# FrankYard/CDV-SLAM

Hardware: AMD Instinct MI355X
Metric: frames/sec per GPU (CDVO update, 96 patches, win=10); ATE vs ref (higher is better)
Workload: dtype f32

## Files before the change

cdv_slam_amd/csrc/cdv_graph.h:

```cpp
#pragma once
#include <stddef.h>
#include <stdint.h>

namespace cdv {

enum {
  GM_U = 0,
  GM_KMIN = 2,
  GM_KMAX = 3,
  GM_JMIN = 4,
  GM_JMAX = 5,
  GM_ERROR = 6,
  GM_E = 7,
  GM_KRANGE = 8,
  GM_HAS_II = 9,
  GM_STAGE = 16,
  GM_MODE = 20,
  GM_GEN = 21,
  GM_TCAP = 23,
  GM_GENNEXT = 24,
  GM_PRECN = 26,
  GM_OVFN = 28,
  GM_TERR = 30,
  GM_WORDS = 64
};

constexpr int GRAPH_MAX_BLOCKS = 1024;
constexpr int ELL_SLOTS = 32;
constexpr int ELL_CHUNKS = 4096;
constexpr int TAB_MAX_DEG = 128;
constexpr int64_t TAB_CAP_MAX = 1 << 16;
constexpr int ORD_BINS = 32;
constexpr int CORR_REC_WORDS = 24;

struct CorrStream {
  const float* coords;
  uint32_t kmod, jmod, kmagic, jmagic, Ng, slots;
  float inv_scale0;
};

struct GraphLayout {
  int64_t E_max, k_range;
  size_t meta, stage, khist, kcount, kcursor, krank, koff_u, kx, ku, pcsr_tmp, pcsr, prec, pell, nprev, nnext, ocnt, order, crec,
      tcur, town, tdeg, tplo, tkid, tlive, ttab, tovf, tprec, total;
  int64_t tab_chunks;
  int64_t ell_chunks;
};

static inline size_t align256(size_t x) { return (x + 255) & ~(size_t)255; }

static inline GraphLayout graph_layout(int64_t E_max, int64_t k_range) {
  GraphLayout L;
  L.E_max = E_max; L.k_range = k_range;
  const int64_t U_max = k_range < E_max ? k_range : E_max;
  size_t o = 0;
  L.meta = o;     o = align256(o + sizeof(int32_t) * GM_WORDS);
  L.stage = o;    o = align256(o + sizeof(int32_t) * 4 * GRAPH_MAX_BLOCKS);
  L.khist = o;    o = align256(o + sizeof(int32_t) * (size_t)(k_range + 1));
  L.kcount = o;   o = align256(o + sizeof(int32_t) * (size_t)(k_range + 1));
  L.kcursor = o;  o = align256(o + sizeof(int32_t) * (size_t)(k_range + 1));
  L.krank = o;    o = align256(o + sizeof(int32_t) * (size_t)k_range);
  L.koff_u = o;   o = align256(o + sizeof(int32_t) * (size_t)(U_max + 1));
  L.kx = o;       o = align256(o + sizeof(int64_t) * (size_t)U_max);
  L.ku = o;       o = align256(o + sizeof(int32_t) * (size_t)E_max);
  L.pcsr_tmp = o; o = align256(o + sizeof(int32_t) * 4 * (size_t)E_max);
  L.pcsr = o;     o = align256(o + sizeof(int32_t) * (size_t)E_max);
  L.prec = o;     o = align256(o + sizeof(int32_t) * 4 * (size_t)E_max);
  L.ell_chunks = (U_max + 15) / 16 < ELL_CHUNKS ? (U_max + 15) / 16 : ELL_CHUNKS;
  L.pell = o;     o = align256(o + sizeof(int32_t) * 4 * 16 * (size_t)ELL_SLOTS * (size_t)L.ell_chunks);
  L.nprev = o;    o = align256(o + sizeof(int32_t) * (size_t)E_max);
  L.nnext = o;    o = align256(o + sizeof(int32_t) * (size_t)E_max);
  L.ocnt = o;     o = align256(o + sizeof(int32_t) * ORD_BINS * GRAPH_MAX_BLOCKS);
  L.order = o;    o = align256(o + sizeof(int32_t) * (size_t)E_max);
  L.crec = o;     o = align256(o + sizeof(uint32_t) * CORR_REC_WORDS * (size_t)E_max);
  const int64_t tcap = k_range < TAB_CAP_MAX ? k_range : TAB_CAP_MAX;
  L.tab_chunks = (tcap + 15) / 16;
  L.tcur = o;     o = align256(o + sizeof(int32_t) * (size_t)(tcap + 16));
  L.town = o;     o = align256(o + sizeof(uint64_t) * (size_t)(tcap + 16));
  L.tdeg = o;     o = align256(o + sizeof(int32_t) * (size_t)(tcap + 16));
  L.tplo = o;     o = align256(o + sizeof(int32_t) * (size_t)(tcap + 16));
  L.tkid = o;     o = align256(o + sizeof(int32_t) * (size_t)(tcap + 16));
  L.tlive = o;    o = align256(o + sizeof(int32_t) * (size_t)(tcap / 8 + 2));
  L.ttab = o;     o = align256(o + sizeof(int32_t) * 4 * 16 * (size_t)ELL_SLOTS * (size_t)L.tab_chunks);
  L.tovf = o;     o = align256(o + sizeof(int32_t) * 4 * (size_t)E_max);
  L.tprec = o;    o = align256(o + sizeof(int32_t) * 4 * ((size_t)E_max + 1));
  L.total = o;
  return L;
}

struct GraphView {
  int32_t* meta;
  int32_t *stage, *khist, *kcount, *kcursor, *krank, *koff_u, *ku, *pcsr_tmp, *pcsr, *prec, *pell, *nprev, *nnext, *ocnt, *order;
  uint32_t* crec;
  int32_t *tcur, *tdeg, *tplo, *tkid, *tlive, *ttab, *tovf, *tprec;
  unsigned long long* town;
  int64_t* kx;
};

static inline GraphView graph_view(void* ws, const GraphLayout& L) {
  char* b = (char*)ws;
  GraphView v;
  v.meta = (int32_t*)(b + L.meta);
  v.stage = (int32_t*)(b + L.stage);
  v.khist = (int32_t*)(b + L.khist);
  v.kcount = (int32_t*)(b + L.kcount);
  v.kcursor = (int32_t*)(b + L.kcursor);
  v.krank = (int32_t*)(b + L.krank);
  v.koff_u = (int32_t*)(b + L.koff_u);
  v.kx = (int64_t*)(b + L.kx);
  v.ku = (int32_t*)(b + L.ku);
  v.pcsr_tmp = (int32_t*)(b + L.pcsr_tmp);
  v.pcsr = (int32_t*)(b + L.pcsr);
  v.prec = (int32_t*)(b + L.prec);
  v.pell = (int32_t*)(b + L.pell);
  v.nprev = (int32_t*)(b + L.nprev);
  v.nnext = (int32_t*)(b + L.nnext);
  v.ocnt = (int32_t*)(b + L.ocnt);
  v.order = (int32_t*)(b + L.order);
  v.crec = (uint32_t*)(b + L.crec);
  v.tcur = (int32_t*)(b + L.tcur);
  v.tdeg = (int32_t*)(b + L.tdeg);
  v.tplo = (int32_t*)(b + L.tplo);
  v.town = (unsigned long long*)(b + L.town);
  v.tkid = (int32_t*)(b + L.tkid);
  v.tlive = (int32_t*)(b + L.tlive);
  v.ttab = (int32_t*)(b + L.ttab);
  v.tovf = (int32_t*)(b + L.tovf);
  v.tprec = (int32_t*)(b + L.tprec);
  return v;
}

}

bool cdv_graph_lookup(const void* ws, cdv::GraphLayout* out);

void cdv_graph_forget(const void* ws);

void cdv_graph_no_corr_order(const void* ws);

bool cdv_graph_has_ii(const void* ws);

bool cdv_graph_is_table(const void* ws);
int64_t cdv_graph_table_capacity(const void* ws);

namespace cdv {
__device__ __forceinline__ int graph_error(const int32_t* __restrict__ meta) {
  const int e = meta[GM_ERROR], t0 = meta[GM_TERR], t1 = meta[GM_TERR + 1], g = meta[GM_GEN];
  return meta[GM_MODE] ? ((g & 1) ? t1 : t0) : e;
}
__device__ __forceinline__ int graph_error_of(const int32_t* __restrict__ meta, bool table) {
  const int e = meta[GM_ERROR], t0 = meta[GM_TERR], t1 = meta[GM_TERR + 1], g = meta[GM_GEN];
  return table ? ((g & 1) ? t1 : t0) : e;
}
}

namespace cdv { struct TFillArgs; }
int cdv_graph_table_prepare(const int64_t* ii, const int64_t* jj, const int64_t* kk, int64_t E, void* ws, size_t ws_bytes,
                            int64_t E_max, int64_t k_range, int64_t tab_cap, int64_t* ix, int64_t* jx, void* stream,
                            cdv::TFillArgs* fill, int* fill_blocks, const int32_t* dyn = nullptr);
int cdv_graph_table_finish(const cdv::TFillArgs& fill, int fill_blocks, void* ws, int64_t E_max, int64_t k_range, int64_t* ix,
                           int64_t* jx, const float* poses, const float* patches, const float* intr, float* coords_out,
                           bool with_stream, void* stream);

namespace cdv { struct HistArgs; }
int cdv_graph_prepare(const int64_t* jj, const int64_t* kk, int64_t E, void* ws, size_t ws_bytes, int64_t E_max,
                      int64_t k_range, int64_t* ix, int64_t* jx, void* stream, cdv::HistArgs* hist, int* hist_blocks);
int cdv_graph_finish(const int64_t* ii, const int64_t* jj, const int64_t* kk, int64_t E, void* ws, int64_t E_max,
                     int64_t k_range, int hist_blocks, int64_t* ix, int64_t* jx, void* stream);
```

cdv_slam_amd/csrc/corr.hip:

```cpp
#include <math.h>
#include <stdlib.h>

#include "cdv_common.h"
#include "cdv_graph.h"
#include "cdv_parts.h"

CDV_STAMP_TU(corr)

#ifdef CDV_STAMPS
#define CDV_EXP(bit) ((exp & (bit)) != 0)
#else
#define CDV_EXP(bit) false
#endif

namespace {

constexpr int PADX = CDV_FMAP_PADX;
constexpr int PADY = CDV_FMAP_PADY;

constexpr int RAW_ROWS = 12;
constexpr int NQ_MAX = 8;
constexpr int RAW_MSH = RAW_ROWS * 16 + 12;
constexpr int RAW_HALFS = 9 * RAW_MSH;
constexpr int CW = 4;
constexpr int OUT_POLICY = 16;
constexpr int OUT_HALFS = 896;
constexpr int WAVE_LDS_BYTES = RAW_HALFS * 2 + OUT_HALFS * 2;
constexpr int DUMP_OFF_B = 3712;
constexpr int WAVE_LDS2_BYTES = DUMP_OFF_B + 512;
static_assert(RAW_HALFS * 2 <= DUMP_OFF_B && OUT_HALFS * 2 <= RAW_HALFS * 2, "LDS layout");

typedef _Float16 cdv_half4 __attribute__((ext_vector_type(4)));
typedef _Float16 cdv_half2 __attribute__((ext_vector_type(2)));

__device__ __forceinline__ void wave_lds_sync() {
  asm volatile("s_waitcnt lgkmcnt(0)" ::: "memory");
  __builtin_amdgcn_wave_barrier();
}

template <bool IS_MIN>
__device__ __forceinline__ int row16_reduce_i32(int v) {
#define CDV_ROR(n)                                                                                             \
  if (IS_MIN) asm volatile("s_nop 1\n\tv_min_i32_dpp %0, %1, %1 row_ror:" #n " row_mask:0xf bank_mask:0xf" : "=v"(v) : "0"(v)); \
  else asm volatile("s_nop 1\n\tv_max_i32_dpp %0, %1, %1 row_ror:" #n " row_mask:0xf bank_mask:0xf" : "=v"(v) : "0"(v));
  CDV_ROR(8) CDV_ROR(4) CDV_ROR(2) CDV_ROR(1)
#undef CDV_ROR
  return v;
}

__device__ __forceinline__ void row16_minmax4(int x, int y, int& xmin, int& xmax, int& ymin, int& ymax) {
  int a = x, b = x, c = y, d = y;
#define CDV_STEP(n)                                                                                  \
  asm volatile("v_min_i32_dpp %0, %0, %0 row_ror:" #n " row_mask:0xf bank_mask:0xf\n\t"               \
               "v_max_i32_dpp %1, %1, %1 row_ror:" #n " row_mask:0xf bank_mask:0xf\n\t"               \
               "v_min_i32_dpp %2, %2, %2 row_ror:" #n " row_mask:0xf bank_mask:0xf\n\t"               \
               "v_max_i32_dpp %3, %3, %3 row_ror:" #n " row_mask:0xf bank_mask:0xf"                    \
               : "+v"(a), "+v"(b), "+v"(c), "+v"(d));
  asm volatile("s_nop 1" ::: "memory");
  CDV_STEP(8) CDV_STEP(4) CDV_STEP(2) CDV_STEP(1)
#undef CDV_STEP
  xmin = a; xmax = b; ymin = c; ymax = d;
}

struct LevelParams {
  const _Float16* fmap;
  int H, W;
  float inv_scale;
  int shift;
};

struct Box {
  int x0, y0;
  int Wb, Hb;
  bool fast;
  int stride;
  bool outside;
  int x0c, y0c;
};

__device__ __forceinline__ int floor_clamped(float v) {
  return (int)fminf(fmaxf(floorf(v), -1.0e6f), 1.0e6f);
}

__device__ __forceinline__ Box make_box(int ixmin, int ixmax, int iymin, int iymax, const LevelParams& LP) {
  Box b;
  b.x0 = ixmin - 3;
  b.y0 = iymin - 3;
  b.Wb = ixmax + 4 - b.x0 + 1;
  b.Hb = iymax + 4 - b.y0 + 1;
  b.fast = (b.Wb <= 16) && (b.Hb <= RAW_ROWS);
  b.stride = b.fast ? b.Wb : 16;
  b.x0c = min(max(b.x0, -PADX), LP.W);
  b.y0c = min(max(b.y0, -PADY), LP.H);
  b.outside = (b.x0c != b.x0) || (b.y0c != b.y0);
  return b;
}

template <int KS>
__device__ __forceinline__ void mfma_row_store(const cdv_half8 (&win)[KS], const cdv_half8 (&pat)[KS],
                                               _Float16* __restrict__ raw_lane, int t) {
  cdv_float4 acc = {0.f, 0.f, 0.f, 0.f};
#pragma unroll
  for (int s = 0; s < KS; s++) acc = __builtin_amdgcn_mfma_f32_16x16x32_f16(win[s], pat[s], acc, 0, 0, 0);
  cdv_half4 h = {(_Float16)acc[0], (_Float16)acc[1], (_Float16)acc[2], (_Float16)acc[3]};
  *reinterpret_cast<cdv_half4*>(raw_lane + t * 16) = h;
}

struct BlendGeo {
  int hb;
  int stride_b;
  cdv_half2 wx;
  float dy;
};

__device__ __forceinline__ BlendGeo blend_geo(float xm, float ym, int m, int xo, const LevelParams& LP,
                                              const Box& b, bool per_pixel) {
  BlendGeo g;
  const float x = xm * LP.inv_scale, y = ym * LP.inv_scale;
  const float fxf = floorf(x), fyf = floorf(y);
  const float dx = (float)(_Float16)(x - fxf);
  g.wx = cdv_half2{(_Float16)(1.0f - dx), (_Float16)dx};
  g.dy = (float)(_Float16)(y - fyf);
  const int bx = per_pixel ? 0 : floor_clamped(x) - 3 - b.x0;
  const int by = per_pixel ? 0 : floor_clamped(y) - 3 - b.y0;
  g.hb = 2 * (m * RAW_MSH + __mul24(by, b.stride) + bx + xo);
  g.stride_b = 2 * b.stride;
  return g;
}

__device__ __forceinline__ float dot2_f16(uint32_t pair, uint32_t w) {
  float r;
  asm("v_dot2_f32_f16 %0, %1, %2, 0" : "=v"(r) : "v"(pair), "v"(w));
  return r;
}

template <typename TR>
__device__ __forceinline__ void blend_level(const _Float16* __restrict__ raw, const BlendGeo& g, TR (&res)[7]) {
  const char* rb = reinterpret_cast<const char*>(raw);
  float h[8];
  const int hb1 = g.hb + g.stride_b;
  const char* p0 = rb + (g.hb & ~3);
  const char* p1 = rb + (hb1 & ~3);
  const unsigned s0 = (unsigned)g.hb << 3, s1 = (unsigned)hb1 << 3;
  const int step2 = 2 * g.stride_b;
  const uint32_t wxb = __builtin_bit_cast(uint32_t, g.wx);
#pragma unroll
  for (int r = 0; r < 8; r++) {
    const uint32_t* pd = reinterpret_cast<const uint32_t*>((r & 1) ? p1 : p0);
    const uint32_t lo = pd[0], hi = pd[1];
    const uint32_t pr = __builtin_amdgcn_alignbit(hi, lo, (r & 1) ? s1 : s0);
    h[r] = dot2_f16(pr, wxb);
    if (r & 1) p1 += step2; else p0 += step2;
  }
#pragma unroll
  for (int yo = 0; yo < 7; yo++) res[yo] = (TR)__builtin_fmaf(g.dy, h[yo + 1] - h[yo], h[yo]);
}

template <int KS, int LM = 1>
__device__ __forceinline__ void slow_level(const LevelParams& LP, int64_t jslot, float xv, float yv,
                                           const cdv_half8 (&pat)[KS], _Float16* __restrict__ raw, int lane, int C) {
  const int n = lane & 15, g = lane >> 4;
  const int Wp = LP.W + 2 * PADX, Hp = LP.H + 2 * PADY;
  const _Float16* fbase = LP.fmap + (size_t)jslot * Hp * Wp * C;
#pragma unroll 1
  for (int m = 0; m < 9; m++) {
    const float xm = __int_as_float(__builtin_amdgcn_readlane(__float_as_int(xv), LM * m));
    const float ym = __int_as_float(__builtin_amdgcn_readlane(__float_as_int(yv), LM * m));
    const int x0 = floor_clamped(xm * LP.inv_scale) - 3, y0 = floor_clamped(ym * LP.inv_scale) - 3;
    const int x0c = min(max(x0, -PADX), LP.W), y0c = min(max(y0, -PADY), LP.H);
    const bool outside = (x0c != x0) || (y0c != y0);
#pragma unroll 1
    for (int t2 = 0; t2 < 4; t2++) {
      const int py = y0c + PADY + 2 * t2 + (n >> 3), px = x0c + PADX + (n & 7);
      cdv_float4 acc = {0.f, 0.f, 0.f, 0.f};
#pragma unroll
      for (int s = 0; s < KS; s++) {
        const int chg = min(32 * s + 8 * g, C - 8);
        const cdv_half8 v = *reinterpret_cast<const cdv_half8*>(fbase + ((size_t)py * Wp + px) * C + chg);
        acc = __builtin_amdgcn_mfma_f32_16x16x32_f16(v, pat[s], acc, 0, 0, 0);
      }
      if (n == m) {
        const int row = 2 * t2 + (g >> 1), col = 4 * (g & 1);
        cdv_half4 h = {(_Float16)acc[0], (_Float16)acc[1], (_Float16)acc[2], (_Float16)acc[3]};
        if (outside) h = cdv_half4{0, 0, 0, 0};
        *reinterpret_cast<cdv_half4*>(raw + m * RAW_MSH + row * 16 + col) = h;
      }
    }
  }
}

__device__ __forceinline__ void zero_raw(_Float16* __restrict__ raw, int lane) {
  typedef uint32_t cdv_u32x4z __attribute__((ext_vector_type(4)));
  const cdv_u32x4z z = {0u, 0u, 0u, 0u};
  for (int i = lane; i < RAW_HALFS / 8; i += 64) reinterpret_cast<cdv_u32x4z*>(raw)[i] = z;
}

template <int KS>
__global__ __launch_bounds__(256) void corr_wide_kernel(const _Float16* __restrict__ gmap, LevelParams L0,
                                                         LevelParams L1, const float* __restrict__ coords,
                                                         const int64_t* __restrict__ kk,
                                                         const int64_t* __restrict__ jj,
                                                         const int32_t* __restrict__ order,
                                                         _Float16* __restrict__ out, int E, int64_t Ng, int64_t slots,
                                                         int C, int nlev, int64_t kmod, int64_t jmod, uint32_t kmagic,
                                                         uint32_t jmagic, int gmap_pm,
                                                         int exp) {
  extern __shared__ __attribute__((aligned(16))) unsigned char smem_raw[];
  const int lane = threadIdx.x & 63;
  const int wave = __builtin_amdgcn_readfirstlane(threadIdx.x >> 6);
  _Float16* raw = reinterpret_cast<_Float16*>(smem_raw + (size_t)wave * WAVE_LDS_BYTES);
  _Float16* outT = raw + RAW_HALFS;
  const int p = blockIdx.x * 4 + wave;
  if (p >= E) return;
  const int e = order ? __builtin_amdgcn_readfirstlane(order[p]) : p;
  CDV_STAMP(corr, p, 0);

  int64_t kpatch = kk[e], jslot = jj[e];
  if (kmod > 0 && kpatch >= 0 && kpatch < ((int64_t)1 << 31)) {
    const uint32_t x = (uint32_t)kpatch, d = (uint32_t)kmod;
    const uint32_t q = __builtin_amdgcn_readfirstlane((int)__umulhi(x, kmagic));
    const int32_t r = (int32_t)(x - q * d);
    kpatch = (d == 1u) ? 0 : (r < 0 ? r + (int32_t)d : r);
  }
  if (jmod > 0 && jslot >= 0 && jslot < ((int64_t)1 << 31)) {
    const uint32_t x = (uint32_t)jslot, d = (uint32_t)jmod;
    const uint32_t q = __builtin_amdgcn_readfirstlane((int)__umulhi(x, jmagic));
    const int32_t r = (int32_t)(x - q * d);
    jslot = (d == 1u) ? 0 : (r < 0 ? r + (int32_t)d : r);
  }
  const bool idx_ok = kpatch >= 0 && kpatch < Ng && jslot >= 0 && jslot < slots;
  if (!idx_ok) { kpatch = 0; jslot = 0; }
  if (CDV_EXP(16)) jslot = 0;
  const float* cptr = coords + (size_t)e * 18;
  const int mm = lane < 9 ? lane : 0;
  const int bm = min(lane / 7, 8), bxo = lane - 7 * (lane / 7);
  const int cval = __float_as_int(cptr[min(lane, 17)]);
  const float xv = __int_as_float(__builtin_amdgcn_ds_bpermute(4 * mm, cval));
  const float yv = __int_as_float(__builtin_amdgcn_ds_bpermute(4 * (9 + mm), cval));
  const float xb = __int_as_float(__builtin_amdgcn_ds_bpermute(4 * bm, cval));
  const float yb = __int_as_float(__builtin_amdgcn_ds_bpermute(4 * (9 + bm), cval));
  const int ixl = floor_clamped(xv * L0.inv_scale), iyl = floor_clamped(yv * L0.inv_scale);
  const int ixmin = __builtin_amdgcn_readfirstlane(row16_reduce_i32<true>(ixl));
  const int ixmax = __builtin_amdgcn_readfirstlane(row16_reduce_i32<false>(ixl));
  const int iymin = __builtin_amdgcn_readfirstlane(row16_reduce_i32<true>(iyl));
  const int iymax = __builtin_amdgcn_readfirstlane(row16_reduce_i32<false>(iyl));
  const Box b0 = make_box(ixmin, ixmax, iymin, iymax, L0);
  const int sh1 = nlev == 2 ? L1.shift : 0;
  const Box b1 = make_box(ixmin >> sh1, ixmax >> sh1, iymin >> sh1, iymax >> sh1, nlev == 2 ? L1 : L0);
  CDV_STAMP(corr, p, 1);

  const int n = lane & 15, g = lane >> 4;
  cdv_half8 pat[KS];
  if (gmap_pm) {
    typedef int cdv_i32x4p __attribute__((ext_vector_type(4)));
    const unsigned tile_b = 9u * (unsigned)C * 2u;
    const auto rs = __builtin_amdgcn_make_buffer_rsrc(
        const_cast<char*>(reinterpret_cast<const char*>(gmap) + (size_t)kpatch * tile_b), (short)0, (int)tile_b, 0x00020000);
#pragma unroll
    for (int s = 0; s < KS; s++) {
      const int chg = 32 * s + 8 * g;
      const unsigned voff = (chg < C) ? (unsigned)(n * C + chg) * 2u : 0x40000000u;
      pat[s] = __builtin_bit_cast(cdv_half8, (cdv_i32x4p)__builtin_amdgcn_raw_buffer_load_b128(rs, (int)voff, 0, 0));
    }
  } else {
    const _Float16* gp = gmap + (size_t)kpatch * C * 9 + (n < 9 ? n : 0);
#pragma unroll
    for (int s = 0; s < KS; s++) {
#pragma unroll
      for (int j = 0; j < 8; j++) {
        const int ch = 32 * s + 8 * g + j;
        const _Float16 v = gp[min(ch, C - 1) * 9];
        pat[s][j] = (n < 9 && ch < C) ? v : (_Float16)0.f;
      }
    }
  }

  float res0[7], res1[7];
#pragma unroll
  for (int i = 0; i < 7; i++) { res0[i] = 0.f; res1[i] = 0.f; }
  _Float16* raw_lane = (n < 9) ? raw + n * RAW_MSH + 4 * g : outT + ((n - 9) * 4 + g) * 4;

  for (int lev = 0; lev < nlev; lev++) {
    const LevelParams& LP = lev == 0 ? L0 : L1;
    Box b = lev == 0 ? b0 : b1;
    b.stride = 16;
    const int Wp = LP.W + 2 * PADX, Hp = LP.H + 2 * PADY;
    if (lev == 1) wave_lds_sync();
    if (b.fast && !b.outside) {
      const _Float16* fb = LP.fmap + (((size_t)jslot * Hp + (b.y0c + PADY)) * Wp + (b.x0c + PADX)) * C;
      for (int t = 0; t < b.Hb; t++) {
        cdv_half8 wa[KS];
#pragma unroll
        for (int s = 0; s < KS; s++)
          wa[s] = *reinterpret_cast<const cdv_half8*>(fb + ((size_t)t * Wp + n) * C + min(32 * s + 8 * g, C - 8));
        cdv_float4 acc = {0.f, 0.f, 0.f, 0.f};
#pragma unroll
        for (int s = 0; s < KS; s++) acc = __builtin_amdgcn_mfma_f32_16x16x32_f16(wa[s], pat[s], acc, 0, 0, 0);
        if (n < 9) {
          cdv_half4 h = {(_Float16)acc[0], (_Float16)acc[1], (_Float16)acc[2], (_Float16)acc[3]};
          *reinterpret_cast<cdv_half4*>(raw_lane + t * 16) = h;
        }
      }
    } else if (!b.fast) {
      slow_level<KS>(LP, jslot, xv, yv, pat, raw, lane, C);
    }
    wave_lds_sync();
    if (!(b.fast && b.outside)) {
      const BlendGeo gg = blend_geo(xb, yb, bm, bxo, LP, b, !b.fast);
      if (lev == 0) blend_level(raw, gg, res0); else blend_level(raw, gg, res1);
    }
  }

  if (lane < 63 && !CDV_EXP(512)) {
    if (nlev == 2) {
      uint32_t* o32 = reinterpret_cast<uint32_t*>(outT) + bxo * 63 + bm;
#pragma unroll
      for (int yo = 0; yo < 7; yo++) {
        const _Float16 h0 = idx_ok ? (_Float16)res0[yo] : (_Float16)0.f;
        const _Float16 h1 = idx_ok ? (_Float16)res1[yo] : (_Float16)0.f;
        const uint32_t lo = __builtin_bit_cast(unsigned short, h0), hi = __builtin_bit_cast(unsigned short, h1);
        o32[yo * 9] = lo | (hi << 16);
      }
    } else {
#pragma unroll
      for (int yo = 0; yo < 7; yo++) outT[(bxo * 7 + yo) * 9 + bm] = idx_ok ? (_Float16)res0[yo] : (_Float16)0.f;
    }
  }
  wave_lds_sync();
  CDV_STAMP(corr, p, 7);
  if (!CDV_EXP(2)) {
  if (nlev == 2) {
    const uint32_t* src = reinterpret_cast<const uint32_t*>(outT);
    uint32_t* dst = reinterpret_cast<uint32_t*>(out) + (size_t)e * 441;
    typedef uint32_t cdv_u32x4 __attribute__((ext_vector_type(4)));
    typedef uint32_t cdv_u32x4u __attribute__((ext_vector_type(4), aligned(4)));
    const cdv_u32x4 v0 = *reinterpret_cast<const cdv_u32x4*>(src + 4 * lane);
    *reinterpret_cast<cdv_u32x4u*>(dst + 4 * lane) = v0;
    if (lane < 46) {
      const cdv_u32x4 v1 = *reinterpret_cast<const cdv_u32x4*>(src + 256 + 4 * lane);
      *reinterpret_cast<cdv_u32x4u*>(dst + 256 + 4 * lane) = v1;
    }
    if (lane == 63) dst[440] = src[440];
  } else {
    _Float16* dst = out + (size_t)e * 441;
#pragma unroll
    for (int i = 0; i < 7; i++) {
      const int t = i * 64 + lane;
      if (t < 441) dst[t] = outT[t];
    }
  }
  }
  CDV_STAMP(corr, p, 8);
}

struct CorrLevel {
  const char* base_m;
  int H, W;
  float inv_scale;
  int shift;
  uint32_t pitch;
  uint32_t slot_bytes;
};
struct CorrArgs2 {
  const float* coords;
  const int64_t* kk;
  const int64_t* jj;
  const int32_t* order;
  int E;
  uint32_t kmod, jmod, kmagic, jmagic;
  uint32_t Ng, slots;
  const char* gmap;
  _Float16* out;
  CorrLevel L0, L1;
  int C;
  int gmap_pm;
  int exp;
  int out_stride, out_off, out_pitch;
  const float* coords_ref;
  float ref_mul;
  const uint32_t* rec;
  const int32_t* dynE;
};

constexpr uint32_t FBIAS = 0x4B000000u;

__device__ __forceinline__ LevelParams level_params(const CorrLevel& L) {
  return LevelParams{reinterpret_cast<const _Float16*>(L.base_m + (size_t)FBIAS), L.H, L.W, L.inv_scale, L.shift};
}

struct EdgeCoords {
  int cval;
  float xb, yb;
  int ixmin, ixmax, iymin, iymax;
};

template <int CC, int NLEV, bool REC>
__device__ __forceinline__ void corr_edge(const CorrArgs2& a, int p, int e, const EdgeCoords& ec, uint32_t kq, uint32_t jq,
                                          bool idx_ok, int lane, _Float16* __restrict__ raw, _Float16* __restrict__ outT) {
  CDV_STAMP(corr, p, 0);
  const int C = CC ? CC : a.C;
#ifdef CDV_STAMPS
  const int exp = a.exp;
#endif
  const int mm = lane < 9 ? lane : 0;
  const int bm = min(lane / 7, 8), bxo = lane - 7 * (lane / 7);
  const int n = lane & 15, g = lane >> 4;
  if (!idx_ok) { kq = 0u; jq = 0u; }
  if (CDV_EXP(16)) jq = 0u;
  const int64_t jslot = (int64_t)jq;

  typedef int cdv_i32x4 __attribute__((ext_vector_type(4)));
  cdv_half8 pat[1];
  if (a.gmap_pm) {
    const unsigned tile_b = 9u * (unsigned)C * 2u;
    const auto rs = __builtin_amdgcn_make_buffer_rsrc(const_cast<char*>(a.gmap) + (size_t)(kq * tile_b), (short)0,
                                                      (int)tile_b, 0x00020000);
    const unsigned voff = (8 * g < C) ? (unsigned)(n * C + 8 * g) * 2u : 0x40000000u;
    pat[0] = __builtin_bit_cast(cdv_half8, (cdv_i32x4)__builtin_amdgcn_raw_buffer_load_b128(rs, (int)voff, 0, 0));
  } else {
    const _Float16* gp = reinterpret_cast<const _Float16*>(a.gmap) + (size_t)kq * C * 9 + (n < 9 ? n : 0);
#pragma unroll
    for (int j = 0; j < 8; j++) {
      const int ch = 8 * g + j;
      const _Float16 v = gp[min(ch, C - 1) * 9];
      pat[0][j] = (n < 9 && ch < C) ? v : (_Float16)0.f;
    }
  }

  const LevelParams L0 = level_params(a.L0), L1 = level_params(NLEV == 2 ? a.L1 : a.L0);
  float xv, yv, xb, yb;
  int ixmin, ixmax, iymin, iymax;
  if (REC) {
    xb = ec.xb; yb = ec.yb;
    xv = xb; yv = yb;
    ixmin = ec.ixmin; ixmax = ec.ixmax; iymin = ec.iymin; iymax = ec.iymax;
  } else {
    const int cval = ec.cval;
    xv = __int_as_float(__builtin_amdgcn_ds_bpermute(4 * mm, cval));
    yv = __int_as_float(__builtin_amdgcn_ds_bpermute(4 * (9 + mm), cval));
    xb = __int_as_float(__builtin_amdgcn_ds_bpermute(4 * bm, cval));
    yb = __int_as_float(__builtin_amdgcn_ds_bpermute(4 * (9 + bm), cval));
    const int ixl = floor_clamped(xv * L0.inv_scale), iyl = floor_clamped(yv * L0.inv_scale);
    int vxmin, vxmax, vymin, vymax;
    row16_minmax4(ixl, iyl, vxmin, vxmax, vymin, vymax);
    ixmin = __builtin_amdgcn_readfirstlane(vxmin); ixmax = __builtin_amdgcn_readfirstlane(vxmax);
    iymin = __builtin_amdgcn_readfirstlane(vymin); iymax = __builtin_amdgcn_readfirstlane(vymax);
  }
  const Box b0 = make_box(ixmin, ixmax, iymin, iymax, L0);
  const int sh1 = NLEV == 2 ? L1.shift : 0;
  const Box b1 = make_box(ixmin >> sh1, ixmax >> sh1, iymin >> sh1, iymax >> sh1, L1);
  CDV_STAMP(corr, p, 1);

  _Float16 res0[7], res1[7];
  _Float16* raw_lane = (n < 9) ? raw + n * RAW_MSH + 4 * g
                               : reinterpret_cast<_Float16*>(reinterpret_cast<char*>(raw) + DUMP_OFF_B +
                                                             4 * ((n * (RAW_MSH / 2) + 2 * g) & 31));

  const unsigned CB = (unsigned)C * 2u;
  const char* r0 = a.L0.base_m + (size_t)(jq * a.L0.slot_bytes + (unsigned)(b0.y0c + PADY) * a.L0.pitch +
                                          (unsigned)(b0.x0c + PADX) * CB);
  const CorrLevel& A1 = NLEV == 2 ? a.L1 : a.L0;
  const char* r1 = A1.base_m + (size_t)(jq * A1.slot_bytes + (unsigned)(b1.y0c + PADY) * A1.pitch +
                                        (unsigned)(b1.x0c + PADX) * CB);
  const unsigned pitch0 = a.L0.pitch, pitch1 = A1.pitch;
  cdv_half8 w[NQ_MAX][1];
  const bool do0 = b0.fast && !b0.outside && idx_ok;
  const bool do1 = NLEV == 2 && b1.fast && !b1.outside && idx_ok;
  const int nq0 = (b0.Wb * b0.Hb + 15) >> 4, nq1 = (b1.Wb * b1.Hb + 15) >> 4;
  typedef float cdv_f32x2 __attribute__((ext_vector_type(2)));
  const float nhalf = (float)n + 0.5f;
  const float lanebase = (8 * g < C) ? (float)((unsigned)n * CB + (unsigned)(8 * g) * 2u) + 8388608.0f : 33554432.0f;
  constexpr int NQF0 = 8, NQF1 = 6;
#define CDV2_LOAD_SETUP(BX, RB, PITCH)                                                             \
    const unsigned Wb_ = (unsigned)(BX).Wb, pitch_ = (PITCH);                                      \
    const auto rsrc_ = __builtin_amdgcn_make_buffer_rsrc(const_cast<char*>(RB), (short)0,          \
                                                         (int)((unsigned)(BX).Hb * pitch_ + FBIAS), 0x00020000); \
    const float invW_ = __builtin_amdgcn_rcpf((float)Wb_);                                         \
    const float wrapf_ = (float)(pitch_ - Wb_ * CB);                                               \
    const cdv_f32x2 dtb_ = {16.0f * invW_, (float)(16u * CB)};
#define CDV2_LD1(q)                                                                                \
    {                                                                                              \
      const float vf_ = __builtin_fmaf(__builtin_floorf(tb_[0]), wrapf_, tb_[1]);                  \
      const cdv_i32x4 v_ = __builtin_amdgcn_raw_buffer_load_b128(rsrc_, __float_as_int(vf_), 0, 0); \
      w[q][0] = __builtin_bit_cast(cdv_half8, v_);                                                 \
      tb_ += dtb_;                                                                                 \
    }
#define CDV2_LOAD_FIXED(BX, RB, PITCH, NQF, NQ)                                                    \
  {                                                                                                \
    CDV2_LOAD_SETUP(BX, RB, PITCH)                                                                 \
    cdv_f32x2 tb_ = {nhalf * invW_, lanebase};                                                     \
    CDV2_LD1(0) CDV2_LD1(1) CDV2_LD1(2) CDV2_LD1(3) CDV2_LD1(4)                                    \
    if (NQF > 6) { CDV2_LD1(5) CDV2_LD1(6) }                                                       \
    if ((NQ) >= (NQF)) { CDV2_LD1(NQF - 1) }                                                       \
  }
#define CDV2_MF1(WQ, q)                                                                            \
    {                                                                                              \
      cdv_float4 acc = {0.f, 0.f, 0.f, 0.f};                                                       \
      acc = __builtin_amdgcn_mfma_f32_16x16x32_f16(WQ, pat[0], acc, 0, 0, 0);                      \
      cdv_half4 h = {(_Float16)acc[0], (_Float16)acc[1], (_Float16)acc[2], (_Float16)acc[3]};      \
      *reinterpret_cast<cdv_half4*>(raw_lane + (q) * 16) = h;                                      \
    }
#define CDV2_MF2(qa, qb) CDV2_MF1(w[qa][0], qa) CDV2_MF1(w[qb][0], qb) __builtin_amdgcn_sched_barrier(0);
#define CDV2_MFMA_FIXED(NQF, NQ)                                                                   \
  {                                                                                                \
    CDV2_MF2(0, 1) CDV2_MF2(2, 3)                                                                  \
    if (NQF > 6) { CDV2_MF2(4, 5) CDV2_MF1(w[6][0], 6) } else { CDV2_MF1(w[4][0], 4) }             \
    if ((NQ) >= (NQF)) { CDV2_MF1(w[NQF - 1][0], NQF - 1) }                                        \
  }
#define CDV2_TAIL(BX, RB, PITCH, NQF, NQ)                                                          \
  if ((NQ) > (NQF)) {                                                                              \
    CDV2_LOAD_SETUP(BX, RB, PITCH)                                                                 \
    cdv_f32x2 tb_ = {(nhalf + (float)(16 * (NQF))) * invW_, lanebase + (float)(16u * (unsigned)(NQF) * CB)}; \
    _Pragma("unroll 1") for (int q_ = (NQF); q_ < (NQ); q_++) {                                    \
      const float vf_ = __builtin_fmaf(__builtin_floorf(tb_[0]), wrapf_, tb_[1]);                  \
      const cdv_i32x4 v_ = __builtin_amdgcn_raw_buffer_load_b128(rsrc_, __float_as_int(vf_), 0, 0); \
      tb_ += dtb_;                                                                                 \
      CDV2_MF1(__builtin_bit_cast(cdv_half8, v_), q_)                                              \
    }                                                                                              \
  }
  if (do0 && !CDV_EXP(1)) CDV2_LOAD_FIXED(b0, r0, pitch0, NQF0, nq0)
  const BlendGeo g0 = blend_geo(xb, yb, bm, bxo, L0, b0, !b0.fast);
  const BlendGeo g1 = blend_geo(xb, yb, bm, bxo, L1, b1, !b1.fast);
  CDV_STAMP(corr, p, 2);
  if (do0 && !CDV_EXP(256)) {
    CDV2_MFMA_FIXED(NQF0, nq0)
    CDV2_TAIL(b0, r0, pitch0, NQF0, nq0)
  } else if (!b0.fast && idx_ok) {
    slow_level<1, REC ? 7 : 1>(L0, jslot, xv, yv, pat, raw, lane, C);
  } else {
    zero_raw(raw, lane);
  }
  __builtin_amdgcn_sched_barrier(0);
  if (do1 && !CDV_EXP(1)) CDV2_LOAD_FIXED(b1, r1, pitch1, NQF1, nq1)
  wave_lds_sync();
  CDV_STAMP(corr, p, 3);
  if (!CDV_EXP(128)) blend_level(raw, g0, res0);
  CDV_STAMP(corr, p, 4);
  if (NLEV == 2) {
    wave_lds_sync();
    if (do1 && !CDV_EXP(256)) {
      CDV2_MFMA_FIXED(NQF1, nq1)
      CDV2_TAIL(b1, r1, pitch1, NQF1, nq1)
    } else if (!b1.fast && idx_ok) {
      slow_level<1, REC ? 7 : 1>(L1, jslot, xv, yv, pat, raw, lane, C);
    } else {
      zero_raw(raw, lane);
    }
    wave_lds_sync();
    CDV_STAMP(corr, p, 5);
    if (!CDV_EXP(128)) blend_level(raw, g1, res1);
    CDV_STAMP(corr, p, 6);
  }
#undef CDV2_LOAD_FIXED
#undef CDV2_LOAD_SETUP
#undef CDV2_LD1
#undef CDV2_MF1
#undef CDV2_MF2
#undef CDV2_MFMA_FIXED
#undef CDV2_TAIL

  wave_lds_sync();
  if (lane < 63 && !CDV_EXP(512)) {
    if (NLEV == 2) {
      uint32_t* o32 = reinterpret_cast<uint32_t*>(outT) + __mul24(bxo, 63) + bm;
#pragma unroll
      for (int yo = 0; yo < 7; yo++) {
        const cdv_half2 h = {res0[yo], res1[yo]};
        o32[yo * 9] = __builtin_bit_cast(uint32_t, h);
      }
    } else {
#pragma unroll
      for (int yo = 0; yo < 7; yo++) outT[(bxo * 7 + yo) * 9 + bm] = res0[yo];
    }
  }
  wave_lds_sync();
  CDV_STAMP(corr, p, 7);
  if (!CDV_EXP(2)) {
    if (NLEV == 2) {
      const uint32_t* src = reinterpret_cast<const uint32_t*>(outT);
      uint32_t* dst = reinterpret_cast<uint32_t*>(a.out) + (size_t)e * 441;
      typedef uint32_t cdv_u32x4 __attribute__((ext_vector_type(4)));
      const cdv_u32x4 v0 = *reinterpret_cast<const cdv_u32x4*>(src + 4 * lane);
      typedef int cdv_i32x4s __attribute__((ext_vector_type(4)));
      const auto rso = __builtin_amdgcn_make_buffer_rsrc(reinterpret_cast<char*>(dst), (short)0, 1768, 0x00020000);
      __builtin_amdgcn_raw_buffer_store_b128((cdv_i32x4s)v0, rso, 16 * lane, 0, OUT_POLICY);
      if (lane < 46) {
        const cdv_u32x4 v1 = *reinterpret_cast<const cdv_u32x4*>(src + 256 + 4 * lane);
        __builtin_amdgcn_raw_buffer_store_b128((cdv_i32x4s)v1, rso, 1024 + 16 * lane, 0, OUT_POLICY);
      }
      if (lane == 63) __builtin_amdgcn_raw_buffer_store_b32((int)src[440], rso, 1760, 0, OUT_POLICY);
    } else {
      _Float16* dst = a.out + (size_t)e * a.out_pitch + a.out_off;
#pragma unroll
      for (int i = 0; i < 7; i++) {
        const int t = i * 64 + lane;
        if (t < 441) dst[t * a.out_stride] = outT[t];
      }
    }
  }
  CDV_STAMP(corr, p, 8);
}

__device__ __forceinline__ bool ring_index(int64_t v64, uint32_t mod, uint32_t magic, uint32_t limit, uint32_t& q) {
  q = (uint32_t)v64;
  const bool small = (uint32_t)(v64 >> 32) == 0u && q < 0x80000000u;
  if (mod > 1u) {
    const int32_t r = (int32_t)(q - __umulhi(q, magic) * mod);
    q = (uint32_t)(r < 0 ? r + (int32_t)mod : r);
  } else if (mod == 1u) {
    q = 0u;
  }
  return small && q < limit;
}

template <int CC, int NLEV, bool REC = false>
__global__ __launch_bounds__(64 * CW) void corr_fused2_kernel(const uint32_t* __restrict__ rec_h, const int32_t* __restrict__ dynE_h,
                                                          int E_h, int eighth_h, const CorrArgs2 a) {
  extern __shared__ __attribute__((aligned(16))) unsigned char smem_raw[];
  const int lane = threadIdx.x & 63;
  const int wave = __builtin_amdgcn_readfirstlane(threadIdx.x >> 6);
  _Float16* raw = reinterpret_cast<_Float16*>(smem_raw + (size_t)wave * WAVE_LDS2_BYTES);
  _Float16* outT = raw;
  int E = E_h, eighth = eighth_h;
  if (REC && dynE_h) {
    E = min(__builtin_amdgcn_readfirstlane(*dynE_h), E_h);
    eighth = (E + 8 * CW - 1) / (8 * CW);
    if (((int)blockIdx.x >> 3) >= eighth) return;
  }
  const int p0 = (((int)blockIdx.x & 7) * eighth + ((int)blockIdx.x >> 3)) * CW + wave;
  if (p0 >= E) return;
  if (REC) {
    const uint32_t* r = rec_h + (size_t)p0 * cdv::CORR_REC_WORDS;
    const int bm = min(lane / 7, 8);
    EdgeCoords ec;
    ec.cval = 0;
    ec.xb = __int_as_float((int)r[bm]);
    ec.yb = __int_as_float((int)r[9 + bm]);
    const int e = (int)r[18];
    const uint32_t kq = r[19], jq = r[20];
    const int bx = (int)r[21], by = (int)r[22];
    ec.ixmin = (int)(short)(bx & 0xffff); ec.ixmax = bx >> 16;
    ec.iymin = (int)(short)(by & 0xffff); ec.iymax = by >> 16;
    corr_edge<CC, NLEV, true>(a, p0, e, ec, kq, jq, jq != 0xFFFFFFFFu, lane, raw, outT);
    return;
  }
  const int e = a.order ? __builtin_amdgcn_readfirstlane(a.order[p0]) : p0;
  const int cval = __float_as_int(a.coords[(size_t)e * 18 + min(lane, 17)]);
  if (NLEV == 1 && a.coords_ref) {
    const float r = a.coords_ref[(size_t)e * 18 + min(lane, 17)] * a.ref_mul;
    if (__all(lane >= 18 || __float_as_int(r) == cval)) return;
  }
  uint32_t kq, jq;
  const bool k_ok = ring_index(a.kk[e], a.kmod, a.kmagic, a.Ng, kq);
  const bool j_ok = ring_index(a.jj[e], a.jmod, a.jmagic, a.slots, jq);
  EdgeCoords ec;
  ec.cval = cval;
  corr_edge<CC, NLEV, false>(a, p0, e, ec, kq, jq, k_ok && j_ok, lane, raw, outT);
}

template <typename T>
__global__ __launch_bounds__(256) void corr_generic_kernel(const T* __restrict__ fmap1, const T* __restrict__ fmap2,
                                                           const float* __restrict__ coords,
                                                           const int64_t* __restrict__ us,
                                                           const int64_t* __restrict__ vs, T* __restrict__ out,
                                                           int64_t M, int64_t N1, int64_t N2, int C, int P, int H2,
                                                           int W2, int R) {
  const int D1 = 2 * R + 1;
  const int64_t total = M * D1 * D1 * P * P;
  for (int64_t idx = (int64_t)blockIdx.x * blockDim.x + threadIdx.x; idx < total;
       idx += (int64_t)gridDim.x * blockDim.x) {
    int64_t t = idx;
    const int j0 = (int)(t % P); t /= P;
    const int i0 = (int)(t % P); t /= P;
    const int yo = (int)(t % D1); t /= D1;
    const int xo = (int)(t % D1); t /= D1;
    const int64_t m = t;
    const int64_t ix = us[m], jx = vs[m];
    const float x = coords[((m * 2 + 0) * P + i0) * P + j0];
    const float y = coords[((m * 2 + 1) * P + i0) * P + j0];
    const float fxf = floorf(x), fyf = floorf(y);
    const float dx = (float)(T)(x - fxf), dy = (float)(T)(y - fyf);
    const int fx = (int)fminf(fmaxf(fxf, -1.0e6f), 1.0e6f), fy = (int)fminf(fmaxf(fyf, -1.0e6f), 1.0e6f);
    float c[2][2];
    const bool idx_ok = ix >= 0 && ix < N1 && jx >= 0 && jx < N2;
#pragma unroll
    for (int a = 0; a < 2; a++)
#pragma unroll
      for (int b = 0; b < 2; b++) {
        const int i1 = fy + yo + a - R, j1 = fx + xo + b - R;
        float s = 0.f;
        if (idx_ok && i1 >= 0 && i1 < H2 && j1 >= 0 && j1 < W2) {
          const T* p1 = fmap1 + ((ix * C) * P + i0) * P + j0;
          const T* p2 = fmap2 + ((jx * C) * (int64_t)H2 + i1) * W2 + j1;
          for (int ch = 0; ch < C; ch++) s += (float)p1[(int64_t)ch * P * P] * (float)p2[(int64_t)ch * H2 * W2];
        }
        c[a][b] = s;
      }
    const float v = (1.f - dx) * (1.f - dy) * c[0][0] + dx * (1.f - dy) * c[0][1] + (1.f - dx) * dy * c[1][0] +
                    dx * dy * c[1][1];
    out[idx] = (T)v;
  }
}

__global__ __launch_bounds__(256) void nchw_to_nhwc_kernel(const _Float16* __restrict__ src,
                                                           _Float16* __restrict__ dst, int64_t first, int64_t count,
                                                           int C, int H, int W) {
  const int G = C / 8;
  const int64_t total = count * H * W * G;
  for (int64_t idx = (int64_t)blockIdx.x * blockDim.x + threadIdx.x; idx < total;
       idx += (int64_t)gridDim.x * blockDim.x) {
    int64_t t = idx;
    const int xw = (int)(t % W); t /= W;
    const int gq = (int)(t % G); t /= G;
    const int yh = (int)(t % H); t /= H;
    const int64_t nslot = first + t;
    cdv_half8 v;
#pragma unroll
    for (int j = 0; j < 8; j++) v[j] = src[((nslot * C + 8 * gq + j) * H + yh) * W + xw];
    *reinterpret_cast<cdv_half8*>(dst + ((nslot * (H + 2 * PADY) + yh + PADY) * (W + 2 * PADX) + xw + PADX) * C +
                                  8 * gq) = v;
  }
}

constexpr int FP_PARTS = 16;

__device__ __forceinline__ void fingerprint_body(const uint32_t* __restrict__ src, int64_t words_per_slot,
                                                 uint64_t* __restrict__ fp, int bid) {
  const int slot = bid / FP_PARTS, part = bid % FP_PARTS;
  typedef uint32_t u32x4 __attribute__((ext_vector_type(4)));
  const u32x4* p = reinterpret_cast<const u32x4*>(src + (size_t)slot * words_per_slot);
  const int64_t n4 = words_per_slot / 4;
  uint64_t acc = 0;
  for (int64_t i = (int64_t)part * 256 + threadIdx.x; i < n4; i += (int64_t)FP_PARTS * 256) {
    const u32x4 v = p[i];
    const uint64_t key = 0x9E3779B97F4A7C15ull + 2ull * (uint64_t)i;
    acc += ((uint64_t)v[0] | ((uint64_t)v[1] << 32)) * key;
    acc += ((uint64_t)v[2] | ((uint64_t)v[3] << 32)) * (key ^ 0xD6E8FEB86659FD92ull);
  }
#pragma unroll
  for (int o = 32; o > 0; o >>= 1) acc += __shfl_xor(acc, o);
  __shared__ uint64_t sw[4];
  if ((threadIdx.x & 63) == 0) sw[threadIdx.x >> 6] = acc;
  __syncthreads();
  if (threadIdx.x == 0) fp[(size_t)slot * FP_PARTS + part] = (sw[0] + sw[1]) + (sw[2] + sw[3]) + 1ull;
}

__global__ __launch_bounds__(256) void fmap_fingerprint_kernel(const uint32_t* __restrict__ src, int64_t words_per_slot,
                                                               uint64_t* __restrict__ fp) {
  fingerprint_body(src, words_per_slot, fp, (int)blockIdx.x);
}

__device__ __forceinline__ void dirty_body(const _Float16* __restrict__ src, _Float16* __restrict__ dst, int C, int H, int W,
                                           const uint64_t* __restrict__ fp_new, const uint64_t* __restrict__ fp_old,
                                           int wg_per_slot, int32_t* __restrict__ n_dirty, int bid) {
  const int64_t nslot = bid / wg_per_slot;
  const int wg = bid % wg_per_slot;
  bool same = true;
#pragma unroll
  for (int i = 0; i < FP_PARTS; i++) same = same && fp_new[nslot * FP_PARTS + i] == fp_old[nslot * FP_PARTS + i];
  if (same) return;
  if (wg == 0 && threadIdx.x == 0 && n_dirty) atomicAdd(n_dirty, 1);
  const int G = C / 8;
  const int64_t total = (int64_t)H * W * G;
  for (int64_t idx = (int64_t)wg * 256 + threadIdx.x; idx < total; idx += (int64_t)wg_per_slot * 256) {
    int64_t t = idx;
    const int xw = (int)(t % W); t /= W;
    const int gq = (int)(t % G); t /= G;
    const int yh = (int)t;
    cdv_half8 v;
#pragma unroll
    for (int j = 0; j < 8; j++) v[j] = src[((nslot * C + 8 * gq + j) * H + yh) * W + xw];
    *reinterpret_cast<cdv_half8*>(dst + ((nslot * (H + 2 * PADY) + yh + PADY) * (W + 2 * PADX) + xw + PADX) * C +
                                  8 * gq) = v;
  }
}

__global__ __launch_bounds__(256) void nchw_to_nhwc_dirty_kernel(const _Float16* __restrict__ src,
                                                                 _Float16* __restrict__ dst, int C, int H, int W,
                                                                 const uint64_t* __restrict__ fp_new,
                                                                 const uint64_t* __restrict__ fp_old, int wg_per_slot,
                                                                 int32_t* __restrict__ n_dirty) {
  dirty_body(src, dst, C, H, W, fp_new, fp_old, wg_per_slot, n_dirty, (int)blockIdx.x);
}

struct ShadowJob {
  const _Float16* src; _Float16* dst;
  uint64_t *fp_new; const uint64_t* fp_old;
  int32_t* n_dirty;
  int64_t words_per_slot;
  int C, H, W, wg_per_slot, fp_blocks, cv_blocks;
};
struct ShadowJobs {
  ShadowJob j[2];
  int n;
  const _Float16* g_src; _Float16* g_dst;
  int64_t g_count;
  int g_C, g_blocks;
};

__global__ __launch_bounds__(256) void shadows_fingerprint_kernel(const ShadowJobs J) {
  int b = (int)blockIdx.x;
  for (int q = 0; q < J.n; q++) {
    if (b < J.j[q].fp_blocks) {
      fingerprint_body(reinterpret_cast<const uint32_t*>(J.j[q].src), J.j[q].words_per_slot, J.j[q].fp_new, b);
      return;
    }
    b -= J.j[q].fp_blocks;
  }
}

__global__ __launch_bounds__(256) void shadows_convert_kernel(const ShadowJobs J) {
  int b = (int)blockIdx.x;
  for (int q = 0; q < J.n; q++) {
    const ShadowJob& s = J.j[q];
    if (b < s.cv_blocks) {
      dirty_body(s.src, s.dst, s.C, s.H, s.W, s.fp_new, s.fp_old, s.wg_per_slot, s.n_dirty, b);
      return;
    }
    b -= s.cv_blocks;
  }
  if (J.g_src) cdv::gmap_pm_convert(J.g_src, J.g_dst, 0, J.g_count, J.g_C, (int64_t)b * 256 + threadIdx.x, (int64_t)J.g_blocks * 256);
}

__global__ __launch_bounds__(256) void gmap_pm_kernel(const _Float16* __restrict__ src, _Float16* __restrict__ dst,
                                                      int64_t first, int64_t count, int C) {
  cdv::gmap_pm_convert(src, dst, first, count, C, (int64_t)blockIdx.x * blockDim.x + threadIdx.x,
                       (int64_t)gridDim.x * blockDim.x);
}

__global__ __launch_bounds__(256) void fmap_ingest_kernel(cdv::IngestArgs a) {
  cdv::ingest_body(a, (int)blockIdx.x, (int)blockDim.x, (int)threadIdx.x);
}

template <typename T>
__global__ __launch_bounds__(256) void patchify_kernel(const T* __restrict__ net, const float* __restrict__ coords,
                                                       T* __restrict__ patches, int B, int64_t M, int C, int H, int W,
                                                       int R) {
  const int D = 2 * R + 2;
  const int64_t total = (int64_t)B * M * C * D * D;
  for (int64_t idx = (int64_t)blockIdx.x * blockDim.x + threadIdx.x; idx < total;
       idx += (int64_t)gridDim.x * blockDim.x) {
    int64_t t = idx;
    const int b2 = (int)(t % D); t /= D;
    const int a2 = (int)(t % D); t /= D;
    const int ch = (int)(t % C); t /= C;
    const int64_t m = t % M; t /= M;
    const int bb = (int)t;
    const float x = coords[(bb * M + m) * 2 + 0], y = coords[(bb * M + m) * 2 + 1];
    const int i = (int)fminf(fmaxf(floorf(y), -1.0e6f), 1.0e6f) + (a2 - R);
    const int j = (int)fminf(fmaxf(floorf(x), -1.0e6f), 1.0e6f) + (b2 - R);
    T v = (T)0.f;
    if (i >= 0 && i < H && j >= 0 && j < W) v = net[(((int64_t)bb * C + ch) * H + i) * W + j];
    patches[idx] = v;
  }
}

template <typename T>
__global__ __launch_bounds__(256) void patchify_blend_kernel(const T* __restrict__ net, const float* __restrict__ coords,
                                                             void* __restrict__ outv, int B, int64_t M, int C, int H,
                                                             int W, int R, int mode) {
  const int d = (mode == 2) ? 1 : 2 * R + 1;
  const int64_t total = (int64_t)B * M * C * d * d;
  for (int64_t idx = (int64_t)blockIdx.x * blockDim.x + threadIdx.x; idx < total;
       idx += (int64_t)gridDim.x * blockDim.x) {
    int64_t t = idx;
    const int b2 = (int)(t % d); t /= d;
    const int a2 = (int)(t % d); t /= d;
    const int ch = (int)(t % C); t /= C;
    const int64_t m = t % M; t /= M;
    const int bb = (int)t;
    const float x = coords[(bb * M + m) * 2 + 0], y = coords[(bb * M + m) * 2 + 1];
    const float fxf = floorf(x), fyf = floorf(y);
    const int i0 = (int)fminf(fmaxf(fyf, -1.0e6f), 1.0e6f) + (a2 - R);
    const int j0 = (int)fminf(fmaxf(fxf, -1.0e6f), 1.0e6f) + (b2 - R);
    const T* np = net + ((int64_t)bb * C + ch) * H * W;
    auto tap = [&](int i, int j) -> T { return (i >= 0 && i < H && j >= 0 && j < W) ? np[(int64_t)i * W + j] : (T)0.f; };
    if (mode == 2) {
      reinterpret_cast<T*>(outv)[idx] = tap(i0, j0);
    } else {
      const float dx = x - fxf, dy = y - fyf;
      const float x00 = (1.0f - dy) * (1.0f - dx) * (float)tap(i0, j0);
      const float x01 = (1.0f - dy) * dx * (float)tap(i0, j0 + 1);
      const float x10 = dy * (1.0f - dx) * (float)tap(i0 + 1, j0);
      const float x11 = dy * dx * (float)tap(i0 + 1, j0 + 1);
      reinterpret_cast<float*>(outv)[idx] = ((x00 + x01) + x10) + x11;
    }
  }
}

struct PatchifyJobs {
  cdv_patchify_job j[CDV_MAX_PATCHIFY_JOBS];
  int first[CDV_MAX_PATCHIFY_JOBS + 1];
  int n_jobs;
};

template <typename T>
__device__ __forceinline__ void patchify_job_body(const cdv_patchify_job& J, const float* __restrict__ coords, int64_t M,
                                                  int64_t idx0, int64_t stride) {
  const int R = J.radius, mode = J.mode, C = J.C, H = J.H, W = J.W;
  const int d = (mode == 2) ? 1 : 2 * R + 1;
  const int64_t total = M * C * d * d;
  const T* net = reinterpret_cast<const T*>(J.net);
  for (int64_t idx = idx0; idx < total; idx += stride) {
    int64_t t = idx;
    const int b2 = (int)(t % d); t /= d;
    const int a2 = (int)(t % d); t /= d;
    const int ch = (int)(t % C); t /= C;
    const int64_t m = t;
    const float x = (coords[m * 2 + 0] + J.ox) * J.sx, y = (coords[m * 2 + 1] + J.oy) * J.sy;
    const float fxf = floorf(x), fyf = floorf(y);
    const int i0 = (int)fminf(fmaxf(fyf, -1.0e6f), 1.0e6f) + (a2 - R);
    const int j0 = (int)fminf(fmaxf(fxf, -1.0e6f), 1.0e6f) + (b2 - R);
    const T* np = net + (int64_t)ch * H * W;
    auto tap = [&](int i, int j) -> T { return (i >= 0 && i < H && j >= 0 && j < W) ? np[(int64_t)i * W + j] : (T)0.f; };
    if (mode == 2) {
      reinterpret_cast<T*>(J.out)[idx] = tap(i0, j0);
    } else {
      const float dx = x - fxf, dy = y - fyf;
      const float x00 = (1.0f - dy) * (1.0f - dx) * (float)tap(i0, j0);
      const float x01 = (1.0f - dy) * dx * (float)tap(i0, j0 + 1);
      const float x10 = dy * (1.0f - dx) * (float)tap(i0 + 1, j0);
      const float x11 = dy * dx * (float)tap(i0 + 1, j0 + 1);
      reinterpret_cast<float*>(J.out)[idx] = ((x00 + x01) + x10) + x11;
    }
  }
}

__global__ __launch_bounds__(256) void patchify_multi_kernel(const PatchifyJobs P, const float* __restrict__ coords,
                                                             int64_t M) {
  int ji = 0;
  while (ji + 1 < P.n_jobs && (int)blockIdx.x >= P.first[ji + 1]) ji++;
  const cdv_patchify_job& J = P.j[ji];
  const int nb = P.first[ji + 1] - P.first[ji];
  const int64_t idx0 = (int64_t)((int)blockIdx.x - P.first[ji]) * 256 + threadIdx.x, stride = (int64_t)nb * 256;
  if (J.dtype == CDV_F16) patchify_job_body<_Float16>(J, coords, M, idx0, stride);
  else patchify_job_body<float>(J, coords, M, idx0, stride);
}

}

extern "C" int cdv_patchify_multi(const cdv_patchify_job* jobs, int n_jobs, const float* coords, int64_t M, void* stream) {
  CDV_REQUIRE(n_jobs >= 0 && n_jobs <= CDV_MAX_PATCHIFY_JOBS, CDV_ERR_ARG, "cdv_patchify_multi: too many jobs");
  if (n_jobs == 0 || M == 0) return CDV_OK;
  CDV_REQUIRE(jobs != nullptr && coords != nullptr && M > 0, CDV_ERR_ARG, "cdv_patchify_multi: NULL argument");
  PatchifyJobs P;
  P.n_jobs = n_jobs;
  P.first[0] = 0;
  for (int i = 0; i < n_jobs; i++) {
    const cdv_patchify_job& J = jobs[i];
    CDV_REQUIRE(J.dtype == CDV_F16 || J.dtype == CDV_F32, CDV_ERR_UNSUPPORTED, "cdv_patchify_multi: dtype must be f16 or f32");
    CDV_REQUIRE(J.mode == 1 || J.mode == 2, CDV_ERR_ARG, "cdv_patchify_multi: mode 1 (bilinear) or 2 (upperleft)");
    CDV_REQUIRE(J.net && J.out && J.C > 0 && J.H > 0 && J.W > 0 && J.radius >= 0, CDV_ERR_ARG, "cdv_patchify_multi: bad job");
    const int d = (J.mode == 2) ? 1 : 2 * J.radius + 1;
    const int64_t total = M * J.C * d * d;
    P.j[i] = J;
    P.first[i + 1] = P.first[i] + (int)(cdv_div_up(total, 256) < 4096 ? cdv_div_up(total, 256) : 4096);
  }
  hipLaunchKernelGGL(patchify_multi_kernel, dim3(P.first[n_jobs]), dim3(256), 0, (hipStream_t)stream, P, coords, M);
  CDV_LAUNCH_CHECK();
  return CDV_OK;
}

extern "C" int cdv_patchify_blend(const void* net, const float* coords, void* out, int B, int64_t M, int C, int H, int W,
                                  int radius, int mode, int dtype, void* stream) {
  CDV_REQUIRE(dtype == CDV_F16 || dtype == CDV_F32, CDV_ERR_UNSUPPORTED, "cdv_patchify_blend: dtype must be f16 or f32");
  CDV_REQUIRE(mode == 1 || mode == 2, CDV_ERR_ARG, "cdv_patchify_blend: mode 1 (bilinear) or 2 (upperleft)");
  const int d = (mode == 2) ? 1 : 2 * radius + 1;
  const int64_t total = (int64_t)B * M * C * d * d;
  if (total == 0) return CDV_OK;
  const int blocks = cdv_div_up(total, 256) < 16384 ? cdv_div_up(total, 256) : 16384;
  hipStream_t s = (hipStream_t)stream;
  if (dtype == CDV_F16)
    hipLaunchKernelGGL(patchify_blend_kernel<_Float16>, dim3(blocks), dim3(256), 0, s, (const _Float16*)net, coords, out,
                       B, M, C, H, W, radius, mode);
  else
    hipLaunchKernelGGL(patchify_blend_kernel<float>, dim3(blocks), dim3(256), 0, s, (const float*)net, coords, out, B, M,
                       C, H, W, radius, mode);
  CDV_LAUNCH_CHECK();
  return CDV_OK;
}

extern "C" int cdv_corr_fwd(const void* fmap1, const void* fmap2, const float* coords, const int64_t* us,
                            const int64_t* vs, void* out, int64_t M, int64_t N1, int64_t N2, int C, int P, int H2,
                            int W2, int radius, int dtype, void* stream) {
  CDV_REQUIRE(dtype == CDV_F16 || dtype == CDV_F32, CDV_ERR_UNSUPPORTED, "cdv_corr_fwd: dtype must be f16 or f32");
  CDV_REQUIRE(C > 0 && P > 0 && radius >= 0 && H2 > 0 && W2 > 0, CDV_ERR_ARG, "cdv_corr_fwd: bad shape");
  if (M == 0) return CDV_OK;
  const int D1 = 2 * radius + 1;
  const int64_t total = M * D1 * D1 * P * P;
  const int blocks = cdv_div_up(total, 256) < 65536 ? cdv_div_up(total, 256) : 65536;
  hipStream_t s = (hipStream_t)stream;
  if (dtype == CDV_F16)
    hipLaunchKernelGGL(corr_generic_kernel<_Float16>, dim3(blocks), dim3(256), 0, s, (const _Float16*)fmap1,
                       (const _Float16*)fmap2, coords, us, vs, (_Float16*)out, M, N1, N2, C, P, H2, W2, radius);
  else
    hipLaunchKernelGGL(corr_generic_kernel<float>, dim3(blocks), dim3(256), 0, s, (const float*)fmap1,
                       (const float*)fmap2, coords, us, vs, (float*)out, M, N1, N2, C, P, H2, W2, radius);
  CDV_LAUNCH_CHECK();
  return CDV_OK;
}

extern "C" size_t cdv_fmap_padded_elems(int64_t slots, int C, int H, int W) {
  return (size_t)slots * (size_t)(H + 2 * PADY) * (size_t)(W + 2 * PADX) * (size_t)C;
}

extern "C" int cdv_fmap_to_nhwc(const void* src_nchw, void* dst_nhwc, int64_t N, int C, int H, int W, int64_t first,
                                int64_t count, void* stream) {
  CDV_REQUIRE(C % 8 == 0 && C > 0, CDV_ERR_ARG, "cdv_fmap_to_nhwc: C must be a multiple of 8");
  CDV_REQUIRE(first >= 0 && count >= 0 && first + count <= N, CDV_ERR_ARG, "cdv_fmap_to_nhwc: slot range");
  CDV_REQUIRE_ALIGNED(dst_nhwc, 16, "cdv_fmap_to_nhwc: dst_nhwc must be 16-byte aligned");
  if (count == 0) return CDV_OK;
  const int64_t total = count * H * W * (C / 8);
  const int blocks = cdv_div_up(total, 256) < 16384 ? cdv_div_up(total, 256) : 16384;
  hipLaunchKernelGGL(nchw_to_nhwc_kernel, dim3(blocks), dim3(256), 0, (hipStream_t)stream, (const _Float16*)src_nchw,
                     (_Float16*)dst_nhwc, first, count, C, H, W);
  CDV_LAUNCH_CHECK();
  return CDV_OK;
}

extern "C" size_t cdv_fmap_sync_workspace_bytes(int64_t N) {
  return (size_t)(2 * (N > 0 ? N : 1) * FP_PARTS) * sizeof(uint64_t) + 64;
}

extern "C" int cdv_fmap_sync_nhwc(const void* src_nchw, void* dst_nhwc, int64_t N, int C, int H, int W, void* ws,
                                  int parity, void* stream) {
  CDV_REQUIRE(C % 8 == 0 && C > 0, CDV_ERR_ARG, "cdv_fmap_sync_nhwc: C must be a multiple of 8");
  CDV_REQUIRE(src_nchw && dst_nhwc && ws && N >= 0 && H > 0 && W > 0, CDV_ERR_ARG, "cdv_fmap_sync_nhwc: bad argument");
  CDV_REQUIRE_ALIGNED(dst_nhwc, 16, "cdv_fmap_sync_nhwc: dst_nhwc must be 16-byte aligned");
  CDV_REQUIRE_ALIGNED(src_nchw, 4, "cdv_fmap_sync_nhwc: src_nchw must be 4-byte aligned");
  CDV_REQUIRE_ALIGNED(ws, 16, "cdv_fmap_sync_nhwc: ws must be 16-byte aligned");
  if (N == 0) return CDV_OK;
  uint64_t* fp = (uint64_t*)ws;
  uint64_t* fp_new = fp + (size_t)(parity & 1) * N * FP_PARTS;
  const uint64_t* fp_old = fp + (size_t)((parity & 1) ^ 1) * N * FP_PARTS;
  int32_t* n_dirty = (int32_t*)(fp + 2 * (size_t)N * FP_PARTS);
  const int64_t words = (int64_t)C * H * W / 2;
  hipStream_t s = (hipStream_t)stream;
  hipLaunchKernelGGL(fmap_fingerprint_kernel, dim3((unsigned)(N * FP_PARTS)), dim3(256), 0, s, (const uint32_t*)src_nchw,
                     words, fp_new);
  const int wg_per_slot = (int)(cdv_div_up((int64_t)H * W * (C / 8), 256) < 64 ? cdv_div_up((int64_t)H * W * (C / 8), 256) : 64);
  hipLaunchKernelGGL(nchw_to_nhwc_dirty_kernel, dim3((unsigned)(N * wg_per_slot)), dim3(256), 0, s, (const _Float16*)src_nchw,
                     (_Float16*)dst_nhwc, C, H, W, fp_new, fp_old, wg_per_slot, n_dirty);
  CDV_LAUNCH_CHECK();
  return CDV_OK;
}

extern "C" int cdv_shadows_sync(const cdv_shadow_ring* rings, int n_rings, const void* gmap_planar, void* gmap_pm, int64_t Ng,
                                int C_tiles, void* stream) {
  CDV_REQUIRE(n_rings >= 0 && n_rings <= 2 && (n_rings == 0 || rings != nullptr), CDV_ERR_ARG, "cdv_shadows_sync: 0 to 2 rings");
  const bool do_g = gmap_planar != nullptr && gmap_pm != nullptr && Ng > 0;
  CDV_REQUIRE(!do_g || (C_tiles % 8 == 0 && C_tiles > 0), CDV_ERR_ARG, "cdv_shadows_sync: C of the tiles must be a multiple of 8");
  CDV_REQUIRE_ALIGNED(gmap_pm, 16, "cdv_shadows_sync: gmap_pm must be 16-byte aligned");
  for (int q = 0; q < n_rings; q++) {
    CDV_REQUIRE_ALIGNED(rings[q].dst_nhwc, 16, "cdv_shadows_sync: dst_nhwc must be 16-byte aligned");
    CDV_REQUIRE_ALIGNED(rings[q].src_nchw, 4, "cdv_shadows_sync: src_nchw must be 4-byte aligned");
    CDV_REQUIRE_ALIGNED(rings[q].ws, 16, "cdv_shadows_sync: ws must be 16-byte aligned");
  }
  ShadowJobs J;
  J.n = 0;
  int fp_total = 0, cv_total = 0;
  for (int q = 0; q < n_rings; q++) {
    const cdv_shadow_ring& r = rings[q];
    CDV_REQUIRE(r.C % 8 == 0 && r.C > 0 && r.src_nchw && r.dst_nhwc && r.ws && r.N >= 0 && r.H > 0 && r.W > 0, CDV_ERR_ARG,
                "cdv_shadows_sync: bad ring");
    if (r.N == 0) continue;
    ShadowJob& s = J.j[J.n++];
    uint64_t* fp = (uint64_t*)r.ws;
    s.src = (const _Float16*)r.src_nchw; s.dst = (_Float16*)r.dst_nhwc;
    s.fp_new = fp + (size_t)(r.parity & 1) * r.N * FP_PARTS;
    s.fp_old = fp + (size_t)((r.parity & 1) ^ 1) * r.N * FP_PARTS;
    s.n_dirty = (int32_t*)(fp + 2 * (size_t)r.N * FP_PARTS);
    s.words_per_slot = (int64_t)r.C * r.H * r.W / 2;
    s.C = r.C; s.H = r.H; s.W = r.W;
    const int64_t per = cdv_div_up((int64_t)r.H * r.W * (r.C / 8), 256);
    s.wg_per_slot = (int)(per < 64 ? per : 64);
    s.fp_blocks = (int)(r.N * FP_PARTS);
    s.cv_blocks = (int)(r.N * s.wg_per_slot);
    fp_total += s.fp_blocks; cv_total += s.cv_blocks;
  }
  J.g_src = do_g ? (const _Float16*)gmap_planar : nullptr;
  J.g_dst = (_Float16*)gmap_pm;
  J.g_count = Ng; J.g_C = C_tiles;
  const int64_t gtotal = do_g ? Ng * 9 * (C_tiles / 8) : 0;
  J.g_blocks = (int)(cdv_div_up(gtotal, 256) < 16384 ? cdv_div_up(gtotal, 256) : 16384);
  if (!do_g) J.g_blocks = 0;
  hipStream_t s = (hipStream_t)stream;
  if (fp_total > 0) hipLaunchKernelGGL(shadows_fingerprint_kernel, dim3((unsigned)fp_total), dim3(256), 0, s, J);
  if (cv_total + J.g_blocks > 0)
    hipLaunchKernelGGL(shadows_convert_kernel, dim3((unsigned)(cv_total + J.g_blocks)), dim3(256), 0, s, J);
  CDV_LAUNCH_CHECK();
  return CDV_OK;
}

extern "C" int cdv_frame_ingest(const void* fmap_chw, void* fmap1_nhwc, void* fmap2_nhwc, void* fmap1_nchw,
                                void* fmap2_nchw, int slot, int C, int H, int W, const void* gmap_planar, void* gmap_pm,
                                int64_t Ng, int64_t gmap_first, int64_t gmap_count, void* stream) {
  CDV_REQUIRE(C % 8 == 0 && C > 0, CDV_ERR_ARG, "cdv_fmap_ingest: C must be a multiple of 8");
  CDV_REQUIRE(H % 4 == 0 && W % 4 == 0, CDV_ERR_ARG, "cdv_fmap_ingest: H and W must be multiples of 4");
  CDV_REQUIRE(slot >= 0, CDV_ERR_ARG, "cdv_fmap_ingest: slot");
  CDV_REQUIRE_ALIGNED(fmap1_nhwc, 16, "cdv_fmap_ingest: fmap1_nhwc must be 16-byte aligned");
  CDV_REQUIRE_ALIGNED(fmap2_nhwc, 16, "cdv_fmap_ingest: fmap2_nhwc must be 16-byte aligned");
  CDV_REQUIRE_ALIGNED(gmap_pm, 16, "cdv_frame_ingest: gmap_pm must be 16-byte aligned");
  const bool do_g = gmap_planar != nullptr && gmap_pm != nullptr && gmap_count > 0;
  CDV_REQUIRE(!do_g || (gmap_first >= 0 && gmap_first + gmap_count <= Ng), CDV_ERR_ARG, "cdv_frame_ingest: tile range");
  const int64_t total = (int64_t)(H / 4) * (W / 4) * (C / 8) * 16;
  const int blocks = cdv_div_up(total, 256);
  const int gblocks = do_g ? (int)cdv_div_up(gmap_count * 9 * (C / 8), 256) : 0;
  const cdv::IngestArgs a{(const _Float16*)fmap_chw, (_Float16*)fmap1_nhwc, (_Float16*)fmap2_nhwc, (_Float16*)fmap1_nchw,
                          (_Float16*)fmap2_nchw, slot, C, H, W, (const _Float16*)gmap_planar, (_Float16*)gmap_pm,
                          gmap_first, gmap_count, blocks, gblocks};
  hipLaunchKernelGGL(fmap_ingest_kernel, dim3(blocks + gblocks), dim3(256), 0, (hipStream_t)stream, a);
  CDV_LAUNCH_CHECK();
  return CDV_OK;
}

extern "C" int cdv_fmap_ingest(const void* fmap_chw, void* fmap1_nhwc, void* fmap2_nhwc, void* fmap1_nchw,
                               void* fmap2_nchw, int slot, int C, int H, int W, void* stream) {
  return cdv_frame_ingest(fmap_chw, fmap1_nhwc, fmap2_nhwc, fmap1_nchw, fmap2_nchw, slot, C, H, W, nullptr, nullptr, 0,
                          0, 0, stream);
}

extern "C" int cdv_gmap_to_pixel_major(const void* gmap_planar, void* gmap_pm, int64_t Ng, int C, int64_t first,
                                       int64_t count, void* stream) {
  CDV_REQUIRE(C % 8 == 0 && C > 0, CDV_ERR_ARG, "cdv_gmap_to_pixel_major: C must be a multiple of 8");
  CDV_REQUIRE(first >= 0 && count >= 0 && first + count <= Ng, CDV_ERR_ARG, "cdv_gmap_to_pixel_major: tile range");
  CDV_REQUIRE_ALIGNED(gmap_pm, 16, "cdv_gmap_to_pixel_major: gmap_pm must be 16-byte aligned");
  if (count == 0) return CDV_OK;
  const int64_t total = count * 9 * (C / 8);
  const int blocks = cdv_div_up(total, 256) < 16384 ? cdv_div_up(total, 256) : 16384;
  hipLaunchKernelGGL(gmap_pm_kernel, dim3(blocks), dim3(256), 0, (hipStream_t)stream, (const _Float16*)gmap_planar,
                     (_Float16*)gmap_pm, first, count, C);
  CDV_LAUNCH_CHECK();
  return CDV_OK;
}

static int corr_fused_impl(const void* gmap, const void* fmap0_nhwc, const void* fmap1_nhwc, const float* coords,
                           const int64_t* kk, const int64_t* jj, const int32_t* order, void* out, int64_t E,
                           int64_t Ng, int64_t slots, int C, int H0, int W0, int H1, int W1, float scale0,
                           float scale1, int nlev, int64_t kmod, int64_t jmod, int gmap_pixel_major, void* stream,
                           int out_stride, int out_off, int out_pitch, const float* coords_ref, float ref_mul,
                           const uint32_t* rec = nullptr, const int32_t* dynE = nullptr) {
  CDV_REQUIRE(nlev == 1 || nlev == 2, CDV_ERR_ARG, "cdv_corr_fused: nlev must be 1 or 2");
  CDV_REQUIRE(C % 8 == 0 && C > 0 && C <= 128, CDV_ERR_UNSUPPORTED, "cdv_corr_fused: C must be a multiple of 8, <= 128");
  CDV_REQUIRE(E >= 0 && E < ((int64_t)1 << 31), CDV_ERR_ARG, "cdv_corr_fused: E out of range");
  int ex0 = 0, ex1 = 0;
  CDV_REQUIRE(scale0 > 0.f && frexpf(scale0, &ex0) == 0.5f && (nlev == 1 || (scale1 > 0.f && frexpf(scale1, &ex1) == 0.5f)),
              CDV_ERR_UNSUPPORTED, "cdv_corr_fused: pyramid scales must be powers of two (1 and 4 in SLAM.corr)");
  CDV_REQUIRE(fmap0_nhwc != nullptr && (nlev == 1 || fmap1_nhwc != nullptr), CDV_ERR_ARG, "cdv_corr_fused: NULL map");
  CDV_REQUIRE_ALIGNED(fmap0_nhwc, 16, "cdv_corr_fused: fmap0_nhwc must be 16-byte aligned");
  CDV_REQUIRE_ALIGNED(nlev == 2 ? fmap1_nhwc : nullptr, 16, "cdv_corr_fused: fmap1_nhwc must be 16-byte aligned");
  CDV_REQUIRE_ALIGNED(gmap_pixel_major ? gmap : nullptr, 16, "cdv_corr_fused: pixel-major gmap must be 16-byte aligned");
  CDV_REQUIRE_ALIGNED(out, 4, "cdv_corr_fused: out must be 4-byte aligned");
  CDV_REQUIRE(cdv_fmap_padded_elems(slots, C, H0, W0) * 2 < ((size_t)1 << 32) &&
                  (nlev == 1 || cdv_fmap_padded_elems(slots, C, H1, W1) * 2 < ((size_t)1 << 32)),
              CDV_ERR_UNSUPPORTED, "cdv_corr_fused: a feature ring of 4 GB or more");
  CDV_REQUIRE(kmod >= 0 && jmod >= 0 && kmod < ((int64_t)1 << 31) && jmod < ((int64_t)1 << 31), CDV_ERR_ARG,
              "cdv_corr_fused: kmod / jmod out of range");
  const uint32_t kmagic = kmod > 1 ? (uint32_t)((((uint64_t)1 << 32) + (uint64_t)kmod - 1) / (uint64_t)kmod) : 0u;
  const uint32_t jmagic = jmod > 1 ? (uint32_t)((((uint64_t)1 << 32) + (uint64_t)jmod - 1) / (uint64_t)jmod) : 0u;
  if (E == 0) return CDV_OK;
  CDV_REQUIRE(nlev == 1 || ex1 >= ex0, CDV_ERR_UNSUPPORTED, "cdv_corr_fused: level 1 must not be finer than level 0");
  const size_t smem = 4 * (size_t)(C <= 32 ? WAVE_LDS2_BYTES : WAVE_LDS_BYTES);
  static const int exp = getenv("CDV_CORR_EXP") ? atoi(getenv("CDV_CORR_EXP")) : 0;
  hipStream_t s = (hipStream_t)stream;
  if (C <= 32) {
    CDV_REQUIRE(Ng < ((int64_t)1 << 31) && slots < ((int64_t)1 << 31) && (size_t)Ng * 9 * (size_t)C * 2 < ((size_t)1 << 32),
                CDV_ERR_UNSUPPORTED, "cdv_corr_fused: 4 GB or more of patch tiles");
    auto level = [&](const void* ring, int H, int W, float scale, int shift) {
      const uint32_t pitch = (uint32_t)(W + 2 * PADX) * (uint32_t)C * 2u;
      return CorrLevel{(const char*)ring - (size_t)FBIAS, H, W, 1.0f / scale, shift, pitch, pitch * (uint32_t)(H + 2 * PADY)};
    };
    const CorrLevel A0 = level(fmap0_nhwc, H0, W0, scale0, 0);
    const CorrArgs2 a{coords, kk, jj, order, (int)E, (uint32_t)kmod, (uint32_t)jmod, kmagic, jmagic, (uint32_t)Ng,
                      (uint32_t)slots, (const char*)gmap, (_Float16*)out, A0,
                      nlev == 2 ? level(fmap1_nhwc, H1, W1, scale1, ex1 - ex0) : A0, C, gmap_pixel_major, exp,
                      out_stride, out_off, out_pitch, coords_ref, ref_mul, rec, dynE};
    const int blocks = 8 * (int)cdv_div_up(E, 8 * CW);
    const size_t smem2 = (size_t)CW * WAVE_LDS2_BYTES;
    if (rec) {
      CDV_REQUIRE(nlev == 2 && coords_ref == nullptr, CDV_ERR_UNSUPPORTED, "cdv_corr_fused_stream: two fused levels only");
      if (C == 24) hipLaunchKernelGGL((corr_fused2_kernel<24, 2, true>), dim3(blocks), dim3(64 * CW), smem2, s, rec, dynE, (int)E, blocks >> 3, a);
      else hipLaunchKernelGGL((corr_fused2_kernel<0, 2, true>), dim3(blocks), dim3(64 * CW), smem2, s, rec, dynE, (int)E, blocks >> 3, a);
    } else if (nlev == 2 && C == 24)
      hipLaunchKernelGGL((corr_fused2_kernel<24, 2>), dim3(blocks), dim3(64 * CW), smem2, s, rec, dynE, (int)E, blocks >> 3, a);
    else if (nlev == 2)
      hipLaunchKernelGGL((corr_fused2_kernel<0, 2>), dim3(blocks), dim3(64 * CW), smem2, s, rec, dynE, (int)E, blocks >> 3, a);
    else if (C == 24)
      hipLaunchKernelGGL((corr_fused2_kernel<24, 1>), dim3(blocks), dim3(64 * CW), smem2, s, rec, dynE, (int)E, blocks >> 3, a);
    else
      hipLaunchKernelGGL((corr_fused2_kernel<0, 1>), dim3(blocks), dim3(64 * CW), smem2, s, rec, dynE, (int)E, blocks >> 3, a);
  } else {
    CDV_REQUIRE(out_stride == 1 && out_off == 0 && coords_ref == nullptr, CDV_ERR_UNSUPPORTED,
                "cdv_corr_fused: checked calls need C <= 32");
    LevelParams L0{(const _Float16*)fmap0_nhwc, H0, W0, 1.0f / scale0, 0};
    LevelParams L1{(const _Float16*)fmap1_nhwc, H1, W1, nlev == 2 ? 1.0f / scale1 : 1.0f, nlev == 2 ? ex1 - ex0 : 0};
    hipLaunchKernelGGL(corr_wide_kernel<4>, dim3(cdv_div_up(E, 4)), dim3(256), smem, s, (const _Float16*)gmap, L0, L1, coords,
                       kk, jj, order, (_Float16*)out, (int)E, Ng, slots, C, nlev, kmod, jmod, kmagic, jmagic,
                       gmap_pixel_major, exp);
  }
  CDV_LAUNCH_CHECK();
  return CDV_OK;
}

extern "C" int cdv_corr_fused(const void* gmap, const void* fmap0_nhwc, const void* fmap1_nhwc, const float* coords,
                              const int64_t* kk, const int64_t* jj, const int32_t* order, void* out, int64_t E,
                              int64_t Ng, int64_t slots, int C, int H0, int W0, int H1, int W1, float scale0,
                              float scale1, int nlev, int64_t kmod, int64_t jmod, int gmap_pixel_major, void* stream) {
  return corr_fused_impl(gmap, fmap0_nhwc, fmap1_nhwc, coords, kk, jj, order, out, E, Ng, slots, C, H0, W0, H1, W1, scale0,
                         scale1, nlev, kmod, jmod, gmap_pixel_major, stream, 1, 0, 441, nullptr, 1.0f);
}

extern "C" int cdv_corr_fused_stream(const void* gmap, const void* fmap0_nhwc, const void* fmap1_nhwc, const void* records,
                                     void* out, int64_t E, int64_t Ng, int64_t slots, int C, int H0, int W0, int H1, int W1,
                                     float scale0, float scale1, int gmap_pixel_major, void* stream) {
  CDV_REQUIRE(records != nullptr, CDV_ERR_ARG, "cdv_corr_fused_stream: NULL record stream");
  CDV_REQUIRE(C <= 32, CDV_ERR_UNSUPPORTED, "cdv_corr_fused_stream: C must be <= 32");
  return corr_fused_impl(gmap, fmap0_nhwc, fmap1_nhwc, nullptr, nullptr, nullptr, nullptr, out, E, Ng, slots, C, H0, W0, H1,
                         W1, scale0, scale1, 2, 0, 0, gmap_pixel_major, stream, 1, 0, 441, nullptr, 1.0f,
                         (const uint32_t*)records);
}

extern "C" int cdv_corr_fused_stream_dyn(const void* gmap, const void* fmap0_nhwc, const void* fmap1_nhwc, const void* records,
                                         void* out, int64_t E_bound, const int32_t* dyn, int64_t Ng, int64_t slots, int C, int H0,
                                         int W0, int H1, int W1, float scale0, float scale1, int gmap_pixel_major, void* stream) {
  CDV_REQUIRE(records != nullptr && dyn != nullptr, CDV_ERR_ARG, "cdv_corr_fused_stream_dyn: NULL record stream / dynamic block");
  CDV_REQUIRE(C <= 32, CDV_ERR_UNSUPPORTED, "cdv_corr_fused_stream_dyn: C must be <= 32");
  return corr_fused_impl(gmap, fmap0_nhwc, fmap1_nhwc, nullptr, nullptr, nullptr, nullptr, out, E_bound, Ng, slots, C, H0, W0,
                         H1, W1, scale0, scale1, 2, 0, 0, gmap_pixel_major, stream, 1, 0, 441, nullptr, 1.0f,
                         (const uint32_t*)records, dyn + CDV_DYN_E);
}

extern "C" int cdv_corr_level_checked_interleaved(const void* gmap, const void* fmap_nhwc, const float* coords,
                                                  const float* coords_ref, float ref_mul, const int64_t* kk, const int64_t* jj,
                                                  void* out, int level, int64_t E, int64_t Ng, int64_t slots, int C, int H, int W,
                                                  float scale, int64_t kmod, int64_t jmod, int gmap_pixel_major, void* stream) {
  CDV_REQUIRE(level == 0 || level == 1, CDV_ERR_ARG, "cdv_corr_level_checked_interleaved: level must be 0 or 1");
  CDV_REQUIRE(coords_ref != nullptr && out != nullptr, CDV_ERR_ARG, "cdv_corr_level_checked_interleaved: NULL argument");
  CDV_REQUIRE(C <= 32, CDV_ERR_UNSUPPORTED, "cdv_corr_level_checked_interleaved: C must be <= 32");
  return corr_fused_impl(gmap, fmap_nhwc, nullptr, coords, kk, jj, nullptr, out, E, Ng, slots, C, H, W, 0, 0, scale, 1.0f, 1,
                         kmod, jmod, gmap_pixel_major, stream, 2, level, 882, coords_ref, ref_mul);
}

extern "C" int cdv_patchify_fwd(const void* net, const float* coords, void* patches, int B, int64_t M, int C, int H,
                                int W, int radius, int dtype, void* stream) {
  CDV_REQUIRE(dtype == CDV_F16 || dtype == CDV_F32, CDV_ERR_UNSUPPORTED, "cdv_patchify_fwd: dtype must be f16 or f32");
  const int D = 2 * radius + 2;
  const int64_t total = (int64_t)B * M * C * D * D;
  if (total == 0) return CDV_OK;
  const int blocks = cdv_div_up(total, 256) < 16384 ? cdv_div_up(total, 256) : 16384;
  hipStream_t s = (hipStream_t)stream;
  if (dtype == CDV_F16)
    hipLaunchKernelGGL(patchify_kernel<_Float16>, dim3(blocks), dim3(256), 0, s, (const _Float16*)net, coords,
                       (_Float16*)patches, B, M, C, H, W, radius);
  else
    hipLaunchKernelGGL(patchify_kernel<float>, dim3(blocks), dim3(256), 0, s, (const float*)net, coords,
                       (float*)patches, B, M, C, H, W, radius);
  CDV_LAUNCH_CHECK();
  return CDV_OK;
}
```

cdv_slam_amd/csrc/graph.hip:

```cpp
#include <mutex>
#include <unordered_map>
#include <unordered_set>
#include <vector>

#include "cdv_common.h"
#include "cdv_graph.h"
#include "cdv_parts.h"

using namespace cdv;

CDV_STAMP_TU(graph)

namespace {

struct RegEntry {
  GraphLayout L;
  bool initialised;
  bool has_ii;
  CorrStream cs;
  bool table;
  int32_t tab_cap;
};
std::mutex g_reg_mutex;
std::unordered_map<const void*, RegEntry> g_registry;
std::unordered_set<const void*> g_no_order;


__global__ __launch_bounds__(256) void graph_init_kernel(int32_t* meta, int32_t* khist, int32_t* kcursor, int32_t* tcur,
                                                         unsigned long long* town, int64_t k_cap) {
  const int64_t n = k_cap + 1 > GM_WORDS ? k_cap + 1 : GM_WORDS;
  const int64_t tcap = (k_cap < TAB_CAP_MAX ? k_cap : TAB_CAP_MAX) + 16;
  for (int64_t t = (int64_t)blockIdx.x * blockDim.x + threadIdx.x; t < n; t += (int64_t)gridDim.x * blockDim.x) {
    if (t <= k_cap) {
      khist[t] = 0;
      kcursor[t] = 0;
      if (t < tcap) { tcur[t] = 0; town[t] = 0ull; }
    }
    if (t < GM_WORDS) {
      meta[t] = 0;
    }
  }
}

__global__ __launch_bounds__(256) void graph_hist_kernel(cdv::HistArgs a) {
  cdv::graph_hist_body(a, (int)blockIdx.x, (int)gridDim.x, (int)blockDim.x, (int)threadIdx.x);
}

__global__ __launch_bounds__(1024) void graph_scan_kernel(int32_t* meta, const int32_t* __restrict__ stage,
                                                          int nstage, int32_t* khist, int32_t* kcount,
                                                          int32_t* krank, int32_t E, int64_t k_cap) {
  cdv::graph_scan_wide_body(meta, stage, nstage, khist, kcount, krank, E, k_cap, (int)blockDim.x, (int)threadIdx.x);
}

constexpr int SCAN_WG = 64, SCAN_T = 256;
__device__ __forceinline__ void scan_wide_range(const int32_t* __restrict__ stage, int nstage, int32_t E, int64_t k_cap, int t,
                                                int (&mm)[4], bool& bad, int& n) {
  constexpr int IMAX = 0x7fffffff, IMIN = (int)0x80000000;
  __shared__ int s_mm[SCAN_T / 64][4];
  int kmin = IMAX, kmax = IMIN, jmin = IMAX, jmax = IMIN;
  for (int i = t; i < nstage; i += SCAN_T) {
    kmin = min(kmin, stage[4 * i]); kmax = max(kmax, stage[4 * i + 1]);
    jmin = min(jmin, stage[4 * i + 2]); jmax = max(jmax, stage[4 * i + 3]);
  }
#pragma unroll
  for (int o = 32; o > 0; o >>= 1) {
    kmin = min(kmin, __shfl_xor(kmin, o)); kmax = max(kmax, __shfl_xor(kmax, o));
    jmin = min(jmin, __shfl_xor(jmin, o)); jmax = max(jmax, __shfl_xor(jmax, o));
  }
  if ((t & 63) == 0) { s_mm[t >> 6][0] = kmin; s_mm[t >> 6][1] = kmax; s_mm[t >> 6][2] = jmin; s_mm[t >> 6][3] = jmax; }
  __syncthreads();
  for (int w = 0; w < SCAN_T / 64; w++) {
    kmin = min(kmin, s_mm[w][0]); kmax = max(kmax, s_mm[w][1]);
    jmin = min(jmin, s_mm[w][2]); jmax = max(jmax, s_mm[w][3]);
  }
  mm[0] = kmin; mm[1] = kmax; mm[2] = jmin; mm[3] = jmax;
  const int64_t krange = (E > 0) ? (int64_t)kmax - kmin + 1 : 0;
  bad = E > 0 && (kmin < 0 || krange > k_cap);
  n = (int)krange;
}
__device__ __forceinline__ int scan_wide_slice(int n) { return ((n + SCAN_WG - 1) / SCAN_WG + SCAN_T - 1) / SCAN_T * SCAN_T; }

__global__ __launch_bounds__(SCAN_T) void graph_scan_part_kernel(const int32_t* __restrict__ stage, int nstage, const int32_t* __restrict__ khist,
                                                                  int32_t* __restrict__ part, int32_t E, int64_t k_cap) {
  const int t = threadIdx.x;
  int mm[4], n; bool bad;
  scan_wide_range(stage, nstage, E, k_cap, t, mm, bad, n);
  __shared__ int s_sum[SCAN_T / 64], s_cnt[SCAN_T / 64];
  int32_t sum = 0, cnt = 0;
  if (!bad && E > 0) {
    const int R = (int)k_cap, b0 = mm[0] % R, S = scan_wide_slice(n);
    const int lo = min((int)blockIdx.x * S, n), hi = min(lo + S, n);
    for (int i = lo + t; i < hi; i += SCAN_T) {
      int bin = b0 + i; bin = (bin >= R) ? bin - R : bin;
      const int32_t v = khist[bin];
      sum += v; cnt += (v > 0);
    }
  }
#pragma unroll
  for (int o = 32; o > 0; o >>= 1) { sum += __shfl_xor(sum, o); cnt += __shfl_xor(cnt, o); }
  if ((t & 63) == 0) { s_sum[t >> 6] = sum; s_cnt[t >> 6] = cnt; }
  __syncthreads();
  if (t == 0) {
    int32_t a = 0, c = 0;
    for (int w = 0; w < SCAN_T / 64; w++) { a += s_sum[w]; c += s_cnt[w]; }
    part[2 * blockIdx.x] = a; part[2 * blockIdx.x + 1] = c;
  }
}

__global__ __launch_bounds__(SCAN_T) void graph_scan_apply_kernel(int32_t* meta, const int32_t* __restrict__ stage, int nstage, int32_t* khist,
                                                                   int32_t* kcount, int32_t* krank, const int32_t* __restrict__ part,
                                                                   int32_t E, int64_t k_cap) {
  const int t = threadIdx.x, lane = t & 63, wv = t >> 6;
  int mm[4], n; bool bad;
  scan_wide_range(stage, nstage, E, k_cap, t, mm, bad, n);
  const int R = (int)k_cap;
  if (blockIdx.x == 0 && t == 0) {
    meta[GM_KMIN] = mm[0]; meta[GM_KMAX] = mm[1]; meta[GM_JMIN] = mm[2]; meta[GM_JMAX] = mm[3];
    meta[GM_E] = E;
    meta[GM_ERROR] = bad ? 1 : 0;
    meta[GM_KRANGE] = bad ? 0 : n;
    if (bad || E == 0) meta[GM_U] = 0;
  }
  if (bad || E == 0) {
    for (int i = blockIdx.x * SCAN_T + t; i < R; i += gridDim.x * SCAN_T) khist[i] = 0;
    return;
  }
  __shared__ int s_a[SCAN_T / 64][4];
  int32_t run = 0, rk = 0, tot = 0, totc = 0;
  for (int w = t; w < SCAN_WG; w += SCAN_T) {
    const int32_t a = part[2 * w], c = part[2 * w + 1];
    tot += a; totc += c;
    if (w < (int)blockIdx.x) { run += a; rk += c; }
  }
#pragma unroll
  for (int o = 32; o > 0; o >>= 1) {
    run += __shfl_xor(run, o); rk += __shfl_xor(rk, o); tot += __shfl_xor(tot, o); totc += __shfl_xor(totc, o);
  }
  if (lane == 0) { s_a[wv][0] = run; s_a[wv][1] = rk; s_a[wv][2] = tot; s_a[wv][3] = totc; }
  __syncthreads();
  run = rk = tot = totc = 0;
  for (int w = 0; w < SCAN_T / 64; w++) { run += s_a[w][0]; rk += s_a[w][1]; tot += s_a[w][2]; totc += s_a[w][3]; }
  if (blockIdx.x == 0 && t == 0) { kcount[n] = tot; meta[GM_U] = totc; }
  const int b0 = mm[0] % R, S = scan_wide_slice(n);
  const int lo = min((int)blockIdx.x * S, n), hi = min(lo + S, n);
  __shared__ int s_ws[SCAN_T / 64], s_wc[SCAN_T / 64];
  for (int i0 = lo; i0 < hi; i0 += SCAN_T) {
    const int i = i0 + t;
    const bool in = i < hi;
    int bin = b0 + min(i, hi - 1); bin = (bin >= R) ? bin - R : bin;
    const int32_t v = in ? khist[bin] : 0;
    int32_t is = v, ic = (v > 0);
#pragma unroll
    for (int o = 1; o < 64; o <<= 1) {
      const int32_t a1 = __shfl_up(is, o), c1 = __shfl_up(ic, o);
      if (lane >= o) { is += a1; ic += c1; }
    }
    __syncthreads();
    if (lane == 63) { s_ws[wv] = is; s_wc[wv] = ic; }
    __syncthreads();
    int32_t wb = 0, wc = 0, rt = 0, rc = 0;
    for (int w = 0; w < SCAN_T / 64; w++) {
      if (w < wv) { wb += s_ws[w]; wc += s_wc[w]; }
      rt += s_ws[w]; rc += s_wc[w];
    }
    if (in) {
      khist[bin] = 0;
      kcount[i] = run + wb + is - v;
      krank[i] = rk + wc + ic - (v > 0);
    }
    run += rt; rk += rc;
  }
}

__device__ __forceinline__ bool corr_ring_index(int64_t v64, uint32_t mod, uint32_t magic, uint32_t limit, uint32_t& q) {
  q = (uint32_t)v64;
  const bool small = (uint32_t)(v64 >> 32) == 0u && q < 0x80000000u;
  if (mod > 1u) {
    const int32_t r = (int32_t)(q - __umulhi(q, magic) * mod);
    q = (uint32_t)(r < 0 ? r + (int32_t)mod : r);
  } else if (mod == 1u) {
    q = 0u;
  }
  return small && q < limit;
}

__global__ __launch_bounds__(256) void graph_fill_kernel(const int64_t* __restrict__ kk, int32_t E,
                                                         const int32_t* __restrict__ meta,
                                                         const int32_t* __restrict__ kcount, int32_t* kcursor,
                                                         const int32_t* __restrict__ krank,
                                                         int32_t* __restrict__ koff_u, int64_t* __restrict__ kx,
                                                         int32_t* __restrict__ ku, int32_t* __restrict__ pcsr_tmp,
                                                         const int64_t* __restrict__ jj,
                                                         const int32_t* __restrict__ ocnt, int nblk_hist,
                                                         int32_t* __restrict__ order, const CorrStream cs,
                                                         uint32_t* __restrict__ crec) {
  const bool do_order = order && nblk_hist == (int)gridDim.x;
  __shared__ int s_pos[ORD_BINS];
  const int t_first = blockIdx.x * blockDim.x + threadIdx.x;
  const int64_t kk_first = t_first < E ? kk[t_first] : 0;
  const int64_t jj_first = t_first < E ? jj[t_first] : 0;
  const int err = meta[GM_ERROR];
  const int krange = meta[GM_KRANGE], kmin = meta[GM_KMIN];
  int d_first = 0, p_first = 0, kc_first = 0, kr_first = 0;
  const int flane = threadIdx.x & 63;
  if (!err) {
    d_first = t_first < E ? (int)kk_first - kmin : 0;
    p_first = (E > cdv::GRAPH_WIDE_EDGES) ? cdv::group_atomic_add(kcursor, d_first, t_first < E, flane)
                                          : cdv::run_atomic_add(kcursor, d_first, t_first < E, flane);
    if (t_first < E) {
      kc_first = kcount[d_first];
      kr_first = krank[d_first];
    }
  }
  if (do_order) {
    __shared__ int s_tot[32][ORD_BINS + 1], s_pre[32][ORD_BINS + 1];
    const int tid = threadIdx.x, bq = tid & 7, part = tid >> 3;
    int tot[4] = {0, 0, 0, 0}, pre[4] = {0, 0, 0, 0};
    const int4* tab = reinterpret_cast<const int4*>(ocnt);
    for (int b0 = part; b0 < nblk_hist; b0 += 32 * 4) {
      int4 c[4];
#pragma unroll
      for (int u = 0; u < 4; u++) {
        const int b = b0 + 32 * u;
        c[u] = (b < nblk_hist) ? tab[b * (ORD_BINS / 4) + bq] : int4{0, 0, 0, 0};
      }
#pragma unroll
      for (int u = 0; u < 4; u++) {
        const bool before = b0 + 32 * u < (int)blockIdx.x;
        tot[0] += c[u].x; tot[1] += c[u].y; tot[2] += c[u].z; tot[3] += c[u].w;
        pre[0] += before ? c[u].x : 0; pre[1] += before ? c[u].y : 0; pre[2] += before ? c[u].z : 0; pre[3] += before ? c[u].w : 0;
      }
    }
#pragma unroll
    for (int q = 0; q < 4; q++) { s_tot[part][4 * bq + q] = tot[q]; s_pre[part][4 * bq + q] = pre[q]; }
    __syncthreads();
    if (tid < ORD_BINS) {
      int t = 0, p = 0;
#pragma unroll
      for (int q = 0; q < 32; q++) { t += s_tot[q][tid]; p += s_pre[q][tid]; }
      int incl = t;
#pragma unroll
      for (int o = 1; o < ORD_BINS; o <<= 1) {
        const int up = __shfl_up(incl, o);
        if (tid >= o) incl += up;
      }
      s_pos[tid] = incl - t + p;
    }
    __syncthreads();
    for (int e = t_first; e < E; e += gridDim.x * blockDim.x) {
      const int64_t j64 = e == t_first ? jj_first : jj[e];
      const int b = (int)j64 & (ORD_BINS - 1);
      const int pos = atomicAdd(&s_pos[b], 1);
      order[pos] = e;
      if (cs.coords) {
        const int64_t k64 = e == t_first ? kk_first : kk[e];
        uint32_t kq, jq;
        const bool ok = corr_ring_index(k64, cs.kmod, cs.kmagic, cs.Ng, kq) & corr_ring_index(j64, cs.jmod, cs.jmagic, cs.slots, jq);
        const float2* c2 = reinterpret_cast<const float2*>(cs.coords + (size_t)e * 18);
        uint32_t* r = crec + (size_t)pos * CORR_REC_WORDS;
        float2 c[9];
#pragma unroll
        for (int i = 0; i < 9; i++) c[i] = c2[i];
        typedef uint32_t u32x4 __attribute__((ext_vector_type(4)));
        const auto bits = [](float f) { return (uint32_t)__float_as_int(f); };
        u32x4* r4 = reinterpret_cast<u32x4*>(r);
        r4[0] = u32x4{bits(c[0].x), bits(c[0].y), bits(c[1].x), bits(c[1].y)};
        r4[1] = u32x4{bits(c[2].x), bits(c[2].y), bits(c[3].x), bits(c[3].y)};
        r4[2] = u32x4{bits(c[4].x), bits(c[4].y), bits(c[5].x), bits(c[5].y)};
        r4[3] = u32x4{bits(c[6].x), bits(c[6].y), bits(c[7].x), bits(c[7].y)};
        r4[4] = u32x4{bits(c[8].x), bits(c[8].y), (uint32_t)e, ok ? kq : 0xFFFFFFFFu};
        const auto fl = [&](float v) { return (int)fminf(fmaxf(floorf(v * cs.inv_scale0), -30000.f), 30000.f); };
        int xlo = 30000, xhi = -30000, ylo = 30000, yhi = -30000;
#pragma unroll
        for (int i = 0; i < 18; i++) {
          const int v = fl((i & 1) ? c[i >> 1].y : c[i >> 1].x);
          if (i < 9) { xlo = min(xlo, v); xhi = max(xhi, v); } else { ylo = min(ylo, v); yhi = max(yhi, v); }
        }
        const uint32_t bxw = ((uint32_t)xhi << 16) | ((uint32_t)xlo & 0xffffu);
        const uint32_t byw = ((uint32_t)yhi << 16) | ((uint32_t)ylo & 0xffffu);
        r4[5] = u32x4{ok ? jq : 0xFFFFFFFFu, bxw, byw, 0u};
      }
    }
  }
  if (err) return;
  const int n = max(E, krange + 1);
  for (int t = blockIdx.x * blockDim.x + threadIdx.x; t - flane < n; t += gridDim.x * blockDim.x) {
    const bool first = t == t_first;
    int p_run = 0;
    if (!first) p_run = (E > cdv::GRAPH_WIDE_EDGES) ? cdv::group_atomic_add(kcursor, t < E ? (int)kk[t] - kmin : 0, t < E, flane)
                                                    : cdv::run_atomic_add(kcursor, t < E ? (int)kk[t] - kmin : 0, t < E, flane);
    if (t <= krange) {
      if (t == krange) {
        koff_u[meta[GM_U]] = kcount[krange];
      } else if (kcount[t + 1] > kcount[t]) {
        const int r = krank[t];
        kx[r] = (int64_t)(kmin + t);
        koff_u[r] = kcount[t];
      }
    }
    if (t < E) {
      const int d = first ? d_first : (int)kk[t] - kmin;
      const int jt = first ? (int)jj_first : (int)jj[t];
      const int p = first ? p_first : p_run;
      *reinterpret_cast<int4*>(pcsr_tmp + 4 * (size_t)((first ? kc_first : kcount[d]) + p)) = make_int4(t, jt, d, 0);
      ku[t] = first ? kr_first : krank[d];
    }
  }
}

__global__ __launch_bounds__(256) void graph_segsort_kernel(const int64_t* __restrict__ ii,
                                                            const int64_t* __restrict__ jj,
                                                            const int64_t* __restrict__ kk, int32_t E,
                                                            int32_t* __restrict__ meta,
                                                            const int32_t* __restrict__ kcount,
                                                            const int32_t* __restrict__ pcsr_tmp,
                                                            int32_t* __restrict__ pcsr, int32_t* __restrict__ prec,
                                                            int32_t* __restrict__ pell, int ell_chunks,
                                                            const int32_t* __restrict__ krank,
                                                            int32_t* __restrict__ nprev,
                                                            int32_t* __restrict__ nnext, int32_t* __restrict__ kcursor,
                                                            int64_t* __restrict__ ix, int64_t* __restrict__ jx) {
  if (meta[GM_ERROR]) {
    if (ix)
      for (int e = blockIdx.x * blockDim.x + threadIdx.x; e < E; e += gridDim.x * blockDim.x) { ix[e] = -1; jx[e] = -1; }
    return;
  }
  if (blockIdx.x == 0 && threadIdx.x == 0) { meta[GM_HAS_II] = ii ? 1 : 0; meta[GM_MODE] = 0; }
  const int krange = meta[GM_KRANGE];
  for (int t = blockIdx.x * blockDim.x + threadIdx.x; t <= krange; t += gridDim.x * blockDim.x)
    kcursor[t] = 0;
  for (int p = blockIdx.x * blockDim.x + threadIdx.x; p < E; p += gridDim.x * blockDim.x) {
    const int4 me = *reinterpret_cast<const int4*>(pcsr_tmp + 4 * (size_t)p);
    const int e = me.x, d = me.z;
    const int lo = kcount[d], hi = kcount[d + 1];
    const uint64_t ke = ((uint64_t)(uint32_t)me.y << 32) | (uint32_t)e;
    int r = 0;
    uint64_t pk = 0, nk = ~(uint64_t)0;
    constexpr int SU = 16;
    for (int s0 = lo; s0 < hi; s0 += SU) {
      uint64_t ko[SU];
#pragma unroll
      for (int u = 0; u < SU; u++) {
        const int2 o = *reinterpret_cast<const int2*>(pcsr_tmp + 4 * (size_t)min(s0 + u, hi - 1));
        ko[u] = ((uint64_t)(uint32_t)o.y << 32) | (uint32_t)o.x;
      }
#pragma unroll
      for (int u = 0; u < SU; u++) {
        const bool in = s0 + u < hi;
        const bool below = in && ko[u] < ke, above = in && ko[u] > ke;
        r += below;
        pk = (below && (ko[u] >= pk)) ? ko[u] : pk;
        nk = (above && (ko[u] <= nk)) ? ko[u] : nk;
      }
    }
    const bool hasp = r > 0, hasn = lo + r + 1 < hi;
    const int pe = hasp ? (int)(uint32_t)pk : -1, ne = hasn ? (int)(uint32_t)nk : -1;
    pcsr[lo + r] = e;
    const int4 record = make_int4(e, ii ? (int)ii[e] : -1, (int)(ke >> 32), 0);
    *reinterpret_cast<int4*>(prec + 4 * (size_t)(lo + r)) = record;
    const int u = krank[d];
    if (r < ELL_SLOTS && (u >> 4) < ell_chunks)
      *reinterpret_cast<int4*>(pell + 4 * ((size_t)((u >> 4) * ELL_SLOTS + r) * 16 + (u & 15))) = record;
    nprev[e] = pe;
    nnext[e] = ne;
    if (ix) {
      ix[e] = (int64_t)pe;
      jx[e] = (int64_t)ne;
    }
  }
}

__global__ __launch_bounds__(256) void graph_neighbors_kernel(int32_t E, const int32_t* __restrict__ meta,
                                                              const int32_t* __restrict__ nprev,
                                                              const int32_t* __restrict__ nnext,
                                                              int64_t* __restrict__ ix, int64_t* __restrict__ jx) {
  const bool bad = graph_error(meta) != 0;
  for (int e = blockIdx.x * blockDim.x + threadIdx.x; e < E; e += gridDim.x * blockDim.x) {
    if (bad) { ix[e] = -1; jx[e] = -1; continue; }
    ix[e] = (int64_t)nprev[e];
    jx[e] = (int64_t)nnext[e];
  }
}

__global__ __launch_bounds__(256) void graph_copy_unique_kernel(const int32_t* __restrict__ meta,
                                                                const int64_t* __restrict__ kx_src,
                                                                const int32_t* __restrict__ ku_src,
                                                                int64_t* __restrict__ kx, int64_t kx_cap,
                                                                int64_t* __restrict__ ku, int32_t E) {
  if (meta[GM_ERROR]) return;
  const int U = meta[GM_U];
  const int n = max(U, E);
  for (int t = blockIdx.x * blockDim.x + threadIdx.x; t < n; t += gridDim.x * blockDim.x) {
    if (kx && t < U && t < kx_cap) kx[t] = kx_src[t];
    if (ku && t < E) ku[t] = (int64_t)ku_src[t];
  }
}

struct TSortArgs {
  int32_t* meta;
  int32_t R, E;
  int32_t *tcur, *tdeg, *tplo, *tkid, *tlive, *ttab, *tovf, *tprec;
  unsigned long long* town;
  int32_t *nprev, *nnext;
  int64_t *ix, *jx;
  int n_patch_wg;
  const int32_t* ocnt;
  int nblk_edges;
  int32_t* order;
  const int64_t *ii, *jj, *kk;
  CorrStream cs;
  uint32_t* crec;
  const float *poses, *patches, *intr;
  float* coords_out;
  const int32_t* dyn;
};

constexpr int TS_OVF_MAX = TAB_MAX_DEG;

typedef int cdv_i4 __attribute__((ext_vector_type(4)));

__device__ __forceinline__ size_t tab_index(int slot, int t) {
  return 4 * ((size_t)((slot >> 4) * ELL_SLOTS + t) * 16 + (slot & 15));
}

__device__ __forceinline__ uint64_t rec_key(const cdv_i4& r) { return ((uint64_t)(uint32_t)r.z << 32) | (uint32_t)r.x; }

__device__ __forceinline__ void reproject_edge(const TSortArgs& A, int64_t ix, int64_t jx, int64_t kx, float (&cx)[9],
                                               float (&cy)[9]) {
  const float* __restrict__ poses = A.poses;
  const float* __restrict__ intr = A.intr;
  float G[7], t[3], q[4];
  tf_relative(poses, ix, jx, false, G, t, q);
  const cdv_float4 Ki = *reinterpret_cast<const cdv_float4*>(intr + 4 * ix);
  const cdv_float4 Kj = *reinterpret_cast<const cdv_float4*>(intr + 4 * jx);
  typedef float f4u __attribute__((ext_vector_type(4), aligned(4)));
  const float* pk = A.patches + kx * 27;
  float pv[28];
#pragma unroll
  for (int v = 0; v < 6; v++) {
    const f4u x4 = *reinterpret_cast<const f4u*>(pk + 4 * v);
    pv[4 * v] = x4[0]; pv[4 * v + 1] = x4[1]; pv[4 * v + 2] = x4[2]; pv[4 * v + 3] = x4[3];
  }
  pv[24] = pk[24]; pv[25] = pk[25]; pv[26] = pk[26];
#pragma unroll
  for (int a = 0; a < 9; a++) {
    float X1[4];
    tf_pixel(t, q, pv[a], pv[9 + a], pv[18 + a], Ki[0], Ki[1], Ki[2], Ki[3], Kj[0], Kj[1], Kj[2], Kj[3], cx[a], cy[a], X1);
  }
}

__global__ __launch_bounds__(256) void graph_tsort_kernel(const TSortArgs A_in) {
  TSortArgs A = A_in;
  if (A.dyn) A.E = min(A.dyn[CDV_DYN_E], A_in.E);
  const int tid = threadIdx.x, lane = tid & 63, wave = tid >> 6;
  CDV_IF_STAMPS(const int sslot = (int)blockIdx.x;)
  if (tid < 64) { CDV_STAMP_RT(graph, sslot, 0); CDV_STAMP(graph, sslot, 1); }
  const int gen = A.meta[GM_GEN], par = gen & 1;
  const bool terr = A.meta[GM_TERR + par] != 0;
  if ((int)blockIdx.x >= A.n_patch_wg) {
    const int bid = (int)blockIdx.x - A.n_patch_wg;
    const int nblk = A.nblk_edges;
    __shared__ int s_pos[ORD_BINS];
    __shared__ int s_tot[32][ORD_BINS + 1], s_pre[32][ORD_BINS + 1];
    __shared__ __attribute__((aligned(16))) float s_xy[256 * 18];
    const int bq = tid & 7, part = tid >> 3;
    const cdv_i4* tab = reinterpret_cast<const cdv_i4*>(A.ocnt);
    cdv_i4 c0[8];
#pragma unroll
    for (int u = 0; u < 8; u++) {
      const int b = part + 32 * u;
      c0[u] = (b < nblk) ? tab[b * (ORD_BINS / 4) + bq] : cdv_i4{0, 0, 0, 0};
    }
    const auto load_edge = [&](int e, bool in, float (&cx)[9], float (&cy)[9], int64_t& k64, int64_t& j64) {
      k64 = 0; j64 = 0;
      if (in) {
        k64 = A.kk[e]; j64 = A.jj[e];
        if (A.poses) {
          reproject_edge(A, A.ii[e], j64, k64, cx, cy);
#pragma unroll
          for (int a = 0; a < 9; a++) { s_xy[tid * 18 + a] = cx[a]; s_xy[tid * 18 + 9 + a] = cy[a]; }
        } else if (A.cs.coords && A.crec) {
          const float2* c2 = reinterpret_cast<const float2*>(A.cs.coords + (size_t)e * 18);
#pragma unroll
          for (int a = 0; a < 9; a++) {
            const float2 v = c2[a];
            if (2 * a < 9) cx[2 * a] = v.x; else cy[2 * a - 9] = v.x;
            if (2 * a + 1 < 9) cx[2 * a + 1] = v.y; else cy[2 * a + 1 - 9] = v.y;
          }
        }
        if (terr && A.ix) { A.ix[e] = -1; A.jx[e] = -1; }
      }
    };
    float cx[9], cy[9];
    int64_t k64 = 0, j64 = 0;
    const int e_first = bid * 256;
    load_edge(e_first + tid, e_first + tid < A.E, cx, cy, k64, j64);
    {
      int tot[4] = {0, 0, 0, 0}, pre[4] = {0, 0, 0, 0};
#pragma unroll
      for (int u = 0; u < 8; u++) {
        const bool before = part + 32 * u < bid;
#pragma unroll
        for (int q = 0; q < 4; q++) { tot[q] += c0[u][q]; pre[q] += before ? c0[u][q] : 0; }
      }
      for (int b0 = part + 32 * 8; b0 < nblk; b0 += 32 * 8) {
        cdv_i4 c[8];
#pragma unroll
        for (int u = 0; u < 8; u++) {
          const int b = b0 + 32 * u;
          c[u] = (b < nblk) ? tab[b * (ORD_BINS / 4) + bq] : cdv_i4{0, 0, 0, 0};
        }
#pragma unroll
        for (int u = 0; u < 8; u++) {
          const bool before = b0 + 32 * u < bid;
#pragma unroll
          for (int q = 0; q < 4; q++) { tot[q] += c[u][q]; pre[q] += before ? c[u][q] : 0; }
        }
      }
#pragma unroll
      for (int q = 0; q < 4; q++) { s_tot[part][4 * bq + q] = tot[q]; s_pre[part][4 * bq + q] = pre[q]; }
      __syncthreads();
      if (tid < ORD_BINS) {
        int t = 0, p = 0;
#pragma unroll
        for (int q = 0; q < 32; q++) { t += s_tot[q][tid]; p += s_pre[q][tid]; }
        int incl = t;
#pragma unroll
        for (int o = 1; o < ORD_BINS; o <<= 1) {
          const int up = __shfl_up(incl, o);
          if (tid >= o) incl += up;
        }
        s_pos[tid] = incl - t + p;
      }
      __syncthreads();
    }
    if (tid < 64) { CDV_STAMP(graph, sslot, 2); }
    for (int e0 = e_first; e0 < A.E; e0 += nblk * 256) {
      const int e = e0 + tid;
      const bool in = e < A.E;
      if (e0 != e_first) load_edge(e, in, cx, cy, k64, j64);
      if (A.poses) {
        __syncthreads();
        const int n_e = min(256, A.E - e0);
        cdv_float4* dst = reinterpret_cast<cdv_float4*>(A.coords_out + (size_t)e0 * 18);
        const cdv_float4* src = reinterpret_cast<const cdv_float4*>(s_xy);
        const int n4 = (n_e * 18) >> 2;
        for (int v = tid; v < n4; v += 256) dst[v] = src[v];
        if (tid == 0 && ((n_e * 18) & 3)) {
          A.coords_out[(size_t)e0 * 18 + 4 * n4] = s_xy[4 * n4];
          A.coords_out[(size_t)e0 * 18 + 4 * n4 + 1] = s_xy[4 * n4 + 1];
        }
      }
      if (in) {
        const int b = (int)j64 & (ORD_BINS - 1);
        const int pos = atomicAdd(&s_pos[b], 1);
        A.order[pos] = e;
        if (A.crec) {
          uint32_t kq, jq;
          const bool ok = corr_ring_index(k64, A.cs.kmod, A.cs.kmagic, A.cs.Ng, kq) &
                          corr_ring_index(j64, A.cs.jmod, A.cs.jmagic, A.cs.slots, jq);
          const auto bits = [](float f) { return (uint32_t)__float_as_int(f); };
          const auto fl = [&](float v) { return (int)fminf(fmaxf(floorf(v * A.cs.inv_scale0), -30000.f), 30000.f); };
          int xlo = 30000, xhi = -30000, ylo = 30000, yhi = -30000;
#pragma unroll
          for (int a = 0; a < 9; a++) {
            const int vx = fl(cx[a]), vy = fl(cy[a]);
            xlo = min(xlo, vx); xhi = max(xhi, vx); ylo = min(ylo, vy); yhi = max(yhi, vy);
          }
          typedef uint32_t u32x4 __attribute__((ext_vector_type(4)));
          u32x4* r4 = reinterpret_cast<u32x4*>(A.crec + (size_t)pos * CORR_REC_WORDS);
          r4[0] = u32x4{bits(cx[0]), bits(cx[1]), bits(cx[2]), bits(cx[3])};
          r4[1] = u32x4{bits(cx[4]), bits(cx[5]), bits(cx[6]), bits(cx[7])};
          r4[2] = u32x4{bits(cx[8]), bits(cy[0]), bits(cy[1]), bits(cy[2])};
          r4[3] = u32x4{bits(cy[3]), bits(cy[4]), bits(cy[5]), bits(cy[6])};
          r4[4] = u32x4{bits(cy[7]), bits(cy[8]), (uint32_t)e, ok ? kq : 0xFFFFFFFFu};
          r4[5] = u32x4{ok ? jq : 0xFFFFFFFFu, ((uint32_t)xhi << 16) | ((uint32_t)xlo & 0xffffu),
                        ((uint32_t)yhi << 16) | ((uint32_t)ylo & 0xffffu), 0u};
        }
      }
      if (A.poses) __syncthreads();
    }
    if (tid < 64) { CDV_STAMP(graph, sslot, 3); CDV_STAMP_RT(graph, sslot, 15); }
    return;
  }
  const int h = tid >> 5, hl = tid & 31;
  const int slot = 8 * (int)blockIdx.x + h;
  const bool in_tab = slot < A.R;
  const int cs = in_tab ? slot : 0;
  const int deg_raw = A.tcur[cs];
  cdv_i4 rec = *reinterpret_cast<const cdv_i4*>(A.ttab + tab_index(cs, hl));
  __shared__ uint64_t s_key[8][32];
  __shared__ int s_e[8][32];
  __shared__ int s_flag[8];
  __shared__ cdv_i4 s_orec[TS_OVF_MAX];
  __shared__ uint64_t s_okey[TS_OVF_MAX];
  __shared__ int s_osort[TS_OVF_MAX], s_ocnt;
  if (blockIdx.x == 0 && tid == 0) {
    A.meta[GM_OVFN + (par ^ 1)] = 0;
    A.meta[GM_TERR + (par ^ 1)] = 0;
    A.meta[GM_GENNEXT] = (int)((unsigned)gen + 1u);
  }
  const int deg = in_tab ? deg_raw : 0;
  const int d32 = min(deg, ELL_SLOTS);
  const int k0 = __shfl(rec.w, lane & 32);
  const bool clash = hl < d32 && rec.w != k0;
  if (__ballot(clash) != 0ull && lane == 0) A.meta[GM_TERR + par] = 1;
  if (in_tab && hl == 0) {
    A.tdeg[slot] = min(deg, TS_OVF_MAX);
    A.tplo[slot] = 0;
    A.tkid[slot] = deg > 0 ? k0 : -1;
    if (deg > 0) { A.tcur[slot] = 0; A.town[slot] = 0ull; }
    s_flag[h] = deg > 0 ? 1 : 0;
  } else if (hl == 0) {
    s_flag[h] = 0;
  }
  if (tid < 64) { CDV_STAMP(graph, sslot, 2); }
  if (deg > 0 && deg <= ELL_SLOTS) {
    const uint64_t key = hl < deg ? rec_key(rec) : ~0ull;
    s_key[h][hl] = key;
    asm volatile("s_waitcnt lgkmcnt(0)" ::: "memory");
    __builtin_amdgcn_wave_barrier();
    int rank = 0;
    for (int u = 0; u < deg; u++) rank += (s_key[h][u] < key) ? 1 : 0;
    if (hl < deg) s_e[h][rank] = rec.x;
    asm volatile("s_waitcnt lgkmcnt(0)" ::: "memory");
    __builtin_amdgcn_wave_barrier();
    if (hl < deg) {
      *reinterpret_cast<cdv_i4*>(A.ttab + tab_index(slot, rank)) = rec;
      const int pe = rank > 0 ? s_e[h][rank - 1] : -1, ne = rank + 1 < deg ? s_e[h][rank + 1] : -1;
      A.nprev[rec.x] = pe;
      A.nnext[rec.x] = ne;
      if (A.ix && !terr) { A.ix[rec.x] = (int64_t)pe; A.jx[rec.x] = (int64_t)ne; }
    }
  }
  __syncthreads();
  if (tid == 0) {
    int n = 0;
#pragma unroll
    for (int u = 0; u < 8; u++) n += s_flag[u];
    A.tlive[blockIdx.x] = n;
  }
  __shared__ int s_deg8[8];
  if (hl == 0) s_deg8[h] = deg;
  __syncthreads();
  if (tid < 64) { CDV_STAMP(graph, sslot, 3); CDV_STAMP_RT(graph, sslot, 15); }
  if (wave != 0) return;
  bool any_ovf = false;
#pragma unroll
  for (int u = 0; u < 8; u++) any_ovf |= s_deg8[u] > ELL_SLOTS;
  if (!any_ovf) return;
  const int n_ovf = A.meta[GM_OVFN + par];
  for (int hs = 0; hs < 8; hs++) {
    const int sdeg = s_deg8[hs], oslot = 8 * (int)blockIdx.x + hs;
    if (sdeg <= ELL_SLOTS) continue;
    if (sdeg > TS_OVF_MAX) {
      if (lane == 0) A.meta[GM_TERR + par] = 1;
      continue;
    }
    if (lane < ELL_SLOTS) s_orec[lane] = *reinterpret_cast<const cdv_i4*>(A.ttab + tab_index(oslot, lane));
    if (lane == 0) s_ocnt = ELL_SLOTS;
    asm volatile("s_waitcnt lgkmcnt(0)" ::: "memory");
    __builtin_amdgcn_wave_barrier();
    const int okid = s_orec[0].w;
    const float rinv = 1.0f / (float)A.R;
    for (int u = lane; u < n_ovf; u += 64) {
      const cdv_i4 r = *reinterpret_cast<const cdv_i4*>(A.tovf + 4 * (size_t)u);
      int q = (int)((float)r.w * rinv);
      int rs = r.w - q * A.R;
      rs = (rs < 0) ? rs + A.R : rs;
      rs = (rs >= A.R) ? rs - A.R : rs;
      if (rs == oslot) {
        if (r.w != okid) A.meta[GM_TERR + par] = 1;
        const int idx = atomicAdd(&s_ocnt, 1);
        if (idx < TS_OVF_MAX) s_orec[idx] = r;
      }
    }
    asm volatile("s_waitcnt lgkmcnt(0)" ::: "memory");
    __builtin_amdgcn_wave_barrier();
    const int total = min(s_ocnt, TS_OVF_MAX);
    for (int x = lane; x < total; x += 64) s_okey[x] = rec_key(s_orec[x]);
    asm volatile("s_waitcnt lgkmcnt(0)" ::: "memory");
    __builtin_amdgcn_wave_barrier();
    for (int x = lane; x < total; x += 64) {
      const uint64_t key = s_okey[x];
      int rank = 0;
      for (int y = 0; y < total; y++) rank += (s_okey[y] < key) ? 1 : 0;
      s_osort[rank] = x;
    }
    int plo = 0;
    if (lane == 0) plo = atomicAdd(&A.meta[GM_PRECN], total);
    plo = __shfl(plo, 0);
    asm volatile("s_waitcnt lgkmcnt(0)" ::: "memory");
    __builtin_amdgcn_wave_barrier();
    for (int x = lane; x < total; x += 64) {
      const cdv_i4 r = s_orec[s_osort[x]];
      *reinterpret_cast<cdv_i4*>(A.tprec + 4 * (size_t)(plo + x)) = r;
      if (x < ELL_SLOTS) *reinterpret_cast<cdv_i4*>(A.ttab + tab_index(oslot, x)) = r;
      const int pe = x > 0 ? s_orec[s_osort[x - 1]].x : -1, ne = x + 1 < total ? s_orec[s_osort[x + 1]].x : -1;
      A.nprev[r.x] = pe;
      A.nnext[r.x] = ne;
      if (A.ix && !terr) { A.ix[r.x] = (int64_t)pe; A.jx[r.x] = (int64_t)ne; }
    }
    if (lane == 0) A.tplo[oslot] = plo;
    asm volatile("s_waitcnt lgkmcnt(0)" ::: "memory");
    __builtin_amdgcn_wave_barrier();
  }
}

__global__ __launch_bounds__(256) void graph_tfill_kernel(cdv::TFillArgs a) {
  cdv::graph_tfill_body(a, (int)blockIdx.x, (int)gridDim.x, (int)blockDim.x, (int)threadIdx.x);
}

inline int grid_for(int64_t n, int threads, int cap) {
  const int b = cdv_div_up(n > 0 ? n : 1, threads);
  return b < cap ? b : cap;
}

}

bool cdv_graph_lookup(const void* ws, GraphLayout* out) {
  std::lock_guard<std::mutex> lk(g_reg_mutex);
  auto it = g_registry.find(ws);
  if (it == g_registry.end()) return false;
  *out = it->second.L;
  return true;
}

bool cdv_graph_has_ii(const void* ws) {
  std::lock_guard<std::mutex> lk(g_reg_mutex);
  auto it = g_registry.find(ws);
  return it != g_registry.end() && it->second.has_ii;
}

void cdv_graph_forget(const void* ws) {
  std::lock_guard<std::mutex> lk(g_reg_mutex);
  g_registry.erase(ws);
  g_no_order.erase(ws);
}

extern "C" int cdv_graph_workspace_init(void* ws, size_t ws_bytes, int64_t E_max, int64_t k_range, void* stream) {
  CDV_REQUIRE(ws != nullptr, CDV_ERR_ARG, "cdv_graph_workspace_init: workspace is NULL");
  CDV_REQUIRE_ALIGNED(ws, 16, "cdv_graph_workspace_init: workspace must be 16-byte aligned");
  CDV_REQUIRE(k_range >= 1 && k_range < ((int64_t)1 << 31) - 64 && E_max >= 1, CDV_ERR_ARG, "cdv_graph_workspace_init: bad sizes");
  const GraphLayout L = graph_layout(E_max, k_range);
  CDV_REQUIRE(L.total <= ws_bytes, CDV_ERR_WORKSPACE, "cdv_graph_workspace_init: workspace too small for (E_max, k_range)");
  const GraphView v = graph_view(ws, L);
  hipLaunchKernelGGL(graph_init_kernel, dim3(grid_for(k_range + 1 + GM_WORDS, 256, 2048)), dim3(256), 0, (hipStream_t)stream,
                     v.meta, v.khist, v.kcursor, v.tcur, v.town, k_range);
  CDV_LAUNCH_CHECK();
  std::lock_guard<std::mutex> lk(g_reg_mutex);
  g_registry[ws] = RegEntry{L, true, false, CorrStream{nullptr, 0, 0, 0, 0, 0, 0, 1.0f}, false, 0};
  return CDV_OK;
}

extern "C" size_t cdv_graph_workspace_bytes(int64_t E_max, int64_t k_range) {
  if (E_max < 1) E_max = 1;
  if (k_range < 1) k_range = 1;
  return graph_layout(E_max, k_range).total;
}

extern "C" int cdv_graph_build(const int64_t* jj, const int64_t* kk, int64_t E, void* ws, size_t ws_bytes,
                               int64_t E_max, int64_t k_range, void* stream) {
  return cdv_graph_build_edges(nullptr, jj, kk, E, ws, ws_bytes, E_max, k_range, nullptr, nullptr, stream);
}

int cdv_graph_prepare(const int64_t* jj, const int64_t* kk, int64_t E, void* ws, size_t ws_bytes, int64_t E_max,
                      int64_t k_range, int64_t* ix, int64_t* jx, void* stream, cdv::HistArgs* hist, int* hist_blocks) {
  (void)jj; (void)kk;
  CDV_REQUIRE((ix == nullptr) == (jx == nullptr), CDV_ERR_ARG, "cdv_graph_build_edges: give both ix and jx or neither");
  CDV_REQUIRE(ws != nullptr, CDV_ERR_ARG, "cdv_graph_build: workspace is NULL");
  CDV_REQUIRE_ALIGNED(ws, 16, "cdv_graph_build: workspace must be 16-byte aligned");
  CDV_REQUIRE(E >= 0 && E < (int64_t)1 << 31, CDV_ERR_ARG, "cdv_graph_build: E out of range");
  CDV_REQUIRE(k_range >= 1 && E_max >= 1 && E <= E_max, CDV_ERR_ARG,
              "cdv_graph_build: need 1 <= E <= E_max, k_range >= 1");
  const GraphLayout L = graph_layout(E_max, k_range);
  CDV_REQUIRE(L.total <= ws_bytes, CDV_ERR_WORKSPACE, "cdv_graph_build: workspace too small for (E_max, k_range)");
  bool need_init;
  {
    std::lock_guard<std::mutex> lk(g_reg_mutex);
    auto it = g_registry.find(ws);
    need_init = it == g_registry.end() || !it->second.initialised || it->second.L.E_max != E_max ||
                it->second.L.k_range != k_range;
    const CorrStream keep = it != g_registry.end() ? it->second.cs : CorrStream{nullptr, 0, 0, 0, 0, 0, 0, 1.0f};
    g_registry[ws] = RegEntry{L, true, false, keep, false, 0};
  }
  const GraphView v = graph_view(ws, L);
  if (need_init)
    hipLaunchKernelGGL(graph_init_kernel, dim3(grid_for(k_range + 1 + GM_WORDS, 256, 2048)), dim3(256), 0,
                       (hipStream_t)stream, v.meta, v.khist, v.kcursor, v.tcur, v.town, k_range);
  *hist = cdv::HistArgs{jj, kk, (int32_t)E, v.stage, v.khist, (int32_t)k_range, v.meta, v.kcount, v.krank, v.ocnt};
  *hist_blocks = E > 0 ? grid_for(E, 256, GRAPH_MAX_BLOCKS) : 0;
  return CDV_OK;
}

int cdv_graph_finish(const int64_t* ii, const int64_t* jj, const int64_t* kk, int64_t E, void* ws, int64_t E_max,
                     int64_t k_range, int hist_blocks, int64_t* ix, int64_t* jx, void* stream) {
  const GraphLayout L = graph_layout(E_max, k_range);
  const GraphView v = graph_view(ws, L);
  CorrStream cs{nullptr, 0, 0, 0, 0, 0, 0, 1.0f};
  bool want_order = true;
  {
    std::lock_guard<std::mutex> lk(g_reg_mutex);
    auto it = g_registry.find(ws);
    if (it != g_registry.end()) {
      it->second.has_ii = ii != nullptr && E > 0;
      cs = it->second.cs;
    }
    want_order = g_no_order.find(ws) == g_no_order.end();
  }
  hipStream_t s = (hipStream_t)stream;
  const int32_t En = (int32_t)E;
  const int tb = 256;
  const int fb = grid_for(E, tb, GRAPH_MAX_BLOCKS);
  if (E > cdv::GRAPH_WIDE_EDGES) {
    hipLaunchKernelGGL(graph_scan_part_kernel, dim3(SCAN_WG), dim3(SCAN_T), 0, s, v.stage, hist_blocks, v.khist, v.ku, En, k_range);
    hipLaunchKernelGGL(graph_scan_apply_kernel, dim3(SCAN_WG), dim3(SCAN_T), 0, s, v.meta, v.stage, hist_blocks, v.khist, v.kcount,
                       v.krank, v.ku, En, k_range);
  } else if (hist_blocks == 0) {
    hipLaunchKernelGGL(graph_scan_kernel, dim3(1), dim3(1024), 0, s, v.meta, v.stage, hist_blocks, v.khist, v.kcount,
                       v.krank, En, k_range);
  }
  if (E > 0) {
    hipLaunchKernelGGL(graph_fill_kernel, dim3(fb), dim3(tb), 0, s, kk, En, v.meta, v.kcount, v.kcursor, v.krank,
                       v.koff_u, v.kx, v.ku, v.pcsr_tmp, jj, v.ocnt, hist_blocks, want_order ? v.order : nullptr, cs, v.crec);
    hipLaunchKernelGGL(graph_segsort_kernel, dim3(fb), dim3(tb), 0, s, ii, jj, kk, En, v.meta, v.kcount, v.pcsr_tmp,
                       v.pcsr, v.prec, v.pell, (int)L.ell_chunks, v.krank, v.nprev, v.nnext, v.kcursor, ix, jx);
  }
  CDV_LAUNCH_CHECK();
  return CDV_OK;
}

void cdv_graph_no_corr_order(const void* ws) {
  std::lock_guard<std::mutex> lk(g_reg_mutex);
  g_no_order.insert(ws);
}

bool cdv_graph_is_table(const void* ws) {
  std::lock_guard<std::mutex> lk(g_reg_mutex);
  auto it = g_registry.find(ws);
  return it != g_registry.end() && it->second.table;
}

int64_t cdv_graph_table_capacity(const void* ws) {
  std::lock_guard<std::mutex> lk(g_reg_mutex);
  auto it = g_registry.find(ws);
  return (it != g_registry.end() && it->second.table) ? it->second.tab_cap : 0;
}

int cdv_graph_table_prepare(const int64_t* ii, const int64_t* jj, const int64_t* kk, int64_t E, void* ws, size_t ws_bytes,
                            int64_t E_max, int64_t k_range, int64_t tab_cap, int64_t* ix, int64_t* jx, void* stream,
                            cdv::TFillArgs* fill, int* fill_blocks, const int32_t* dyn) {
  CDV_REQUIRE((ix == nullptr) == (jx == nullptr), CDV_ERR_ARG, "cdv_graph_build_table: give both ix and jx or neither");
  CDV_REQUIRE(ws != nullptr, CDV_ERR_ARG, "cdv_graph_build_table: workspace is NULL");
  CDV_REQUIRE_ALIGNED(ws, 16, "cdv_graph_build_table: workspace must be 16-byte aligned");
  CDV_REQUIRE(E >= 0 && E < (int64_t)1 << 31, CDV_ERR_ARG, "cdv_graph_build_table: E out of range");
  CDV_REQUIRE(k_range >= 1 && k_range < ((int64_t)1 << 31) - 64 && E_max >= 1 && E <= E_max, CDV_ERR_ARG,
              "cdv_graph_build_table: need 1 <= E <= E_max, 1 <= k_range < 2^31");
  CDV_REQUIRE(tab_cap >= 1 && tab_cap <= k_range && tab_cap <= TAB_CAP_MAX, CDV_ERR_ARG,
              "cdv_graph_build_table: table capacity must lie in [1, min(k_range, 65536)]");
  const GraphLayout L = graph_layout(E_max, k_range);
  CDV_REQUIRE(L.total <= ws_bytes, CDV_ERR_WORKSPACE, "cdv_graph_build_table: workspace too small for (E_max, k_range)");
  bool need_init;
  {
    std::lock_guard<std::mutex> lk(g_reg_mutex);
    auto it = g_registry.find(ws);
    need_init = it == g_registry.end() || !it->second.initialised || it->second.L.E_max != E_max ||
                it->second.L.k_range != k_range;
    const CorrStream keep = it != g_registry.end() ? it->second.cs : CorrStream{nullptr, 0, 0, 0, 0, 0, 0, 1.0f};
    g_registry[ws] = RegEntry{L, true, ii != nullptr && E > 0, keep, true, (int32_t)tab_cap};
  }
  const GraphView v = graph_view(ws, L);
  if (need_init)
    hipLaunchKernelGGL(graph_init_kernel, dim3(grid_for(k_range + 1 + GM_WORDS, 256, 2048)), dim3(256), 0,
                       (hipStream_t)stream, v.meta, v.khist, v.kcursor, v.tcur, v.town, k_range);
  *fill = cdv::TFillArgs{ii, jj, kk, (int32_t)E, (int32_t)tab_cap, v.meta, v.tcur, v.town, v.ttab, v.tovf, v.tprec, v.ocnt, dyn};
  *fill_blocks = grid_for(E, 256, GRAPH_MAX_BLOCKS);
  return CDV_OK;
}

int cdv_graph_table_finish(const cdv::TFillArgs& fill, int fill_blocks, void* ws, int64_t E_max, int64_t k_range, int64_t* ix,
                           int64_t* jx, const float* poses, const float* patches, const float* intr, float* coords_out,
                           bool with_stream, void* stream) {
  const GraphLayout L = graph_layout(E_max, k_range);
  const GraphView v = graph_view(ws, L);
  CorrStream cs{nullptr, 0, 0, 0, 0, 0, 0, 1.0f};
  {
    std::lock_guard<std::mutex> lk(g_reg_mutex);
    auto it = g_registry.find(ws);
    if (it != g_registry.end()) cs = it->second.cs;
  }
  const bool stream_ok = with_stream && (poses != nullptr || cs.coords != nullptr);
  TSortArgs A;
  A.meta = v.meta; A.R = fill.R; A.E = fill.E; A.town = v.town;
  A.tcur = v.tcur; A.tdeg = v.tdeg; A.tplo = v.tplo; A.tkid = v.tkid; A.tlive = v.tlive; A.ttab = v.ttab; A.tovf = v.tovf;
  A.tprec = v.tprec;
  A.nprev = v.nprev; A.nnext = v.nnext; A.ix = ix; A.jx = jx;
  A.n_patch_wg = (fill.R + 7) / 8;
  A.ocnt = v.ocnt; A.nblk_edges = fill_blocks; A.order = v.order;
  A.ii = fill.ii; A.jj = fill.jj; A.kk = fill.kk;
  A.cs = cs; A.crec = stream_ok ? v.crec : nullptr;
  A.poses = poses; A.patches = patches; A.intr = intr; A.coords_out = coords_out;
  A.dyn = fill.dyn;
  const int n_edge_wg = fill.E > 0 ? fill_blocks : 0;
  hipLaunchKernelGGL(graph_tsort_kernel, dim3(A.n_patch_wg + n_edge_wg), dim3(256), 0, (hipStream_t)stream, A);
  CDV_LAUNCH_CHECK();
  return CDV_OK;
}

extern "C" int cdv_graph_build_table(const int64_t* ii, const int64_t* jj, const int64_t* kk, int64_t E, void* ws,
                                     size_t ws_bytes, int64_t E_max, int64_t k_range, int64_t table_capacity, int64_t* ix,
                                     int64_t* jx, void* stream) {
  cdv::TFillArgs f;
  int fb = 0;
  const int rc = cdv_graph_table_prepare(ii, jj, kk, E, ws, ws_bytes, E_max, k_range, table_capacity, ix, jx, stream, &f, &fb, nullptr);
  if (rc != CDV_OK) return rc;
  hipLaunchKernelGGL(graph_tfill_kernel, dim3(fb), dim3(256), 0, (hipStream_t)stream, f);
  return cdv_graph_table_finish(f, fb, ws, E_max, k_range, ix, jx, nullptr, nullptr, nullptr, nullptr, true, stream);
}

extern "C" int cdv_graph_table_offsets(int64_t E_max, int64_t k_range, int64_t* out) {
  CDV_REQUIRE(out != nullptr && E_max >= 1 && k_range >= 1, CDV_ERR_ARG, "cdv_graph_table_offsets: bad argument");
  const GraphLayout L = graph_layout(E_max, k_range);
  out[0] = (int64_t)L.tdeg; out[1] = (int64_t)L.tplo; out[2] = (int64_t)L.ttab; out[3] = (int64_t)L.tprec;
  out[4] = (int64_t)L.order; out[5] = (int64_t)L.crec; out[6] = (int64_t)L.tkid;
  return CDV_OK;
}

extern "C" int cdv_graph_build_edges(const int64_t* ii, const int64_t* jj, const int64_t* kk, int64_t E, void* ws,
                                     size_t ws_bytes, int64_t E_max, int64_t k_range, int64_t* ix, int64_t* jx,
                                     void* stream) {
  cdv::HistArgs h;
  int hb = 0;
  const int rc = cdv_graph_prepare(jj, kk, E, ws, ws_bytes, E_max, k_range, ix, jx, stream, &h, &hb);
  if (rc != CDV_OK) return rc;
  if (hb > 0) hipLaunchKernelGGL(graph_hist_kernel, dim3(hb), dim3(256), 0, (hipStream_t)stream, h);
  return cdv_graph_finish(ii, jj, kk, E, ws, E_max, k_range, hb, ix, jx, stream);
}

extern "C" const int32_t* cdv_graph_corr_order(const void* ws) {
  GraphLayout L;
  if (!cdv_graph_lookup(ws, &L)) return nullptr;
  return graph_view((void*)ws, L).order;
}

extern "C" int cdv_graph_bind_corr_stream(void* ws, const float* coords, int64_t kmod, int64_t jmod, int64_t Ng,
                                          int64_t slots, float scale0) {
  CDV_REQUIRE(scale0 > 0.f, CDV_ERR_ARG, "cdv_graph_bind_corr_stream: scale of level 0 must be positive");
  CDV_REQUIRE(ws != nullptr, CDV_ERR_ARG, "cdv_graph_bind_corr_stream: workspace is NULL");
  CDV_REQUIRE_ALIGNED(coords, 8, "cdv_graph_bind_corr_stream: coords must be 8-byte aligned");
  CDV_REQUIRE(kmod >= 0 && jmod >= 0 && kmod < ((int64_t)1 << 31) && jmod < ((int64_t)1 << 31) && Ng >= 0 &&
                  Ng < ((int64_t)1 << 31) && slots >= 0 && slots < ((int64_t)1 << 31),
              CDV_ERR_ARG, "cdv_graph_bind_corr_stream: moduli / ring sizes out of range");
  CorrStream cs{coords, (uint32_t)kmod, (uint32_t)jmod, 0u, 0u, (uint32_t)Ng, (uint32_t)slots, 1.0f / scale0};
  cs.kmagic = kmod > 1 ? (uint32_t)((((uint64_t)1 << 32) + (uint64_t)kmod - 1) / (uint64_t)kmod) : 0u;
  cs.jmagic = jmod > 1 ? (uint32_t)((((uint64_t)1 << 32) + (uint64_t)jmod - 1) / (uint64_t)jmod) : 0u;
  std::lock_guard<std::mutex> lk(g_reg_mutex);
  auto it = g_registry.find(ws);
  if (it == g_registry.end()) g_registry[ws] = RegEntry{GraphLayout{}, false, false, cs, false, 0};
  else it->second.cs = cs;
  return CDV_OK;
}

extern "C" const uint32_t* cdv_graph_corr_records(const void* ws) {
  GraphLayout L;
  if (!cdv_graph_lookup(ws, &L)) return nullptr;
  return graph_view((void*)ws, L).crec;
}

extern "C" int cdv_graph_read_meta_host(const void* ws, int64_t* meta_host, void* stream) {
  GraphLayout L;
  CDV_REQUIRE(cdv_graph_lookup(ws, &L), CDV_ERR_ARG, "cdv_graph_read_meta_host: workspace has no built graph");
  int32_t m[GM_WORDS];
  CDV_HIP_CHECK(hipMemcpyAsync(m, (const char*)ws + L.meta, sizeof(m), hipMemcpyDeviceToHost, (hipStream_t)stream));
  CDV_HIP_CHECK(hipStreamSynchronize((hipStream_t)stream));
  if (cdv_graph_is_table(ws)) {
    const int err = m[GM_TERR + (m[GM_GEN] & 1)] != 0;
    const int cap = (int)cdv_graph_table_capacity(ws);
    std::vector<int32_t> kid((size_t)(cap > 0 ? cap : 0));
    if (cap > 0) {
      CDV_HIP_CHECK(hipMemcpyAsync(kid.data(), (const char*)ws + L.tkid, sizeof(int32_t) * (size_t)cap, hipMemcpyDeviceToHost,
                                   (hipStream_t)stream));
      CDV_HIP_CHECK(hipStreamSynchronize((hipStream_t)stream));
    }
    int64_t U = 0, lo = 0x7fffffff, hi = -1;
    for (int32_t k : kid)
      if (k >= 0) { U++; lo = k < lo ? k : lo; hi = k > hi ? k : hi; }
    meta_host[0] = err ? 0 : U; meta_host[1] = 1; meta_host[2] = lo; meta_host[3] = hi;
    meta_host[4] = 0; meta_host[5] = 0; meta_host[6] = err; meta_host[7] = m[GM_E];
    return CDV_OK;
  }
  meta_host[0] = m[GM_U]; meta_host[1] = 0; meta_host[2] = m[GM_KMIN]; meta_host[3] = m[GM_KMAX];
  meta_host[4] = m[GM_JMIN]; meta_host[5] = m[GM_JMAX]; meta_host[6] = m[GM_ERROR]; meta_host[7] = m[GM_E];
  return CDV_OK;
}

extern "C" int cdv_graph_get_unique(const void* ws, int64_t* kx, int64_t kx_capacity, int64_t* ku, int64_t E,
                                    void* stream) {
  GraphLayout L;
  CDV_REQUIRE(cdv_graph_lookup(ws, &L), CDV_ERR_ARG, "cdv_graph_get_unique: workspace has no built graph");
  CDV_REQUIRE(!cdv_graph_is_table(ws), CDV_ERR_UNSUPPORTED,
              "cdv_graph_get_unique: the workspace holds a patch table (no ranks); build the ranked index (cdv_graph_build*)");
  if (E == 0) return CDV_OK;
  const GraphView v = graph_view((void*)ws, L);
  const int64_t n = E > kx_capacity ? E : kx_capacity;
  hipLaunchKernelGGL(graph_copy_unique_kernel, dim3(grid_for(n, 256, 1024)), dim3(256), 0, (hipStream_t)stream, v.meta,
                     v.kx, v.ku, kx, kx_capacity, ku, (int32_t)E);
  CDV_LAUNCH_CHECK();
  return CDV_OK;
}

extern "C" int cdv_neighbors(const void* ws, int64_t E, int64_t* ix, int64_t* jx, void* stream) {
  GraphLayout L;
  CDV_REQUIRE(cdv_graph_lookup(ws, &L), CDV_ERR_ARG, "cdv_neighbors: workspace has no built graph");
  if (E == 0) return CDV_OK;
  const GraphView v = graph_view((void*)ws, L);
  hipLaunchKernelGGL(graph_neighbors_kernel, dim3(grid_for(E, 256, 1024)), dim3(256), 0, (hipStream_t)stream,
                     (int32_t)E, v.meta, v.nprev, v.nnext, ix, jx);
  CDV_LAUNCH_CHECK();
  return CDV_OK;
}
```

cdv_slam_amd/csrc/prologue.hip:

```cpp
#include "cdv_common.h"
#include "cdv_graph.h"
#include "cdv_parts.h"

namespace {

__global__ __launch_bounds__(256) void update_prologue_kernel(cdv::IngestArgs ing, int n_ing, cdv::TfArgs tf, int n_tf,
                                                              cdv::HistArgs hist, int n_hist) {
  int b = (int)blockIdx.x;
  if (b < n_hist) {
    cdv::graph_hist_body(hist, b, n_hist, 256, (int)threadIdx.x);
    return;
  }
  b -= n_hist;
  if (b < n_ing) {
    cdv::ingest_body(ing, b, 256, (int)threadIdx.x);
    return;
  }
  b -= n_ing;
  cdv::transform_body<3>(tf, (int64_t)b * 256 + threadIdx.x);
}

__global__ __launch_bounds__(256) void update_prologue_table_kernel(cdv::IngestArgs ing, int n_ing, cdv::TFillArgs fill,
                                                                    int n_fill) {
  int b = (int)blockIdx.x;
  if (b < n_fill) {
    cdv::graph_tfill_body(fill, b, n_fill, 256, (int)threadIdx.x);
    return;
  }
  cdv::ingest_body(ing, b - n_fill, 256, (int)threadIdx.x);
}

}

static int prologue_table_impl(
    const void* fmap_chw, void* fmap1_nhwc, void* fmap2_nhwc, int slot, int C, int H, int W, const void* gmap_planar,
    void* gmap_pm, int64_t Ng, int64_t gmap_first, int64_t gmap_count, const float* poses, const float* patches,
    const float* intrinsics, const int64_t* ii, const int64_t* jj, const int64_t* kk, int64_t E, float* coords,
    void* graph_ws, size_t graph_ws_bytes, int64_t E_max, int64_t k_range, int64_t table_capacity, int64_t* ix, int64_t* jx,
    void* stream, const int32_t* dyn, int dyn_mem, int dyn_pmem) {
  CDV_REQUIRE(C % 8 == 0 && C > 0, CDV_ERR_ARG, "cdv_update_prologue_table: C must be a multiple of 8");
  CDV_REQUIRE(H % 4 == 0 && W % 4 == 0, CDV_ERR_ARG, "cdv_update_prologue_table: H and W must be multiples of 4");
  CDV_REQUIRE(slot >= 0, CDV_ERR_ARG, "cdv_update_prologue_table: slot");
  CDV_REQUIRE(fmap_chw && fmap1_nhwc && fmap2_nhwc && coords && poses && patches && intrinsics && ii, CDV_ERR_ARG,
              "cdv_update_prologue_table: NULL buffer");
  CDV_REQUIRE(((uintptr_t)coords & 15) == 0, CDV_ERR_ARG, "cdv_update_prologue_table: coords must be 16-byte aligned");
  CDV_REQUIRE(((uintptr_t)intrinsics & 15) == 0, CDV_ERR_ARG, "cdv_update_prologue_table: intrinsics must be 16-byte aligned");
  CDV_REQUIRE_ALIGNED(fmap1_nhwc, 16, "cdv_update_prologue_table: fmap1_nhwc must be 16-byte aligned");
  CDV_REQUIRE_ALIGNED(fmap2_nhwc, 16, "cdv_update_prologue_table: fmap2_nhwc must be 16-byte aligned");
  CDV_REQUIRE_ALIGNED(gmap_pm, 16, "cdv_update_prologue_table: gmap_pm must be 16-byte aligned");
  const bool do_g = gmap_planar != nullptr && gmap_pm != nullptr && gmap_count > 0;
  CDV_REQUIRE(!do_g || (gmap_first >= 0 && gmap_first + gmap_count <= Ng), CDV_ERR_ARG, "cdv_update_prologue_table: tile range");
  cdv::TFillArgs fill;
  int n_fill = 0;
  const int rc = cdv_graph_table_prepare(ii, jj, kk, E, graph_ws, graph_ws_bytes, E_max, k_range, table_capacity, ix, jx, stream,
                                         &fill, &n_fill, dyn);
  if (rc != CDV_OK) return rc;
  const int fblocks = cdv_div_up((int64_t)(H / 4) * (W / 4) * (C / 8) * 16, 256);
  const int gblocks = do_g ? cdv_div_up(gmap_count * 9 * (C / 8), 256) : 0;
  const cdv::IngestArgs ing{(const _Float16*)fmap_chw, (_Float16*)fmap1_nhwc, (_Float16*)fmap2_nhwc, nullptr, nullptr,
                            slot, C, H, W, (const _Float16*)gmap_planar, (_Float16*)gmap_pm, gmap_first, gmap_count,
                            fblocks, gblocks, dyn, dyn_mem, dyn_pmem};
  const int n_ing = fblocks + gblocks;
  hipLaunchKernelGGL(update_prologue_table_kernel, dim3(n_fill + n_ing), dim3(256), 0, (hipStream_t)stream, ing, n_ing, fill,
                     n_fill);
  CDV_LAUNCH_CHECK();
  return cdv_graph_table_finish(fill, n_fill, graph_ws, E_max, k_range, ix, jx, poses, patches, intrinsics, coords, true, stream);
}

extern "C" int cdv_update_prologue_table(
    const void* fmap_chw, void* fmap1_nhwc, void* fmap2_nhwc, int slot, int C, int H, int W, const void* gmap_planar,
    void* gmap_pm, int64_t Ng, int64_t gmap_first, int64_t gmap_count, const float* poses, const float* patches,
    const float* intrinsics, const int64_t* ii, const int64_t* jj, const int64_t* kk, int64_t E, float* coords,
    void* graph_ws, size_t graph_ws_bytes, int64_t E_max, int64_t k_range, int64_t table_capacity, int64_t* ix, int64_t* jx,
    void* stream) {
  return prologue_table_impl(fmap_chw, fmap1_nhwc, fmap2_nhwc, slot, C, H, W, gmap_planar, gmap_pm, Ng, gmap_first, gmap_count,
                             poses, patches, intrinsics, ii, jj, kk, E, coords, graph_ws, graph_ws_bytes, E_max, k_range,
                             table_capacity, ix, jx, stream, nullptr, 0, 0);
}

extern "C" int cdv_update_prologue_table_dyn(
    const void* fmap_chw, void* fmap1_nhwc, void* fmap2_nhwc, int mem, int pmem, int C, int H, int W, const void* gmap_planar,
    void* gmap_pm, int64_t Ng, int64_t tiles_per_frame, const float* poses, const float* patches, const float* intrinsics,
    const int64_t* ii, const int64_t* jj, const int64_t* kk, int64_t E_bound, const int32_t* dyn, float* coords, void* graph_ws,
    size_t graph_ws_bytes, int64_t E_max, int64_t k_range, int64_t table_capacity, void* stream) {
  CDV_REQUIRE(dyn != nullptr && mem >= 1 && pmem >= 1 && tiles_per_frame >= 1 && (int64_t)pmem * tiles_per_frame <= Ng, CDV_ERR_ARG,
              "cdv_update_prologue_table_dyn: dyn / ring sizes");
  CDV_REQUIRE(E_bound >= 1, CDV_ERR_ARG, "cdv_update_prologue_table_dyn: E_bound must be >= 1");
  return prologue_table_impl(fmap_chw, fmap1_nhwc, fmap2_nhwc, 0, C, H, W, gmap_planar, gmap_pm, Ng, 0, tiles_per_frame, poses,
                             patches, intrinsics, ii, jj, kk, E_bound, coords, graph_ws, graph_ws_bytes, E_max, k_range,
                             table_capacity, nullptr, nullptr, stream, dyn, mem, pmem);
}

extern "C" int cdv_update_prologue(
    const void* fmap_chw, void* fmap1_nhwc, void* fmap2_nhwc, int slot, int C, int H, int W, const void* gmap_planar,
    void* gmap_pm, int64_t Ng, int64_t gmap_first, int64_t gmap_count,
    const float* poses, const float* patches, const float* intrinsics, const int64_t* ii, const int64_t* jj,
    const int64_t* kk, int64_t E, int tf_flags, float* coords,
    void* graph_ws, size_t graph_ws_bytes, int64_t E_max, int64_t k_range, int64_t* ix, int64_t* jx, void* stream) {
  CDV_REQUIRE(C % 8 == 0 && C > 0, CDV_ERR_ARG, "cdv_update_prologue: C must be a multiple of 8");
  CDV_REQUIRE(H % 4 == 0 && W % 4 == 0, CDV_ERR_ARG, "cdv_update_prologue: H and W must be multiples of 4");
  CDV_REQUIRE(slot >= 0, CDV_ERR_ARG, "cdv_update_prologue: slot");
  CDV_REQUIRE(fmap_chw && fmap1_nhwc && fmap2_nhwc && coords, CDV_ERR_ARG, "cdv_update_prologue: NULL buffer");
  CDV_REQUIRE_ALIGNED(fmap1_nhwc, 16, "cdv_update_prologue: fmap1_nhwc must be 16-byte aligned");
  CDV_REQUIRE_ALIGNED(fmap2_nhwc, 16, "cdv_update_prologue: fmap2_nhwc must be 16-byte aligned");
  CDV_REQUIRE_ALIGNED(gmap_pm, 16, "cdv_update_prologue: gmap_pm must be 16-byte aligned");
  const bool do_g = gmap_planar != nullptr && gmap_pm != nullptr && gmap_count > 0;
  CDV_REQUIRE(!do_g || (gmap_first >= 0 && gmap_first + gmap_count <= Ng), CDV_ERR_ARG, "cdv_update_prologue: tile range");
  cdv::HistArgs hist;
  int n_hist = 0;
  const int rc = cdv_graph_prepare(jj, kk, E, graph_ws, graph_ws_bytes, E_max, k_range, ix, jx, stream, &hist, &n_hist);
  if (rc != CDV_OK) return rc;
  const int fblocks = cdv_div_up((int64_t)(H / 4) * (W / 4) * (C / 8) * 16, 256);
  const int gblocks = do_g ? cdv_div_up(gmap_count * 9 * (C / 8), 256) : 0;
  const cdv::IngestArgs ing{(const _Float16*)fmap_chw, (_Float16*)fmap1_nhwc, (_Float16*)fmap2_nhwc, nullptr, nullptr,
                            slot, C, H, W, (const _Float16*)gmap_planar, (_Float16*)gmap_pm, gmap_first, gmap_count,
                            fblocks, gblocks};
  const cdv::TfArgs tf{poses, patches, intrinsics, ii, jj, kk, E, tf_flags, coords, nullptr, nullptr, nullptr, nullptr,
                       nullptr};
  const int n_ing = fblocks + gblocks, n_tf = cdv_div_up(E, 256);
  hipLaunchKernelGGL(update_prologue_kernel, dim3(n_ing + n_tf + n_hist), dim3(256), 0, (hipStream_t)stream, ing, n_ing,
                     tf, n_tf, hist, n_hist);
  CDV_LAUNCH_CHECK();
  return cdv_graph_finish(ii, jj, kk, E, graph_ws, E_max, k_range, n_hist, ix, jx, stream);
}
```

cdv_slam_amd/ops.py:

```python
import ctypes
import os

import torch

from . import _lib

F16, F32, F64 = 0, 1, 2
_DT = {torch.float16: F16, torch.float32: F32, torch.float64: F64}
LIE_OPS = {"exp": 0, "log": 1, "inv": 2, "mul": 3, "adj": 4, "adjT": 5, "act": 6, "act4": 7, "matrix": 8}

DEFAULT_K_RANGE = 4096 * 96


try:
    _raw_stream, _raw_device = torch._C._cuda_getCurrentRawStream, torch._C._cuda_getDevice
except AttributeError:
    _raw_stream = _raw_device = None


def _stream():
    if _raw_stream is not None:
        return _raw_stream(_raw_device())
    return torch.cuda.current_stream().cuda_stream


_ENV_RAW = getattr(os.environ, "_data", None)
if not isinstance(_ENV_RAW, dict) or (len(_ENV_RAW) and not isinstance(next(iter(_ENV_RAW)), bytes)):
    _ENV_RAW = None


def _env(name, default):
    if _ENV_RAW is None:
        return os.environ.get(name, default)
    v = _ENV_RAW.get(name.encode())
    return default if v is None else v.decode()


def _p(t):
    return None if t is None else t.data_ptr()


def _ident(t):
    return (t.data_ptr(), t._version, t.shape, t.stride(), t.dtype)


def _place(t):
    return (t.data_ptr(), t.shape, t.stride(), t.dtype)


def touched(*ts):
    for t in ts:
        torch.autograd.graph.increment_version(t)


def _need_cuda(*ts):
    for t in ts:
        if t is not None and not t.is_cuda:
            raise RuntimeError("cdv_slam_amd: tensors must live on the GPU (HIP path only, no CPU fallback)")


def _sync_check():
    return _env("CDV_CHECK", "0") == "1"


def version():
    return _lib.load().cdv_version().decode()


_FAST_SYMS = ("cdv_shadows_sync", "cdv_corr_fused", "cdv_corr_level_checked_interleaved",
              "cdv_graph_build_table", "cdv_ba_workspace_bytes", "cdv_ba_forward", "cdv_transform")
_fast = None
_armed_pair = None
_armed_graph = None


def _fast_mod():
    global _fast
    if _fast is None:
        try:
            from . import _dropin_fast as m
            lib = _lib.load()
            m.bind({n: ctypes.cast(getattr(lib, n), ctypes.c_void_p).value for n in _FAST_SYMS})
            _fast = m
            import atexit
            atexit.register(_fast_release)
        except ImportError as e:
            import warnings
            warnings.warn("cdv_slam_amd: the compiled drop-in bookkeeping (_dropin_fast.so, `make -C cdv_slam_amd/csrc`) is not "
                          "available (%s); the Python bookkeeping serves every call" % e, RuntimeWarning)
            _fast = False
    return _fast


def _fast_release():
    if _fast:
        _fast.drop_pending()
        _fast.disarm_pair()
        _fast.disarm_graph()


def fast_lane_enabled():
    return _env("CDV_DROPIN_FAST", "1") != "0" and bool(_fast_mod())


def _disarm_pair():
    global _armed_pair
    if _armed_pair is None:
        return
    pairing, ea, eb, tiles = _armed_pair
    _armed_pair = None
    st = _fast.disarm_pair()
    pairing.fast_token = 0
    ea.pop("fast", None)
    eb.pop("fast", None)
    tiles.fast = False
    if st is not None:
        ea["version"], ea["parity"] = st["A_version"], st["A_parity"]
        eb["version"], eb["parity"] = st["B_version"], st["B_parity"]
        src = st["tiles_src"]
        tiles.src, tiles.ident = src, (src.data_ptr(), st["tiles_version"], src.shape, src.stride(), src.dtype)


def _disarm_graph(g=None):
    global _armed_graph
    if _armed_graph is None or (g is not None and _armed_graph[1] is not g):
        return
    g = _armed_graph[1]
    _armed_graph = None
    st = _fast.disarm_graph()
    g._key = g._nbr = None
    if st is not None and st["has_key"]:
        idn = lambda t, v: (t.data_ptr(), v, t.shape, t.stride(), t.dtype)
        jj, kk, ii = st["jj"], st["kk"], st["ii"]
        g._key = (idn(jj, st["jj_version"]), idn(kk, st["kk_version"]), None if ii is None else idn(ii, st["ii_version"]),
                  (jj, kk, ii), "table")
        g.E, g.is_table = kk.numel(), True
        if st["ix"] is not None:
            g._nbr = (st["ix"], st["jx"])



class GraphIndex:

    def __init__(self, device, E_cap=1 << 16, k_range=DEFAULT_K_RANGE, table_capacity=None):
        self.lib = _lib.load()
        self.device = device
        self.E_cap, self.k_range = 0, k_range
        self.table_capacity = min(k_range, 1 << 16, int(table_capacity)) if table_capacity else 0
        self.ws = None
        self._key = None
        self.E = 0
        self.is_table = False
        self.n_builds = 0
        self._events = None
        self._graph_events_seen = 0
        self._reserve(E_cap)

    @property
    def events(self):
        if self._events is None:
            self._events = EventBlock(self.device, "GraphIndex@%x" % id(self))
        return self._events

    def _reserve(self, E):
        if self.ws is not None and E <= self.E_cap:
            return
        _disarm_graph(self)
        self.E_cap = max(E, int(self.E_cap * 1.5), 1024)
        nbytes = self.lib.cdv_graph_workspace_bytes(self.E_cap, self.k_range)
        self.ws = torch.empty(nbytes, dtype=torch.uint8, device=self.device)
        self.ws_bytes = nbytes
        _lib.check(self.lib.cdv_graph_workspace_init(_p(self.ws), nbytes, self.E_cap, self.k_range, _stream()),
                   "cdv_graph_workspace_init")
        if getattr(self, "_stream_cfg", None) is not None:
            self.bind_corr_stream(*self._stream_cfg)
        self._key = None

    @staticmethod
    def _make_key(jj, kk, ii):
        return (_ident(jj), _ident(kk), None if ii is None else _ident(ii), (jj, kk, ii))

    def _same_key(self, key):
        k = self._key
        if k is None or k[0] != key[0] or k[1] != key[1]:
            return False
        if key[2] is None or k[2] is None:
            return True
        return k[2] == key[2]

    def corr_order_ptr(self):
        p = self.lib.cdv_graph_corr_order(_p(self.ws))
        return ctypes.c_void_p(p) if p else None

    def bind_corr_stream(self, coords, kmod, jmod, Ng, slots, scale0=1.0):
        if coords is not None:
            _need_cuda(coords)
            if coords.dtype != torch.float32 or not coords.is_contiguous():
                raise TypeError("bind_corr_stream: coords must be a contiguous float32 buffer")
        _lib.check(self.lib.cdv_graph_bind_corr_stream(_p(self.ws), _p(coords), int(kmod), int(jmod), int(Ng), int(slots), float(scale0)),
                   "cdv_graph_bind_corr_stream")
        self._stream_coords = coords
        self._stream_cfg = (coords, kmod, jmod, Ng, slots, scale0)

    def corr_records_ptr(self):
        p = self.lib.cdv_graph_corr_records(_p(self.ws))
        return ctypes.c_void_p(p) if p else None

    def build(self, jj, kk, force=False, with_neighbors=False, ii=None):
        _disarm_graph(self)
        _need_cuda(jj, kk)
        if jj.dtype != torch.int64 or kk.dtype != torch.int64:
            raise TypeError("index tensors must be int64")
        jj, kk = jj.contiguous(), kk.contiguous()
        if ii is not None:
            ii = ii.contiguous()
        key = self._make_key(jj, kk, ii)
        if not force and not self.is_table and self._same_key(key):
            return self
        E = kk.numel()
        if jj.numel() != E:
            raise ValueError("jj and kk must have the same length")
        self.is_table = False
        self._reserve(E)
        self._nbr = None
        if ii is not None:
            _need_cuda(ii)
            if ii.dtype != torch.int64 or ii.numel() != E:
                raise TypeError("ii must be int64 with one entry per edge")
        ix = jx = None
        if with_neighbors and E > 0:
            ix = torch.empty(E, dtype=torch.int64, device=self.device)
            jx = torch.empty(E, dtype=torch.int64, device=self.device)
            self._nbr = (ix, jx)
        rc = self.lib.cdv_graph_build_edges(_p(ii), _p(jj), _p(kk), E, _p(self.ws), self.ws_bytes, self.E_cap,
                                            self.k_range, _p(ix), _p(jx), _stream())
        _lib.check(rc, "cdv_graph_build_edges")
        self.n_builds += 1
        self._key = key
        self.E = E
        if _sync_check():
            self.meta()
        return self

    def index_for_ba(self, jj, kk, ii, N):
        _disarm_graph(self)
        if N > 32 or N < 1:
            return self.build(jj, kk, ii=ii)
        key = self._make_key(jj, kk, ii)
        if self._key is not None and self._same_key(key):
            return self
        return self.build_table(jj, kk, ii=ii) if (prefer_table() and self.table_capacity) else self.build(jj, kk, ii=ii)

    def build_table(self, jj, kk, ii=None, force=False, with_neighbors=False):
        _disarm_graph(self)
        _need_cuda(jj, kk)
        if not self.table_capacity:
            raise RuntimeError("GraphIndex.build_table: this workspace was created without a table capacity")
        if jj.dtype != torch.int64 or kk.dtype != torch.int64:
            raise TypeError("index tensors must be int64")
        jj, kk = jj.contiguous(), kk.contiguous()
        if ii is not None:
            ii = ii.contiguous()
        key = self._make_key(jj, kk, ii) + ("table",)
        if not force and self.is_table and self._same_key(key):
            return self
        E = kk.numel()
        if jj.numel() != E or (ii is not None and (ii.dtype != torch.int64 or ii.numel() != E)):
            raise ValueError("ii / jj / kk must be int64 tensors of one length")
        self._reserve(E)
        self._nbr = None
        ix = jx = None
        if with_neighbors and E > 0:
            ix = torch.empty(E, dtype=torch.int64, device=self.device)
            jx = torch.empty(E, dtype=torch.int64, device=self.device)
            self._nbr = (ix, jx)
        rc = self.lib.cdv_graph_build_table(_p(ii), _p(jj), _p(kk), E, _p(self.ws), self.ws_bytes, self.E_cap, self.k_range,
                                            self.table_capacity, _p(ix), _p(jx), _stream())
        _lib.check(rc, "cdv_graph_build_table")
        self.n_builds += 1
        self._key = key
        self.E = E
        self.is_table = True
        if _sync_check():
            self.meta()
        return self

    def table_arrays(self):
        off = (ctypes.c_int64 * 7)()
        _lib.check(self.lib.cdv_graph_table_offsets(self.E_cap, self.k_range, off), "cdv_graph_table_offsets")
        w32 = self.ws.view(torch.int32)
        o = [int(v) // 4 for v in off]
        R, chunks = self.table_capacity, (self.table_capacity + 15) // 16
        return (w32[o[0]:o[0] + R], w32[o[1]:o[1] + R], w32[o[2]:o[2] + chunks * 32 * 16 * 4].view(-1, 4),
                w32[o[3]:o[3] + (self.E_cap + 1) * 4].view(-1, 4), w32[o[4]:o[4] + self.E_cap],
                w32[o[5]:o[5] + self.E_cap * 24].view(-1, 24), w32[o[6]:o[6] + R])

    def meta(self):
        m = (ctypes.c_int64 * 8)()
        _lib.check(self.lib.cdv_graph_read_meta_host(_p(self.ws), m, _stream()), "cdv_graph_read_meta_host")
        m = list(m)
        if m[6]:
            raise _lib.CdvError("patch-graph index: patch-id range exceeds the workspace capacity "
                                "(k_range=%d; got k in [%d,%d])" % (self.k_range, m[2], m[3]))
        return m

    def neighbors(self):
        _disarm_graph(self)
        if getattr(self, "_nbr", None) is not None:
            return self._nbr
        ix = torch.empty(self.E, dtype=torch.int64, device=self.device)
        jx = torch.empty(self.E, dtype=torch.int64, device=self.device)
        _lib.check(self.lib.cdv_neighbors(_p(self.ws), self.E, _p(ix), _p(jx), _stream()), "cdv_neighbors")
        self._nbr = (ix, jx)
        return ix, jx

    def unique(self):
        _disarm_graph(self)
        if self.is_table:
            jj, kk, ii = self._key[3]
            self.build(jj, kk, force=True, ii=ii)
        U = self.meta()[0] if self.E else 0
        kx = torch.empty(U, dtype=torch.int64, device=self.device)
        ku = torch.empty(self.E, dtype=torch.int64, device=self.device)
        _lib.check(self.lib.cdv_graph_get_unique(_p(self.ws), _p(kx), U, _p(ku), self.E, _stream()),
                   "cdv_graph_get_unique")
        return kx, ku


def update_prologue(graph, fmap_chw, fmap1_nhwc, fmap2_nhwc, slot, gmap, gmap_pm, gmap_first, gmap_count, poses, patches,
                    intrinsics, ii, jj, kk, layout_e2pp=True, coords_out=None):
    lib = _lib.load()
    _need_cuda(fmap_chw, fmap1_nhwc, fmap2_nhwc, poses, patches, intrinsics, ii, jj, kk)
    C, H, W = fmap_chw.shape[-3:]
    E, P = kk.numel(), patches.shape[-1]
    if P != 3 or poses.dtype != torch.float32:
        raise TypeError("update_prologue: float32 state, 3x3 patches")
    dev = poses.device
    _disarm_graph(graph)
    graph._reserve(E)
    shape = (1, E, 2, P, P) if layout_e2pp else (1, E, P, P, 2)
    if coords_out is not None:
        coords = coords_out.view(-1)[: E * 2 * P * P].view(shape)
    else:
        coords = torch.empty(shape, dtype=torch.float32, device=dev)
    ix = torch.empty(E, dtype=torch.int64, device=dev)
    jx = torch.empty(E, dtype=torch.int64, device=dev)
    Ng = gmap.numel() // (C * 9) if gmap is not None else 0
    rc = lib.cdv_update_prologue(_p(fmap_chw.contiguous()), _p(fmap1_nhwc), _p(fmap2_nhwc), int(slot), C, H, W, _p(gmap),
                                 _p(gmap_pm), Ng, int(gmap_first), int(gmap_count), _p(poses), _p(patches),
                                 _p(intrinsics), _p(ii), _p(jj), _p(kk), E, 1 if layout_e2pp else 0, _p(coords),
                                 _p(graph.ws), graph.ws_bytes, graph.E_cap, graph.k_range, _p(ix), _p(jx), _stream())
    _lib.check(rc, "cdv_update_prologue")
    graph.n_builds += 1
    graph._key = graph._make_key(jj, kk, ii)
    graph.E = E
    graph.is_table = False
    graph._nbr = (ix, jx)
    return coords


def update_prologue_table(graph, fmap_chw, fmap1_nhwc, fmap2_nhwc, slot, gmap, gmap_pm, gmap_first, gmap_count, poses, patches,
                          intrinsics, ii, jj, kk, coords_out=None):
    lib = _lib.load()
    _need_cuda(fmap_chw, fmap1_nhwc, fmap2_nhwc, poses, patches, intrinsics, ii, jj, kk)
    C, H, W = fmap_chw.shape[-3:]
    E, P = kk.numel(), patches.shape[-1]
    if P != 3 or poses.dtype != torch.float32:
        raise TypeError("update_prologue_table: float32 state, 3x3 patches")
    dev = poses.device
    _disarm_graph(graph)
    graph._reserve(E)
    if coords_out is not None:
        coords = coords_out.view(-1)[: E * 18].view(1, E, 2, P, P)
    else:
        coords = torch.empty((1, E, 2, P, P), dtype=torch.float32, device=dev)
    ix = torch.empty(E, dtype=torch.int64, device=dev)
    jx = torch.empty(E, dtype=torch.int64, device=dev)
    Ng = gmap.numel() // (C * 9) if gmap is not None else 0
    rc = lib.cdv_update_prologue_table(_p(fmap_chw.contiguous()), _p(fmap1_nhwc), _p(fmap2_nhwc), int(slot), C, H, W, _p(gmap),
                                       _p(gmap_pm), Ng, int(gmap_first), int(gmap_count), _p(poses), _p(patches),
                                       _p(intrinsics), _p(ii), _p(jj), _p(kk), E, _p(coords), _p(graph.ws), graph.ws_bytes,
                                       graph.E_cap, graph.k_range, graph.table_capacity, _p(ix), _p(jx), _stream())
    _lib.check(rc, "cdv_update_prologue_table")
    graph.n_builds += 1
    graph._key = graph._make_key(jj, kk, ii) + ("table",)
    graph.E = E
    graph.is_table = True
    graph._nbr = (ix, jx)
    return coords


_graphs = {}


def prefer_table():
    return _env("CDV_INDEX", "table") != "ranked"


_table_capacity = None


def configure_table(capacity):
    global _table_capacity
    _table_capacity = int(capacity) if capacity else None
    _disarm_graph()
    _graphs.clear()


def table_capacity():
    if _table_capacity is not None:
        return _table_capacity
    env = _env("CDV_TABLE_CAPACITY", None)
    return int(env) if env else 0


def set_patch_capacity(n_patches):
    global DEFAULT_K_RANGE
    DEFAULT_K_RANGE = int(n_patches)
    _disarm_graph()
    _graphs.clear()


def _device_graph(dev, **kw):
    g = _graphs.get(dev)
    if g is None:
        g = _graphs[dev] = GraphIndex(dev, **({"k_range": DEFAULT_K_RANGE, "table_capacity": table_capacity()} | kw))
    return g


def _table_still_fits(g, dev=None):
    if not g.table_capacity or g._events is None:
        return
    n = g._events.counts()[3]
    if n > g._graph_events_seen:
        g._graph_events_seen = n
        import warnings
        warnings.warn("cdv_slam_amd: the patch table (capacity %d) did not hold the live patch ids -- one update was skipped; "
                      "falling back to the ranked index on %s from now on" % (g.table_capacity, g.device), RuntimeWarning, stacklevel=3)
        g.table_capacity = 0
        g._key = None


def graph_for(jj, kk, ii=None, **kw):
    g = _device_graph(kk.device, **kw)
    _disarm_graph(g)
    _table_still_fits(g)
    key = g._make_key(jj.contiguous(), kk.contiguous(), None if ii is None else ii.contiguous())
    if g._key is not None and g._same_key(key):
        return g
    if prefer_table() and g.table_capacity:
        return g.build_table(jj, kk, ii=ii, with_neighbors=True)
    return g.build(jj, kk, ii=ii, with_neighbors=True)


def neighbors(kk, jj):
    if kk.numel() == 0:
        e = torch.empty(0, dtype=torch.int64, device=kk.device)
        return e, e.clone()
    ag = _armed_graph
    if ag is not None and _env("CDV_DROPIN_FAST", "1") != "0" and prefer_table() and not _sync_check():
        r = _fast.neighbors(ag[0], kk, jj, _stream())
        if r is not None:
            if type(r) is int:
                _lib.check(r, "cdv_graph_build_table")
            ag[1].n_builds += r[2]
            return r[0], r[1]
    return graph_for(jj, kk).neighbors()



def transform(poses, patches, intrinsics, ii, jj, kk, layout_e2pp=False, valid=False, jacobian=False, tonly=False):
    lib = _lib.load()
    _need_cuda(poses, patches, intrinsics, ii, jj, kk)
    if poses.dtype != torch.float32:
        raise TypeError("cdv_transform is float32 (the reference state buffers are float32, patchgraph.py:28-32)")
    poses, patches, intrinsics = poses.contiguous(), patches.contiguous(), intrinsics.contiguous()
    ii, jj, kk = ii.contiguous(), jj.contiguous(), kk.contiguous()
    E, P = ii.numel(), patches.shape[-1]
    dev = poses.device
    shape = (1, E, 2, P, P) if layout_e2pp else (1, E, P, P, 2)
    coords = torch.empty(shape, dtype=torch.float32, device=dev)
    vpx = torch.empty((1, E, P, P), dtype=torch.float32, device=dev) if valid else None
    v = Ji = Jj = Jz = None
    if jacobian:
        v = torch.empty((1, E), dtype=torch.float32, device=dev)
        Ji = torch.empty((1, E, 2, 6), dtype=torch.float32, device=dev)
        Jj = torch.empty((1, E, 2, 6), dtype=torch.float32, device=dev)
        Jz = torch.empty((1, E, 2, 1), dtype=torch.float32, device=dev)
    flags = (1 if layout_e2pp else 0) | (2 if tonly else 0)
    rc = lib.cdv_transform(_p(poses), _p(patches), _p(intrinsics), _p(ii), _p(jj), _p(kk), E, P, flags, _p(coords),
                           _p(vpx), _p(v), _p(Ji), _p(Jj), _p(Jz), _stream())
    _lib.check(rc, "cdv_transform")
    if jacobian:
        return coords, v, (Ji, Jj, Jz)
    if valid:
        return coords, vpx
    return coords


def fastba_reproject(poses, patches, intrinsics, ii, jj, kk):
    lib = _lib.load()
    _need_cuda(poses, patches, intrinsics, ii, jj, kk)
    poses, patches, intrinsics = poses.contiguous(), patches.contiguous(), intrinsics.contiguous()
    E, P = ii.numel(), patches.shape[-1]
    coords = torch.empty((1, E, 2, P, P), dtype=torch.float32, device=poses.device)
    rc = lib.cdv_fastba_reproject(_p(poses), _p(patches), _p(intrinsics), _p(ii.contiguous()), _p(jj.contiguous()),
                                  _p(kk.contiguous()), E, P, _p(coords), _stream())
    _lib.check(rc, "cdv_fastba_reproject")
    return coords



FMAP_PADX, FMAP_PADY = 16, 12


def alloc_fmap_ring(slots, C, H, W, device):
    return torch.zeros((slots, H + 2 * FMAP_PADY, W + 2 * FMAP_PADX, C), dtype=torch.float16, device=device)


def fmap_interior(ring):
    return ring[:, FMAP_PADY:-FMAP_PADY, FMAP_PADX:-FMAP_PADX, :]


class NhwcCache:

    def __init__(self, max_entries=4):
        self.entries = []
        self.max_entries = max_entries

    def get(self, fmap):
        place = _place(fmap)
        for ent in self.entries:
            if ent["place"] == place:
                if "fast" in ent:
                    _disarm_pair()
                if ent["version"] != fmap._version:
                    self._sync(ent)
                return ent["shadow"]
        C, H, W = fmap.shape[-3:]
        N = fmap.numel() // (C * H * W)
        lib = _lib.load()
        ent = {"src": fmap, "place": place, "version": None, "parity": 0,
               "shadow": torch.zeros(fmap.shape[:-3] + (H + 2 * FMAP_PADY, W + 2 * FMAP_PADX, C), dtype=fmap.dtype,
                                     device=fmap.device),
               "ws": torch.zeros(lib.cdv_fmap_sync_workspace_bytes(N), dtype=torch.uint8, device=fmap.device)}
        self._sync(ent)
        self.entries.append(ent)
        if len(self.entries) > self.max_entries:
            if "fast" in self.entries[0]:
                _disarm_pair()
            self.entries.pop(0)
        return ent["shadow"]

    def entry(self, fmap):
        place = _place(fmap)
        for ent in self.entries:
            if ent["place"] == place:
                return ent
        return None

    @staticmethod
    def _sync(ent):
        lib = _lib.load()
        fmap = ent["src"]
        C, H, W = fmap.shape[-3:]
        N = fmap.numel() // (C * H * W)
        _lib.check(lib.cdv_fmap_sync_nhwc(_p(fmap), _p(ent["shadow"]), N, C, H, W, _p(ent["ws"]), ent["parity"], _stream()),
                   "cdv_fmap_sync_nhwc")
        ent["parity"] ^= 1
        ent["version"] = fmap._version

    def converted_slots(self, fmap):
        place = _place(fmap)
        for ent in self.entries:
            if ent["place"] == place:
                return int(ent["ws"][-64:-60].view(torch.int32).item())
        return 0


_nhwc = NhwcCache()


class TileCache:

    def __init__(self):
        self.src, self.ident, self.shadow = None, None, None
        self.n_converted = 0
        self.fast = False

    def get(self, gmap):
        if self.fast:
            _disarm_pair()
        idn = _ident(gmap)
        if self.ident != idn or self.shadow is None:
            g = gmap[0] if gmap.dim() == 5 else gmap
            same_place = self.ident is not None and self.ident[0] == idn[0] and self.ident[2:] == idn[2:]
            self.shadow = gmap_to_pixel_major(g.contiguous(), out=self.shadow if (self.shadow is not None and same_place) else None)
            self.src, self.ident = gmap, idn
# ... 613 lines not shown
```

Measured before the change: 10370.

## Precompute correlation box descriptors in graph records for fused corr kernel

The graph-build kernels now compute per-edge box geometry for both pyramid levels (ring offsets, buffer ranges, fast/outside/do flags, sizes) and store it in correlation records widened from 24 to 32 words. The fused correlation kernel gains a descriptor mode that reads these words instead of rebuilding boxes and address arithmetic per edge, chosen when the registered level geometry matches the launch. The aim is less scalar and integer work on the corr critical path. In exchange the records are larger, so there is more memory traffic in both build and corr, and the host launch path adds a registry scan under a mutex.

```diff
diff --git a/cdv_slam_amd/csrc/cdv_corr_box.h b/cdv_slam_amd/csrc/cdv_corr_box.h
--- /dev/null
+++ b/cdv_slam_amd/csrc/cdv_corr_box.h
@@ -0,0 +1,69 @@
+#pragma once
+#include <stdint.h>
+
+#include "cdv_common.h"
+
+namespace cdv {
+
+constexpr int PADX = CDV_FMAP_PADX;
+constexpr int PADY = CDV_FMAP_PADY;
+constexpr int RAW_ROWS = 12;
+constexpr uint32_t FBIAS = 0x4B000000u;
+
+struct Box {
+  int x0, y0;
+  int Wb, Hb;
+  bool fast;
+  int stride;
+  bool outside;
+  int x0c, y0c;
+};
+
+__device__ __forceinline__ int floor_clamped(float v) {
+  return (int)fminf(fmaxf(floorf(v), -1.0e6f), 1.0e6f);
+}
+
+__device__ __forceinline__ Box make_box(int ixmin, int ixmax, int iymin, int iymax, int H, int W) {
+  Box b;
+  b.x0 = ixmin - 3;
+  b.y0 = iymin - 3;
+  b.Wb = ixmax + 4 - b.x0 + 1;
+  b.Hb = iymax + 4 - b.y0 + 1;
+  b.fast = (b.Wb <= 16) && (b.Hb <= RAW_ROWS);
+  b.stride = b.fast ? b.Wb : 16;
+  b.x0c = min(max(b.x0, -PADX), W);
+  b.y0c = min(max(b.y0, -PADY), H);
+  b.outside = (b.x0c != b.x0) || (b.y0c != b.y0);
+  return b;
+}
+
+constexpr uint32_t DESC_FAST = 1u << 24, DESC_OUTSIDE = 1u << 25, DESC_DO = 1u << 26;
+
+struct CorrLevelGeo {
+  int H, W;
+  uint32_t pitch;
+  uint32_t slot_bytes;
+};
+
+__host__ __device__ __forceinline__ CorrLevelGeo corr_level_geo(int C, int H, int W) {
+  const uint32_t pitch = (uint32_t)(W + 2 * PADX) * (uint32_t)C * 2u;
+  return CorrLevelGeo{H, W, pitch, pitch * (uint32_t)(H + 2 * PADY)};
+}
+
+__device__ __forceinline__ uint32_t box_ring_offset(const Box& b, uint32_t jq, const CorrLevelGeo& G, uint32_t CB) {
+  return jq * G.slot_bytes + (uint32_t)(b.y0c + PADY) * G.pitch + (uint32_t)(b.x0c + PADX) * CB;
+}
+
+__device__ __forceinline__ void box_desc_words(int ixmin, int ixmax, int iymin, int iymax, uint32_t jq, bool idx_ok,
+                                               const CorrLevelGeo& G, uint32_t CB, uint32_t (&w)[4]) {
+  const Box b = make_box(ixmin, ixmax, iymin, iymax, G.H, G.W);
+  const bool run = b.fast && !b.outside && idx_ok;
+  const uint32_t nq = b.fast ? (uint32_t)((b.Wb * b.Hb + 15) >> 4) : 0u;
+  w[0] = b.fast ? box_ring_offset(b, idx_ok ? jq : 0u, G, CB) : 0u;
+  w[1] = b.fast ? (uint32_t)b.Hb * G.pitch + FBIAS : 0u;
+  w[2] = (uint32_t)min(b.Wb, 255) | ((uint32_t)min(b.Hb, 255) << 8) | (nq << 16) | (b.fast ? DESC_FAST : 0u) |
+         (b.outside ? DESC_OUTSIDE : 0u) | (run ? DESC_DO : 0u);
+  w[3] = ((uint32_t)b.y0 << 16) | ((uint32_t)b.x0 & 0xffffu);
+}
+
+}
diff --git a/cdv_slam_amd/csrc/cdv_graph.h b/cdv_slam_amd/csrc/cdv_graph.h
--- a/cdv_slam_amd/csrc/cdv_graph.h
+++ b/cdv_slam_amd/csrc/cdv_graph.h
@@ -1,6 +1,8 @@
 #pragma once
 #include <stddef.h>
 #include <stdint.h>
+
+#include "cdv_corr_box.h"
 
 namespace cdv {
 
@@ -31,12 +33,20 @@
 constexpr int TAB_MAX_DEG = 128;
 constexpr int64_t TAB_CAP_MAX = 1 << 16;
 constexpr int ORD_BINS = 32;
-constexpr int CORR_REC_WORDS = 24;
+constexpr int CORR_REC_WORDS = 32;
+constexpr int CORR_REC_DESC = 23;
 
 struct CorrStream {
   const float* coords;
   uint32_t kmod, jmod, kmagic, jmagic, Ng, slots;
   float inv_scale0;
+  int have_levels;
+  int C, shift1;
+  CorrLevelGeo G0, G1;
+};
+
+struct CorrLevels {
+  int C, H0, W0, H1, W1, shift1;
 };
 
 struct GraphLayout {
@@ -138,6 +148,8 @@
 
 void cdv_graph_no_corr_order(const void* ws);
 
+bool cdv_graph_corr_stream_of(const void* records, cdv::CorrStream* out);
+
 bool cdv_graph_has_ii(const void* ws);
 
 bool cdv_graph_is_table(const void* ws);
@@ -160,10 +172,11 @@
                             cdv::TFillArgs* fill, int* fill_blocks, const int32_t* dyn = nullptr);
 int cdv_graph_table_finish(const cdv::TFillArgs& fill, int fill_blocks, void* ws, int64_t E_max, int64_t k_range, int64_t* ix,
                            int64_t* jx, const float* poses, const float* patches, const float* intr, float* coords_out,
-                           bool with_stream, void* stream);
+                           bool with_stream, void* stream, const cdv::CorrLevels* levels = nullptr);
 
 namespace cdv { struct HistArgs; }
 int cdv_graph_prepare(const int64_t* jj, const int64_t* kk, int64_t E, void* ws, size_t ws_bytes, int64_t E_max,
                       int64_t k_range, int64_t* ix, int64_t* jx, void* stream, cdv::HistArgs* hist, int* hist_blocks);
 int cdv_graph_finish(const int64_t* ii, const int64_t* jj, const int64_t* kk, int64_t E, void* ws, int64_t E_max,
-                     int64_t k_range, int hist_blocks, int64_t* ix, int64_t* jx, void* stream);
+                     int64_t k_range, int hist_blocks, int64_t* ix, int64_t* jx, void* stream,
+                     const cdv::CorrLevels* levels = nullptr);
diff --git a/cdv_slam_amd/csrc/corr.hip b/cdv_slam_amd/csrc/corr.hip
--- a/cdv_slam_amd/csrc/corr.hip
+++ b/cdv_slam_amd/csrc/corr.hip
@@ -2,6 +2,7 @@
 #include <stdlib.h>
 
 #include "cdv_common.h"
+#include "cdv_corr_box.h"
 #include "cdv_graph.h"
 #include "cdv_parts.h"
 
@@ -15,10 +16,8 @@
 
 namespace {
 
-constexpr int PADX = CDV_FMAP_PADX;
-constexpr int PADY = CDV_FMAP_PADY;
-
-constexpr int RAW_ROWS = 12;
+using cdv::PADX; using cdv::PADY; using cdv::RAW_ROWS; using cdv::FBIAS; using cdv::Box; using cdv::floor_clamped;
+
 constexpr int NQ_MAX = 8;
 constexpr int RAW_MSH = RAW_ROWS * 16 + 12;
 constexpr int RAW_HALFS = 9 * RAW_MSH;
@@ -69,31 +68,8 @@
   int shift;
 };
 
-struct Box {
-  int x0, y0;
-  int Wb, Hb;
-  bool fast;
-  int stride;
-  bool outside;
-  int x0c, y0c;
-};
-
-__device__ __forceinline__ int floor_clamped(float v) {
-  return (int)fminf(fmaxf(floorf(v), -1.0e6f), 1.0e6f);
-}
-
 __device__ __forceinline__ Box make_box(int ixmin, int ixmax, int iymin, int iymax, const LevelParams& LP) {
-  Box b;
-  b.x0 = ixmin - 3;
-  b.y0 = iymin - 3;
-  b.Wb = ixmax + 4 - b.x0 + 1;
-  b.Hb = iymax + 4 - b.y0 + 1;
-  b.fast = (b.Wb <= 16) && (b.Hb <= RAW_ROWS);
-  b.stride = b.fast ? b.Wb : 16;
-  b.x0c = min(max(b.x0, -PADX), LP.W);
-  b.y0c = min(max(b.y0, -PADY), LP.H);
-  b.outside = (b.x0c != b.x0) || (b.y0c != b.y0);
-  return b;
+  return cdv::make_box(ixmin, ixmax, iymin, iymax, LP.H, LP.W);
 }
 
 template <int KS>
@@ -382,8 +358,6 @@
   const int32_t* dynE;
 };
 
-constexpr uint32_t FBIAS = 0x4B000000u;
-
 __device__ __forceinline__ LevelParams level_params(const CorrLevel& L) {
   return LevelParams{reinterpret_cast<const _Float16*>(L.base_m + (size_t)FBIAS), L.H, L.W, L.inv_scale, L.shift};
 }
@@ -392,12 +366,25 @@
   int cval;
   float xb, yb;
   int ixmin, ixmax, iymin, iymax;
+  uint32_t d[8];
 };
 
-template <int CC, int NLEV, bool REC>
+__device__ __forceinline__ Box box_from_words(uint32_t w2, uint32_t w3) {
+  Box b;
+  b.x0 = (int)(short)(w3 & 0xffffu); b.y0 = (int)w3 >> 16;
+  b.Wb = (int)(w2 & 0xffu); b.Hb = (int)((w2 >> 8) & 0xffu);
+  b.fast = (w2 & cdv::DESC_FAST) != 0u;
+  b.stride = b.fast ? b.Wb : 16;
+  b.outside = (w2 & cdv::DESC_OUTSIDE) != 0u;
+  b.x0c = 0; b.y0c = 0;
+  return b;
+}
+
+template <int CC, int NLEV, int MODE>
 __device__ __forceinline__ void corr_edge(const CorrArgs2& a, int p, int e, const EdgeCoords& ec, uint32_t kq, uint32_t jq,
                                           bool idx_ok, int lane, _Float16* __restrict__ raw, _Float16* __restrict__ outT) {
   CDV_STAMP(corr, p, 0);
+  constexpr bool REC = MODE != 0, DESC = MODE == 2;
   const int C = CC ? CC : a.C;
 #ifdef CDV_STAMPS
   const int exp = a.exp;
@@ -446,9 +433,9 @@
     ixmin = __builtin_amdgcn_readfirstlane(vxmin); ixmax = __builtin_amdgcn_readfirstlane(vxmax);
     iymin = __builtin_amdgcn_readfirstlane(vymin); iymax = __builtin_amdgcn_readfirstlane(vymax);
   }
-  const Box b0 = make_box(ixmin, ixmax, iymin, iymax, L0);
   const int sh1 = NLEV == 2 ? L1.shift : 0;
-  const Box b1 = make_box(ixmin >> sh1, ixmax >> sh1, iymin >> sh1, iymax >> sh1, L1);
+  const Box b0 = DESC ? box_from_words(ec.d[2], ec.d[3]) : make_box(ixmin, ixmax, iymin, iymax, L0);
+  const Box b1 = DESC ? box_from_words(ec.d[6], ec.d[7]) : make_box(ixmin >> sh1, ixmax >> sh1, iymin >> sh1, iymax >> sh1, L1);
   CDV_STAMP(corr, p, 1);
 
   _Float16 res0[7], res1[7];
@@ -457,24 +444,26 @@
                                                              4 * ((n * (RAW_MSH / 2) + 2 * g) & 31));
 
   const unsigned CB = (unsigned)C * 2u;
-  const char* r0 = a.L0.base_m + (size_t)(jq * a.L0.slot_bytes + (unsigned)(b0.y0c + PADY) * a.L0.pitch +
-                                          (unsigned)(b0.x0c + PADX) * CB);
   const CorrLevel& A1 = NLEV == 2 ? a.L1 : a.L0;
-  const char* r1 = A1.base_m + (size_t)(jq * A1.slot_bytes + (unsigned)(b1.y0c + PADY) * A1.pitch +
-                                        (unsigned)(b1.x0c + PADX) * CB);
   const unsigned pitch0 = a.L0.pitch, pitch1 = A1.pitch;
+  const uint32_t off0 = DESC ? ec.d[0] : jq * a.L0.slot_bytes + (unsigned)(b0.y0c + PADY) * pitch0 + (unsigned)(b0.x0c + PADX) * CB;
+  const uint32_t off1 = DESC ? ec.d[4] : jq * A1.slot_bytes + (unsigned)(b1.y0c + PADY) * pitch1 + (unsigned)(b1.x0c + PADX) * CB;
+  const uint32_t range0 = DESC ? ec.d[1] : (unsigned)b0.Hb * pitch0 + FBIAS;
+  const uint32_t range1 = DESC ? ec.d[5] : (unsigned)b1.Hb * pitch1 + FBIAS;
+  const char* r0 = a.L0.base_m + (size_t)off0;
+  const char* r1 = A1.base_m + (size_t)off1;
   cdv_half8 w[NQ_MAX][1];
-  const bool do0 = b0.fast && !b0.outside && idx_ok;
-  const bool do1 = NLEV == 2 && b1.fast && !b1.outside && idx_ok;
-  const int nq0 = (b0.Wb * b0.Hb + 15) >> 4, nq1 = (b1.Wb * b1.Hb + 15) >> 4;
+  const bool do0 = DESC ? (ec.d[2] & cdv::DESC_DO) != 0u : b0.fast && !b0.outside && idx_ok;
+  const bool do1 = NLEV == 2 && (DESC ? (ec.d[6] & cdv::DESC_DO) != 0u : b1.fast && !b1.outside && idx_ok);
+  const int nq0 = DESC ? (int)((ec.d[2] >> 16) & 0xffu) : (b0.Wb * b0.Hb + 15) >> 4;
+  const int nq1 = DESC ? (int)((ec.d[6] >> 16) & 0xffu) : (b1.Wb * b1.Hb + 15) >> 4;
   typedef float cdv_f32x2 __attribute__((ext_vector_type(2)));
   const float nhalf = (float)n + 0.5f;
   const float lanebase = (8 * g < C) ? (float)((unsigned)n * CB + (unsigned)(8 * g) * 2u) + 8388608.0f : 33554432.0f;
   constexpr int NQF0 = 8, NQF1 = 6;
-#define CDV2_LOAD_SETUP(BX, RB, PITCH)                                                             \
+#define CDV2_LOAD_SETUP(BX, RB, PITCH, RANGE)                                                      \
     const unsigned Wb_ = (unsigned)(BX).Wb, pitch_ = (PITCH);                                      \
-    const auto rsrc_ = __builtin_amdgcn_make_buffer_rsrc(const_cast<char*>(RB), (short)0,          \
-                                                         (int)((unsigned)(BX).Hb * pitch_ + FBIAS), 0x00020000); \
+    const auto rsrc_ = __builtin_amdgcn_make_buffer_rsrc(const_cast<char*>(RB), (short)0, (int)(RANGE), 0x00020000); \
     const float invW_ = __builtin_amdgcn_rcpf((float)Wb_);                                         \
     const float wrapf_ = (float)(pitch_ - Wb_ * CB);                                               \
     const cdv_f32x2 dtb_ = {16.0f * invW_, (float)(16u * CB)};
@@ -485,9 +474,9 @@
       w[q][0] = __builtin_bit_cast(cdv_half8, v_);                                                 \
       tb_ += dtb_;                                                                                 \
     }
-#define CDV2_LOAD_FIXED(BX, RB, PITCH, NQF, NQ)                                                    \
+#define CDV2_LOAD_FIXED(BX, RB, PITCH, RANGE, NQF, NQ)                                             \
   {                                                                                                \
-    CDV2_LOAD_SETUP(BX, RB, PITCH)                                                                 \
+    CDV2_LOAD_SETUP(BX, RB, PITCH, RANGE)                                                               \
     cdv_f32x2 tb_ = {nhalf * invW_, lanebase};                                                     \
     CDV2_LD1(0) CDV2_LD1(1) CDV2_LD1(2) CDV2_LD1(3) CDV2_LD1(4)                                    \
     if (NQF > 6) { CDV2_LD1(5) CDV2_LD1(6) }                                                       \
@@ -507,9 +496,9 @@
     if (NQF > 6) { CDV2_MF2(4, 5) CDV2_MF1(w[6][0], 6) } else { CDV2_MF1(w[4][0], 4) }             \
     if ((NQ) >= (NQF)) { CDV2_MF1(w[NQF - 1][0], NQF - 1) }                                        \
   }
-#define CDV2_TAIL(BX, RB, PITCH, NQF, NQ)                                                          \
+#define CDV2_TAIL(BX, RB, PITCH, RANGE, NQF, NQ)                                                   \
   if ((NQ) > (NQF)) {                                                                              \
-    CDV2_LOAD_SETUP(BX, RB, PITCH)                                                                 \
+    CDV2_LOAD_SETUP(BX, RB, PITCH, RANGE)                                                               \
     cdv_f32x2 tb_ = {(nhalf + (float)(16 * (NQF))) * invW_, lanebase + (float)(16u * (unsigned)(NQF) * CB)}; \
     _Pragma("unroll 1") for (int q_ = (NQF); q_ < (NQ); q_++) {                                    \
       const float vf_ = __builtin_fmaf(__builtin_floorf(tb_[0]), wrapf_, tb_[1]);                  \
@@ -518,20 +507,20 @@
       CDV2_MF1(__builtin_bit_cast(cdv_half8, v_), q_)                                              \
     }                                                                                              \
   }
-  if (do0 && !CDV_EXP(1)) CDV2_LOAD_FIXED(b0, r0, pitch0, NQF0, nq0)
+  if (do0 && !CDV_EXP(1)) CDV2_LOAD_FIXED(b0, r0, pitch0, range0, NQF0, nq0)
   const BlendGeo g0 = blend_geo(xb, yb, bm, bxo, L0, b0, !b0.fast);
   const BlendGeo g1 = blend_geo(xb, yb, bm, bxo, L1, b1, !b1.fast);
   CDV_STAMP(corr, p, 2);
   if (do0 && !CDV_EXP(256)) {
     CDV2_MFMA_FIXED(NQF0, nq0)
-    CDV2_TAIL(b0, r0, pitch0, NQF0, nq0)
+    CDV2_TAIL(b0, r0, pitch0, range0, NQF0, nq0)
   } else if (!b0.fast && idx_ok) {
     slow_level<1, REC ? 7 : 1>(L0, jslot, xv, yv, pat, raw, lane, C);
   } else {
     zero_raw(raw, lane);
   }
   __builtin_amdgcn_sched_barrier(0);
-  if (do1 && !CDV_EXP(1)) CDV2_LOAD_FIXED(b1, r1, pitch1, NQF1, nq1)
+  if (do1 && !CDV_EXP(1)) CDV2_LOAD_FIXED(b1, r1, pitch1, range1, NQF1, nq1)
   wave_lds_sync();
   CDV_STAMP(corr, p, 3);
   if (!CDV_EXP(128)) blend_level(raw, g0, res0);
@@ -540,7 +529,7 @@
     wave_lds_sync();
     if (do1 && !CDV_EXP(256)) {
       CDV2_MFMA_FIXED(NQF1, nq1)
-      CDV2_TAIL(b1, r1, pitch1, NQF1, nq1)
+      CDV2_TAIL(b1, r1, pitch1, range1, NQF1, nq1)
     } else if (!b1.fast && idx_ok) {
       slow_level<1, REC ? 7 : 1>(L1, jslot, xv, yv, pat, raw, lane, C);
     } else {
@@ -613,7 +602,7 @@
   return small && q < limit;
 }
 
-template <int CC, int NLEV, bool REC = false>
+template <int CC, int NLEV, int MODE = 0>
 __global__ __launch_bounds__(64 * CW) void corr_fused2_kernel(const uint32_t* __restrict__ rec_h, const int32_t* __restrict__ dynE_h,
                                                           int E_h, int eighth_h, const CorrArgs2 a) {
   extern __shared__ __attribute__((aligned(16))) unsigned char smem_raw[];
@@ -621,6 +610,7 @@
   const int wave = __builtin_amdgcn_readfirstlane(threadIdx.x >> 6);
   _Float16* raw = reinterpret_cast<_Float16*>(smem_raw + (size_t)wave * WAVE_LDS2_BYTES);
   _Float16* outT = raw;
+  constexpr bool REC = MODE != 0;
   int E = E_h, eighth = eighth_h;
   if (REC && dynE_h) {
     E = min(__builtin_amdgcn_readfirstlane(*dynE_h), E_h);
@@ -638,10 +628,16 @@
     ec.yb = __int_as_float((int)r[9 + bm]);
     const int e = (int)r[18];
     const uint32_t kq = r[19], jq = r[20];
-    const int bx = (int)r[21], by = (int)r[22];
-    ec.ixmin = (int)(short)(bx & 0xffff); ec.ixmax = bx >> 16;
-    ec.iymin = (int)(short)(by & 0xffff); ec.iymax = by >> 16;
-    corr_edge<CC, NLEV, true>(a, p0, e, ec, kq, jq, jq != 0xFFFFFFFFu, lane, raw, outT);
+    if (MODE == 2) {
+      ec.ixmin = ec.ixmax = ec.iymin = ec.iymax = 0;
+#pragma unroll
+      for (int i = 0; i < 8; i++) ec.d[i] = r[cdv::CORR_REC_DESC + i];
+    } else {
+      const int bx = (int)r[21], by = (int)r[22];
+      ec.ixmin = (int)(short)(bx & 0xffff); ec.ixmax = bx >> 16;
+      ec.iymin = (int)(short)(by & 0xffff); ec.iymax = by >> 16;
+    }
+    corr_edge<CC, NLEV, MODE>(a, p0, e, ec, kq, jq, jq != 0xFFFFFFFFu, lane, raw, outT);
     return;
   }
   const int e = a.order ? __builtin_amdgcn_readfirstlane(a.order[p0]) : p0;
@@ -655,7 +651,7 @@
   const bool j_ok = ring_index(a.jj[e], a.jmod, a.jmagic, a.slots, jq);
   EdgeCoords ec;
   ec.cval = cval;
-  corr_edge<CC, NLEV, false>(a, p0, e, ec, kq, jq, k_ok && j_ok, lane, raw, outT);
+  corr_edge<CC, NLEV, 0>(a, p0, e, ec, kq, jq, k_ok && j_ok, lane, raw, outT);
 }
 
 template <typename T>
@@ -1179,8 +1175,15 @@
     const size_t smem2 = (size_t)CW * WAVE_LDS2_BYTES;
     if (rec) {
       CDV_REQUIRE(nlev == 2 && coords_ref == nullptr, CDV_ERR_UNSUPPORTED, "cdv_corr_fused_stream: two fused levels only");
-      if (C == 24) hipLaunchKernelGGL((corr_fused2_kernel<24, 2, true>), dim3(blocks), dim3(64 * CW), smem2, s, rec, dynE, (int)E, blocks >> 3, a);
-      else hipLaunchKernelGGL((corr_fused2_kernel<0, 2, true>), dim3(blocks), dim3(64 * CW), smem2, s, rec, dynE, (int)E, blocks >> 3, a);
+      cdv::CorrStream cs;
+      const bool desc = cdv_graph_corr_stream_of(rec, &cs) && cs.have_levels && cs.C == C && cs.slots == (uint32_t)slots &&
+                        cs.inv_scale0 == A0.inv_scale && cs.shift1 == a.L1.shift && cs.G0.H == H0 && cs.G0.W == W0 &&
+                        cs.G1.H == H1 && cs.G1.W == W1 && cs.G0.pitch == A0.pitch && cs.G0.slot_bytes == A0.slot_bytes &&
+                        cs.G1.pitch == a.L1.pitch && cs.G1.slot_bytes == a.L1.slot_bytes && exp == 0;
+      if (desc && C == 24) hipLaunchKernelGGL((corr_fused2_kernel<24, 2, 2>), dim3(blocks), dim3(64 * CW), smem2, s, rec, dynE, (int)E, blocks >> 3, a);
+      else if (desc) hipLaunchKernelGGL((corr_fused2_kernel<0, 2, 2>), dim3(blocks), dim3(64 * CW), smem2, s, rec, dynE, (int)E, blocks >> 3, a);
+      else if (C == 24) hipLaunchKernelGGL((corr_fused2_kernel<24, 2, 1>), dim3(blocks), dim3(64 * CW), smem2, s, rec, dynE, (int)E, blocks >> 3, a);
+      else hipLaunchKernelGGL((corr_fused2_kernel<0, 2, 1>), dim3(blocks), dim3(64 * CW), smem2, s, rec, dynE, (int)E, blocks >> 3, a);
     } else if (nlev == 2 && C == 24)
       hipLaunchKernelGGL((corr_fused2_kernel<24, 2>), dim3(blocks), dim3(64 * CW), smem2, s, rec, dynE, (int)E, blocks >> 3, a);
     else if (nlev == 2)
diff --git a/cdv_slam_amd/csrc/graph.hip b/cdv_slam_amd/csrc/graph.hip
--- a/cdv_slam_amd/csrc/graph.hip
+++ b/cdv_slam_amd/csrc/graph.hip
@@ -25,6 +25,26 @@
 std::unordered_map<const void*, RegEntry> g_registry;
 std::unordered_set<const void*> g_no_order;
 
+
+__device__ __forceinline__ void corr_rec_tail(uint32_t* __restrict__ r, const CorrStream& cs, uint32_t jq, bool ok, int xlo,
+                                              int xhi, int ylo, int yhi) {
+  typedef uint32_t u32x4 __attribute__((ext_vector_type(4)));
+  u32x4* r4 = reinterpret_cast<u32x4*>(r);
+  const uint32_t bxw = ((uint32_t)xhi << 16) | ((uint32_t)xlo & 0xffffu);
+  const uint32_t byw = ((uint32_t)yhi << 16) | ((uint32_t)ylo & 0xffffu);
+  if (!cs.have_levels) {
+    r4[5] = u32x4{ok ? jq : 0xFFFFFFFFu, bxw, byw, 0u};
+    return;
+  }
+  const uint32_t CB = (uint32_t)cs.C * 2u;
+  const int sh = cs.shift1;
+  uint32_t d0[4], d1[4];
+  box_desc_words(xlo, xhi, ylo, yhi, jq, ok, cs.G0, CB, d0);
+  box_desc_words(xlo >> sh, xhi >> sh, ylo >> sh, yhi >> sh, jq, ok, cs.G1, CB, d1);
+  r4[5] = u32x4{ok ? jq : 0xFFFFFFFFu, bxw, byw, d0[0]};
+  r4[6] = u32x4{d0[1], d0[2], d0[3], d1[0]};
+  r4[7] = u32x4{d1[1], d1[2], d1[3], 0u};
+}
 
 __global__ __launch_bounds__(256) void graph_init_kernel(int32_t* meta, int32_t* khist, int32_t* kcursor, int32_t* tcur,
                                                          unsigned long long* town, int64_t k_cap) {
@@ -276,9 +296,7 @@
           const int v = fl((i & 1) ? c[i >> 1].y : c[i >> 1].x);
           if (i < 9) { xlo = min(xlo, v); xhi = max(xhi, v); } else { ylo = min(ylo, v); yhi = max(yhi, v); }
         }
-        const uint32_t bxw = ((uint32_t)xhi << 16) | ((uint32_t)xlo & 0xffffu);
-        const uint32_t byw = ((uint32_t)yhi << 16) | ((uint32_t)ylo & 0xffffu);
-        r4[5] = u32x4{ok ? jq : 0xFFFFFFFFu, bxw, byw, 0u};
+        corr_rec_tail(r, cs, jq, ok, xlo, xhi, ylo, yhi);
       }
     }
   }
@@ -574,8 +592,7 @@
           r4[2] = u32x4{bits(cx[8]), bits(cy[0]), bits(cy[1]), bits(cy[2])};
           r4[3] = u32x4{bits(cy[3]), bits(cy[4]), bits(cy[5]), bits(cy[6])};
           r4[4] = u32x4{bits(cy[7]), bits(cy[8]), (uint32_t)e, ok ? kq : 0xFFFFFFFFu};
-          r4[5] = u32x4{ok ? jq : 0xFFFFFFFFu, ((uint32_t)xhi << 16) | ((uint32_t)xlo & 0xffffu),
-                        ((uint32_t)yhi << 16) | ((uint32_t)ylo & 0xffffu), 0u};
+          corr_rec_tail(A.crec + (size_t)pos * CORR_REC_WORDS, A.cs, jq, ok, xlo, xhi, ylo, yhi);
         }
       }
       if (A.poses) __syncthreads();
@@ -724,6 +741,25 @@
   if (it == g_registry.end()) return false;
   *out = it->second.L;
   return true;
+}
+
+bool cdv_graph_corr_stream_of(const void* records, CorrStream* out) {
+  std::lock_guard<std::mutex> lk(g_reg_mutex);
+  for (const auto& kv : g_registry) {
+    if (!kv.second.initialised || (const char*)kv.first + kv.second.L.crec != (const char*)records) continue;
+    *out = kv.second.cs;
+    return true;
+  }
+  return false;
+}
+
+static void corr_stream_set_levels(CorrStream& cs, const CorrLevels* lv, bool records_written) {
+  cs.have_levels = 0;
+  if (!lv || !records_written) return;
+  cs.have_levels = 1;
+  cs.C = lv->C; cs.shift1 = lv->shift1;
+  cs.G0 = corr_level_geo(lv->C, lv->H0, lv->W0);
+  cs.G1 = corr_level_geo(lv->C, lv->H1, lv->W1);
 }
 
 bool cdv_graph_has_ii(const void* ws) {
@@ -794,19 +830,20 @@
 }
 
 int cdv_graph_finish(const int64_t* ii, const int64_t* jj, const int64_t* kk, int64_t E, void* ws, int64_t E_max,
-                     int64_t k_range, int hist_blocks, int64_t* ix, int64_t* jx, void* stream) {
+                     int64_t k_range, int hist_blocks, int64_t* ix, int64_t* jx, void* stream, const CorrLevels* levels) {
   const GraphLayout L = graph_layout(E_max, k_range);
   const GraphView v = graph_view(ws, L);
   CorrStream cs{nullptr, 0, 0, 0, 0, 0, 0, 1.0f};
   bool want_order = true;
   {
     std::lock_guard<std::mutex> lk(g_reg_mutex);
+    want_order = g_no_order.find(ws) == g_no_order.end();
     auto it = g_registry.find(ws);
     if (it != g_registry.end()) {
       it->second.has_ii = ii != nullptr && E > 0;
+      corr_stream_set_levels(it->second.cs, levels, it->second.cs.coords != nullptr && want_order);
       cs = it->second.cs;
     }
-    want_order = g_no_order.find(ws) == g_no_order.end();
   }
   hipStream_t s = (hipStream_t)stream;
   const int32_t En = (int32_t)E;
@@ -880,14 +917,17 @@
 
 int cdv_graph_table_finish(const cdv::TFillArgs& fill, int fill_blocks, void* ws, int64_t E_max, int64_t k_range, int64_t* ix,
                            int64_t* jx, const float* poses, const float* patches, const float* intr, float* coords_out,
-                           bool with_stream, void* stream) {
+                           bool with_stream, void* stream, const CorrLevels* levels) {
   const GraphLayout L = graph_layout(E_max, k_range);
   const GraphView v = graph_view(ws, L);
   CorrStream cs{nullptr, 0, 0, 0, 0, 0, 0, 1.0f};
   {
     std::lock_guard<std::mutex> lk(g_reg_mutex);
     auto it = g_registry.find(ws);
-    if (it != g_registry.end()) cs = it->second.cs;
+    if (it != g_registry.end()) {
+      corr_stream_set_levels(it->second.cs, levels, with_stream && (poses != nullptr || it->second.cs.coords != nullptr));
+      cs = it->second.cs;
+    }
   }
   const bool stream_ok = with_stream && (poses != nullptr || cs.coords != nullptr);
   TSortArgs A;
diff --git a/cdv_slam_amd/csrc/prologue.hip b/cdv_slam_amd/csrc/prologue.hip
--- a/cdv_slam_amd/csrc/prologue.hip
+++ b/cdv_slam_amd/csrc/prologue.hip
@@ -64,7 +64,8 @@
   hipLaunchKernelGGL(update_prologue_table_kernel, dim3(n_fill + n_ing), dim3(256), 0, (hipStream_t)stream, ing, n_ing, fill,
                      n_fill);
   CDV_LAUNCH_CHECK();
-  return cdv_graph_table_finish(fill, n_fill, graph_ws, E_max, k_range, ix, jx, poses, patches, intrinsics, coords, true, stream);
+  const cdv::CorrLevels lv{C, H, W, H / 4, W / 4, 2};
+  return cdv_graph_table_finish(fill, n_fill, graph_ws, E_max, k_range, ix, jx, poses, patches, intrinsics, coords, true, stream, &lv);
 }
 
 extern "C" int cdv_update_prologue_table(
@@ -121,5 +122,6 @@
   hipLaunchKernelGGL(update_prologue_kernel, dim3(n_ing + n_tf + n_hist), dim3(256), 0, (hipStream_t)stream, ing, n_ing,
                      tf, n_tf, hist, n_hist);
   CDV_LAUNCH_CHECK();
-  return cdv_graph_finish(ii, jj, kk, E, graph_ws, E_max, k_range, n_hist, ix, jx, stream);
+  const cdv::CorrLevels lv{C, H, W, H / 4, W / 4, 2};
+  return cdv_graph_finish(ii, jj, kk, E, graph_ws, E_max, k_range, n_hist, ix, jx, stream, &lv);
 }
diff --git a/cdv_slam_amd/ops.py b/cdv_slam_amd/ops.py
--- a/cdv_slam_amd/ops.py
+++ b/cdv_slam_amd/ops.py
@@ -293,7 +293,7 @@
         R, chunks = self.table_capacity, (self.table_capacity + 15) // 16
         return (w32[o[0]:o[0] + R], w32[o[1]:o[1] + R], w32[o[2]:o[2] + chunks * 32 * 16 * 4].view(-1, 4),
                 w32[o[3]:o[3] + (self.E_cap + 1) * 4].view(-1, 4), w32[o[4]:o[4] + self.E_cap],
-                w32[o[5]:o[5] + self.E_cap * 24].view(-1, 24), w32[o[6]:o[6] + R])
+                w32[o[5]:o[5] + self.E_cap * 32].view(-1, 32), w32[o[6]:o[6] + R])
 
     def meta(self):
         m = (ctypes.c_int64 * 8)()
```

Result: slower. 10130 (-2.3%).
